# avikde/robobee3d

Measured on AMD Instinct MI355X. Metric: closed-loop MPC steps/sec (QP+dyn), higher is better.
Workload: dtype f32

## Files before the change

### robobee3d_amd/asmstep.py

```python
import functools
import os
import struct

from . import asmgen, asmtext, symbolic
from .asmgen import (A_D, A_L, A_LO, A_M, A_Q, NLDS, NVZ, S_ALPHA, S_CNT, S_ITERS, S_OMA, S_RHO, S_RINV, S_SIGMA,
                     V_W, V_WZ, V_X, V_Y, V_Z, Emit, f32bits, pk, _sb, _vp)

HERE = os.path.dirname(os.path.abspath(__file__))

PTRS = ["state", "ctrl", "ref", "ws", "out", "stats", "status", "info", "Ib", "gain", "aT0",
        "taskf", "weights", "wl", "wlu", "wlw",
        "done"]
NPTR_RES = 11
INTS = ["stride", "K", "maxIter", "nsub", "plant", "seq"]
TAIL_INTS = ["refstep"]
FLOATS = ["dt", "dtg", "Tmax", "wpr", "wpf", "ws_", "wvr", "wvf", "wds", "wthrust", "wmom",
          "iwpr", "iwpf", "iws", "iwvr", "iwvf", "iwds", "iwthrust", "iwmom",
          "Ib0", "Ib1", "Ib2", "Ibi0", "Ibi1", "Ibi2", "h", "hh", "h6", "taulim", "gpl", "idt", "mbg"]
WNAMES = ["wpr", "wpf", "ws_", "wvr", "wvf", "wds", "wthrust", "wmom"]
WROW = {"ws_": 0, "wds": 1, "wpr": 2, "wpf": 3, "wvr": 4, "wvf": 5, "wthrust": 6, "wmom": 7}
A_W, A_IW = 230, 238
S_PARAM = 4
S_PBLK = 2
S_PTR = {n: 40 + 2 * k for k, n in enumerate(PTRS[:NPTR_RES])}
S_PTR["taskf"], S_PTR["weights"] = 0, 96
S_PTR["wl"], S_PTR["wlu"], S_PTR["wlw"] = 30, 32, 34
S_INT = {"stride": 10, "K": 13, "maxIter": S_ITERS, "nsub": 5, "plant": 39}
S_F = {n: 64 + k for k, n in enumerate(FLOATS)}
assert max(S_F.values()) <= 95
S_STEP, S_SUB, S_RUIZ = 12, 15, 15
S_EXACT = 14
S_MBAD, S_MP0 = 62, 14
S_M0, S_M1, S_M2, S_M3 = 30, 32, 34, 36
S_C = {"minscal": 16, "maxscal": 17, "c45": 18, "eps10": 19, "eps": 38, "rho": 6, "rinv": 7, "rmin": 8,
       "rmininv": 9, "infty_ms": 100, "rhotol": 101}
S_TMP = 4
OFF = {}
_o = 0
for _n in PTRS:
    OFF[_n] = _o
    _o += 8
for _n in INTS + FLOATS + TAIL_INTS:
    OFF[_n] = _o
    _o += 4
PARAM_BYTES = _o
HIST_INTS = ["statestep", "outstep", "statusstep", "infostep"]
HIST_OFF = (PARAM_BYTES + 7) // 8 * 8
for _k, _n in enumerate(HIST_INTS):
    OFF[_n] = HIST_OFF + 4 * _k
HIST_BYTES = 4 * len(HIST_INTS)
S_HIST = 32
IMP_OFF = HIST_OFF + HIST_BYTES
assert IMP_OFF % 8 == 0
OFF["imp"], OFF["impstep"] = IMP_OFF, IMP_OFF + 8
IMP_BYTES = 16
S_IMP = 32

VFIRST, VEND = 2, 256
NRING = 6
XV_N, XV_B = 2, 254
NT_PTRS = ("state", "ctrl", "ref", "out", "stats")
A_SPARE, N_SPARE_D = 246, 9


class Pool:

    def __init__(self, e):
        self.e = e
        self.free_ = set(range(VFIRST, VEND))
        self.peak = 0
        self.fixed = set()

    def _take(self, regs):
        for r in regs:
            assert r in self.free_, "v%d is not free" % r
            self.free_.discard(r)
        self.peak = max(self.peak, VEND - VFIRST - len(self.free_))

    def reserve(self, lo, n):
        self._take(range(lo, lo + n))
        return lo

    def get(self):
        cand = sorted(self.free_)
        assert cand, "out of VGPRs"
        for r in cand:
            if (r ^ 1) not in self.free_:
                self._take([r])
                return r
        self._take([cand[0]])
        return cand[0]

    def get2(self):
        for r in sorted(self.free_):
            if r % 2 == 0 and r + 1 in self.free_:
                self._take([r, r + 1])
                return r
        raise AssertionError("out of aligned VGPR pairs")

    def get4(self):
        for r in sorted(self.free_):
            if r % 4 == 0 and all(r + k in self.free_ for k in range(4)):
                self._take([r, r + 1, r + 2, r + 3])
                return r
        raise AssertionError("out of aligned VGPR quads")

    def getn(self, n):
        for r in sorted(self.free_):
            if r % 2 == 0 and all(r + k in self.free_ for k in range(n)):
                self._take(range(r, r + n))
                return r
        raise AssertionError("out of consecutive VGPRs")

    def getn_high(self, n):
        r = VEND - n - (VEND - n) % 2
# ... 77 lines not shown
        for p in range(len(s.A_i)):
            if p in used:
                continue
            i0, j0 = s.A_i[p], self.col_of[p]
            for q_ in range(p + 1, len(s.A_i)):
                if q_ in used:
                    continue
                i1, j1 = s.A_i[q_], self.col_of[q_]
                if (self.zs[i0] ^ 1) == self.zs[i1] and (j0 == j1 or (self.xs[j0] ^ 1) == self.xs[j1]):
                    lo, hi = (p, q_) if self.zs[i0] % 2 == 0 else (q_, p)
                    pairs.append((lo, hi))
                    used.update((p, q_))
                    break
        self.apairs = pairs
        self.asingles = [p for p in range(len(s.A_i)) if p not in used]
        self.apos = [0] * len(s.A_i)
        k = 0
        for (lo, hi) in pairs:
            self.apos[lo], self.apos[hi] = k, k + 1
            k += 2
        for p in self.asingles:
            self.apos[p] = k
            k += 1
        self.na = k
        self.pair_of = {}
        for (lo, hi) in pairs:
            self.pair_of[lo] = self.pair_of[hi] = (lo, hi)
        NYv = symbolic.NY
        self.qnz = list(range(s.N * NYv)) + [s.N * NYv + k_ * NYv + i for k_ in range(s.N) for i in range(3)]
        self.qslot = {}
        for j in range(s.N * NYv):
            self.qslot[j] = self.xs[j]
        base = s.N * NYv
        for k_ in range(s.N):
            for i in range(3):
                self.qslot[s.N * NYv + k_ * NYv + i] = base + 3 * k_ + i
        self.nq = base + 3 * s.N
        self.qzero = frozenset(j for j in range(nx) if j not in self.qslot)
        lnz = set(range(6)) | set(range(3 * 6, 3 * 6 + 6)) | set(range(4 * 6, 4 * 6 + 3)) | {5 * 6 + 2}
        self.lzero = frozenset(i for i in range(self.neq) if i not in lnz) if s.N == 3 else frozenset()

    def weight_of(self, j):
        N, NYv = self.s.N, symbolic.NY
        if j < N * NYv:
            k, i = divmod(j, NYv)
            return ("wpf" if k == N - 1 else "wpr") if i < 3 else "ws_"
        if j < 2 * N * NYv:
            k, i = divmod(j - N * NYv, NYv)
            return ("wvf" if k == N - 1 else "wvr") if i < 3 else "wds"
        return "wthrust" if (j - 2 * N * NYv) % 3 == 0 else "wmom"


class StepGen:
    def __init__(self, N=3, perm=None, quad=False, exact_ruiz=False):
        self.st = Struct(N, perm)
        self.s = self.st.s
        self.e = Emit()
        self.pool = Pool(self.e)
        self.lab = 20
        self.lab_spec = 500
        self.quad = quad
        self.speculate = not quad and not exact_ruiz
        self.ruiz_span = self.restart_at = None
        self.nt = () if quad else ("nt",)
        self.homes = asmgen.Homes(NRING, 0 if quad else XV_N, XV_B)

    def label(self):
        self.lab += 1
        return str(self.lab)

    def label_spec(self):
        self.lab_spec += 1
        return str(self.lab_spec)

    def rcp_nr(self, dst, src, t):
        e = self.e
        e("v_rcp_f32", v(dst), v(src))
        e("s_nop", 0)
        e("v_fma_f32", v(t), "-" + v(src), v(dst), 1.0)
        e("v_fma_f32", v(dst), v(t), v(dst), v(dst))

    def rows_ptr(self, voff, first_row):
        e = self.e
        if first_row == 0:
            e("v_mov_b32", v(voff), "v0")
        else:
            e("s_mul_i32", sg(S_TMP), sg(S_INT["stride"]), first_row)
            e("v_add_u32", v(voff), sg(S_TMP), "v0")

    def load_taskf(self):
        e = self.e
        e("s_lshl_b32", sg(S_TMP), sg(S_STEP), 5)
        e("s_load_dwordx2", sp(S_M0), sp(S_PTR["taskf"]), sg(S_TMP), "offset:0")
        e("s_load_dwordx4", "s[%d:%d]" % (S_M0 + 2, S_M0 + 5), sp(S_PTR["taskf"]), sg(S_TMP), "offset:8")
        e("s_load_dwordx2", sp(S_M0 + 6), sp(S_PTR["taskf"]), sg(S_TMP), "offset:24")
        e("s_waitcnt", "vmcnt(0) lgkmcnt(0)")

    def adv(self, voff):
        self.e("v_add_u32", v(voff), sg(S_INT["stride"]), v(voff))

    def advance_ptr(self, ptr, sstep):
        e, lo = self.e, S_PTR[ptr]
        e("s_add_i32", sg(lo), sg(lo), sg(sstep))
        e("s_cmp_lt_u32", sg(lo), sg(sstep))
        e("s_cselect_b32", sg(sstep), 1, 0)
        e("s_add_i32", sg(lo + 1), sg(lo + 1), sg(sstep))

    def impulse(self, Y0, YS):
        e = self.e
        lab_off = self.label()
        lo, hi, st, oh = S_IMP, S_IMP + 1, S_IMP + 2, S_IMP + 3
        e("s_mov_b32", sg(S_TMP), IMP_OFF)
        e("s_load_dwordx4", "s[%d:%d]" % (S_IMP, S_IMP + 3), sp(S_PBLK), sg(S_TMP))
        e("s_waitcnt", "lgkmcnt(0)")
        e("s_cmp_eq_u64", sp(lo), 0)
        e("s_cbranch_scc1", lab_off + "f")
        e("s_mul_hi_u32", sg(oh), sg(S_STEP), sg(st))
        e("s_mul_i32", sg(st), sg(S_STEP), sg(st))
        e("s_add_i32", sg(hi), sg(hi), sg(oh))
        for i in range(6):
            addend = st if i == 0 else S_INT["stride"]
            lab_nc = self.label()
            e("s_add_i32", sg(lo), sg(lo), sg(addend))
            e("s_cmp_gt_u32", sg(addend), sg(lo))
            e("s_cbranch_scc0", lab_nc + "f")
            e("s_add_i32", sg(hi), sg(hi), 1)
            e("label", lab_nc)
            e("global_load_dword", v(YS + i), "v0", sp(lo))
        e("s_waitcnt", "vmcnt(0)")
        for i in range(6):
            e("v_add_f32", v(Y0 + 12 + i), v(Y0 + 12 + i), v(YS + i))
        e("label", lab_off)

    def load_rows(self, ptr, first_row, regs, voff=None):
        own = voff is None
        if own:
            voff = self.pool.get()
        self.rows_ptr(voff, first_row)
        for k, r in enumerate(regs):
            self.e("global_load_dword", r if isinstance(r, str) else v(r), v(voff), sp(S_PTR[ptr]),
                   *(self.nt if ptr in NT_PTRS or ptr == "ws" else ()))
            if k + 1 < len(regs):
                self.adv(voff)
        if own:
            self.pool.free(voff, kill=False)

    def store_rows(self, ptr, first_row, regs, voff=None):
        own = voff is None
        if own:
            voff = self.pool.get()
        self.rows_ptr(voff, first_row)
        for k, r in enumerate(regs):
# ... 186 lines not shown
        dtT0 = g_()
        e("v_mul_f32", v(dtT0), SF("dt"), v(T0))
        s0dt = [g_() for _ in range(3)]
        Bdt = [g_() for _ in range(6)]
        for i in range(3):
            e("v_mul_f32", v(s0dt[i]), SF("dt"), v(s0[i]))
        for i in range(6):
            e("v_mul_f32", v(Bdt[i]), SF("dt"), v(Btau[i]))
        pool.free(*Btau, *ds0, T0)
        VP = pool.getn(nx + 1)
        VQ = pool.getn_high(st.nq + st.nq % 2)
        VA = pool.getn(st.na + st.na % 2)
        self.VP, self.VQ, self.VA = VP, VQ, VA
        RP = lambda j: VP + st.xs[j]
        RA = lambda p: VA + st.apos[p]
        RQ = lambda j: VQ + st.qslot[j]
        self.RP, self.RA, self.RQ = RP, RA, RQ
        for j in range(nx):
            e("v_accvgpr_read_b32", v(RP(j)), "a%d" % (A_W + WNAMES.index(st.weight_of(j))))
        e("v_mov_b32", v(VP + nx), 0)
        ydes = RF[0:3] + RF[6:9]
        dpdes = RF[3:6]
        WV = {n: pool.get() for n in ("wpr", "wpf", "ws_", "wvr", "wvf")}
        for n, r in WV.items():
            e("v_accvgpr_read_b32", v(r), "a%d" % (A_W + WNAMES.index(n)))
        for j in st.qnz:
            if j < N * NYv:
                k, i = divmod(j, NYv)
                wname = ("wpf" if k == N - 1 else "wpr") if i < 3 else "ws_"
                e("v_mul_f32", v(RQ(j)), "-" + v(WV[wname]), v(ydes[i]))
            else:
                k, i = divmod(j - N * NYv, NYv)
                e("v_mul_f32", v(RQ(j)), "-" + v(WV["wvf" if k == N - 1 else "wvr"]), v(dpdes[i]))
        if st.nq % 2:
            e("v_mov_b32", v(VQ + st.nq), 0)
        for p, tag in enumerate(s.A_tag):
            if tag[0] == 'c':
                e("v_mov_b32", v(RA(p)), float(tag[1]))
            elif tag[0] == 'dt':
                e("v_mov_b32", v(RA(p)), SF("dt"))
            elif tag[0] == 'T0dt':
                e("v_mov_b32", v(RA(p)), v(dtT0))
            elif tag[0] == 's0':
                e("v_mov_b32", v(RA(p)), v(s0dt[tag[1]]))
            else:
                e("v_mov_b32", v(RA(p)), v(Bdt[tag[1]]))
        if st.na % 2:
            e("v_mov_b32", v(VA + st.na), 0)
        pool.free(dtT0, *s0dt, *Bdt, t)
        pool.free(*ST)
        pool.free(*RF)
        pool.free(*WV.values())
        pool.free_range(LS, 20)
        self.ruiz_quad() if self.quad else self.ruiz()
        self.recover_and_bounds()
        self.factor()

    def maxabs(self, dst, regs, acc_in=False):
        e = self.e
        regs = list(regs)
        if not acc_in:
            if len(regs) == 1:
                e("v_and_b32", v(dst), 0x7fffffff, v(regs[0]))
                return
            if len(regs) == 2:
                e("v_max_f32", v(dst), "|%s|" % v(regs[0]), "|%s|" % v(regs[1]))
                return
            e("v_max3_f32", v(dst), "|%s|" % v(regs[0]), "|%s|" % v(regs[1]), "|%s|" % v(regs[2]))
            regs = regs[3:]
        while len(regs) >= 2:
            e("v_max3_f32", v(dst), v(dst), "|%s|" % v(regs[0]), "|%s|" % v(regs[1]))
            regs = regs[2:]
        if regs:
            e("v_max_f32", v(dst), v(dst), "|%s|" % v(regs[0]))

    def limit(self, regs, rsq):
        e = self.e
        regs = list(regs)
        prev = None
        for r in regs + [None]:
            if r is not None:
                e("v_cmp_lt_f32", "vcc", sg(S_C["minscal"]), v(r))
            if prev is not None:
                e("v_min_f32", v(prev), sg(S_C["maxscal"]), v(prev))
            if r is not None:
                e("v_cndmask_b32", v(r), 1.0, v(r), "vcc")
            prev = r
        if rsq:
            for r in regs:
                e("v_rsq_f32", v(r), v(r))
            e("s_nop", 0)

    def scalings(self, regs, track):
        if track is None:
            return self.limit(regs, rsq=True)
        e = self.e
        regs = list(regs)
        lo, hi = track
        for k in range(0, len(regs) - 1, 2):
            e("v_min3_f32", v(lo), v(lo), v(regs[k]), v(regs[k + 1]))
            e("v_max3_f32", v(hi), v(hi), v(regs[k]), v(regs[k + 1]))
        if len(regs) % 2:
            e("v_min_f32", v(lo), v(lo), v(regs[-1]))
            e("v_max_f32", v(hi), v(hi), v(regs[-1]))
        for r in regs:
            e("v_rsq_f32", v(r), v(r))
        e("s_nop", 0)

# ... 252 lines not shown
        self.maxabs(qn, [hostQ[C] for C in sorted(hostQ)])
        e("s_mov_b64", "exec", sp(S_L3))
        e("v_mov_b32", v(acc), 0)
        e("v_mov_b32", v(qn), 0)
        e("s_mov_b64", "exec", sp(asmquad.S_EXEC))
        e("s_nop", 4)
        for perm_ in ([1, 0, 3, 2], [2, 3, 0, 1]):
            e("v_add_f32_dpp", v(acc), v(acc), v(acc), asmquad.qperm(perm_))
            e("v_max_f32_dpp", v(qn), v(qn), v(qn), asmquad.qperm(perm_))
            e("s_nop", 1)
        e("v_mul_f32", v(acc), sg(S_C["c45"]), v(acc))
        self.limit([qn], rsq=False)
        e("v_max_f32", v(acc), v(acc), v(qn))
        self.limit([acc], rsq=False)
        self.rcp_nr(ct, acc, tt)
        for C in range(15):
            e("v_mul_f32", v(hostP[C]), v(hostP[C]), v(ct))
            if C in hostQ:
                e("v_mul_f32", v(hostQ[C]), v(hostQ[C]), v(ct))
        e("v_mul_f32", v(cs), v(cs), v(ct))
        e("s_sub_i32", sg(S_RUIZ), sg(S_RUIZ), 1)
        e("s_cmp_gt_i32", sg(S_RUIZ), 0)
        e("s_cbranch_scc1", top + "b")
        e("s_nop", 1)

        def bcast(dst, src, ln):
            e("v_mov_b32_dpp", v(dst), v(src), asmquad.qperm([ln] * 4))
        for key, d in rp.slots.items():
            for ln in sorted(d, reverse=True):
                bcast(RA(d[ln]), hostA[key], ln)
        for C, m in colmem.items():
            for ln in sorted(m, reverse=True):
                bcast(RP(m[ln]), hostP[C], ln)
            if C in hostQ:
                for ln in sorted(m, reverse=True):
                    bcast(RQ(m[ln]), hostQ[C], ln)
        e("v_mov_b32", v(self.VP + nx), 0)
        if st.nq % 2:
            e("v_mov_b32", v(self.VQ + st.nq), 0)
        if st.na % 2:
            e("v_mov_b32", v(self.VA + st.na), 0)
        e("s_nop", 1)
        e("quad_end", tuple(keep))

    def recover_and_bounds(self):
        e, pool, st, s = self.e, self.pool, self.st, self.s
        N, nx, nc, neq = s.N, s.nx, s.nc, st.neq
        RP, RA, RQ, RE, cs = self.RP, self.RA, self.RQ, self.RE, self.cs
        SF = lambda n: sg(S_F[n])
        cinv, t, d, r = pool.get(), pool.get(), pool.get(), pool.get()
        self.rcp_nr(cinv, cs, t)
        voff = pool.get()
        npark = 0 if self.quad else N_SPARE_D
        self.rows_ptr(voff, npark)
        rows_of_col = {}
        for i in range(nc):
            rows_of_col.setdefault(st.unit[i][1], []).append(i)
        IWV = {n: pool.get() for n in WNAMES}
        for k, n in enumerate(WNAMES):
            e("v_accvgpr_read_b32", v(IWV[n]), "a%d" % (A_IW + k))
        for j in range(nx):
            e("v_mul_f32", v(d), v(RP(j)), v(cinv))
            e("v_mul_f32", v(d), v(IWV[st.weight_of(j)]), v(d))
            e("v_sqrt_f32", v(d), v(d))
            e("s_nop", 0)
            if j < npark:
                e("v_accvgpr_write_b32", "a%d" % (A_SPARE + j), v(d))
            else:
                e("global_store_dword", v(voff), v(d), sp(S_PTR["ws"]), *self.nt)
                self.adv(voff)
            if j in rows_of_col:
                e("v_rcp_f32", v(r), v(d))
                e("s_nop", 0)
                for i in rows_of_col[j]:
                    e("v_mul_f32", v(RE(i)), "|%s|" % v(RA(st.unit[i][0])), v(r))
        assert asmgen.WS_ES == asmgen.WS_DS + nx and asmgen.WS_C == asmgen.WS_ES + nc
        for i in range(nc):
            e("global_store_dword", v(voff), v(RE(i)), sp(S_PTR["ws"]), *self.nt)
            self.adv(voff)
        if npark:
            e("v_accvgpr_write_b32", "a%d" % (A_SPARE + N_SPARE_D), v(cs))
        else:
            e("global_store_dword", v(voff), v(cs), sp(S_PTR["ws"]))
        self.store_rows("ctrl", nx + 2 * nc + 1, [RE(neq + k) for k in range(N)], voff)
        pool.free(cinv, d, r, voff, cs, *IWV.values())
        LS = pool.getn(20)
        for qd in range(5):
            e("ds_read_b128", "v[%d:%d]" % (LS + 4 * qd, LS + 4 * qd + 3), "v1", qd * 1024)
        zero = pool.get()
        e("v_mov_b32", v(zero), 0)
        for j in range(nx):
            e("v_accvgpr_write_b32", "a%d" % (A_Q + j), v(RQ(j)) if j in st.qslot else v(zero))
        e("s_waitcnt", "lgkmcnt(0)")
        src = {}
        for i in range(6):
            src[i] = LS + i
            src[3 * 6 + i] = LS + 6 + i
        for i in range(3):
            src[4 * 6 + i] = LS + 12 + i
        for i in range(neq):
            if i in src:
                e("v_mul_f32", v(t), v(src[i]), v(RE(i)))
                e("v_accvgpr_write_b32", "a%d" % (A_LO + i), v(t))
            elif i == 5 * 6 + 2:
                e("v_mul_f32", v(t), SF("dtg"), v(RE(i)))
                e("v_accvgpr_write_b32", "a%d" % (A_LO + i), v(t))
            else:
                e("v_accvgpr_write_b32", "a%d" % (A_LO + i), v(zero))
        for k in range(N):
            e("v_mul_f32", v(t), v(LS + 15), v(RE(neq + k)))
            e("v_accvgpr_write_b32", "a%d" % (A_M + k), v(t))
            e("v_mul_f32", v(t), v(LS + 16), v(RE(neq + k)))
            e("v_accvgpr_write_b32", "a%d" % (A_M + N + k), v(t))
        pool.free(zero, t)
        pool.free_range(LS, 20)
        pool.free_range(self.VE, nc + 1)
        pool.free_range(self.VQ, st.nq + st.nq % 2)

    def factor(self):
        e, pool, st, s = self.e, self.pool, self.st, self.s
        nx, nc, nk, neq = s.nx, s.nc, s.nk, st.neq
        RP, RA = self.RP, self.RA
        lpos = st.lpos
        last_row = {}
        for c in range(nk):
            if s.L_p[c + 1] > s.L_p[c]:
                last_row[c] = s.L_i[s.L_p[c + 1] - 1]
        done_at = {}
        for c, r in last_row.items():
            done_at.setdefault(r, []).append(c)
# ... 60 lines not shown
                pool.free(yc)
            assert not y
            di = pool.get()
            self.rcp_nr(di, dk, t)
            pool.free(dk)
            Dinv[k] = di
            for c in done_at.get(k, []):
                retire_col(c)
            if k not in last_row:
                retire_dinv(k)
        assert not nL and not Dinv
        pool.free(t)
        if self._rinv_reg is not None:
            pool.free(self._rinv_reg)
            self._rinv_reg = None
        if st.na % 2:
            pool.free(self.VA + st.na)
        pool.free(self.VP + nx)

    _rinv_reg = None

    def _vconst_rinv(self):
        if self._rinv_reg is None:
            self._rinv_reg = self.pool.get()
            self.e("v_mov_b32", v(self._rinv_reg), sg(S_RINV))
        return v(self._rinv_reg)

    def admm(self):
        e, pool, st, s = self.e, self.pool, self.st, self.s
        nx, nc = s.nx, s.nc
        left = set(range(VFIRST, VEND)) - pool.free_ - set(range(246, 256))
        assert not left, "phase A leaked registers: %s" % sorted(left)
        pool.reserve(V_W, V_X - V_W)
        pool.reserve(V_X, V_Y - V_X)
        pool.reserve(V_Y, V_Z - V_Y)
        pool.reserve(V_Z, 40)
        voff = 245
        self.load_rows("ctrl", 0, [V_X + st.xs[r] for r in range(nx)] + [V_Y + st.zs[r] for r in range(nc)] +
                       [V_Z + st.zs[r] for r in range(nc)], voff)
        for pad in (V_X + nx, V_Y + nc, V_Z + nc, V_W + nx, V_WZ + nc):
            e("v_mov_b32", v(pad), 0)
        e("s_waitcnt", "vmcnt(0) lgkmcnt(0)")
        plan = st.plan
        zk = dict(qzero=st.qzero, lzero=st.lzero, homes=self.homes)
        asmgen.body(e, s, first=True, capture=True, plan=plan, delta_in_w=True, **zk)
        if self.quad:
            from . import asmquad
            lab6 = self.label()
            e("s_cmp_lt_i32", sg(S_ITERS), 2)
            e("s_cbranch_scc1", lab6 + "f")
            asmquad.section(e, asmquad.QuadPlan(st), self.label)
            e("label", lab6)
        else:
            self._admm_rest(plan, zk)
        for i in range(st.neq):
            pool.free(V_Z + st.zs[i], kill=True)
        pool.free_range(246, 10)


    def _admm_rest(self, plan, zk):
        e, s, st = self.e, self.s, self.st
        import numpy as np
        for p_ in range(NVZ):
            e("v_accvgpr_read_b32", v(V_Z + p_), "a%d" % (A_L + p_))
        lab7, lab6 = self.label(), self.label()
        e("s_sub_i32", sg(S_CNT), sg(S_ITERS), 1)
        e("s_cmp_lt_i32", sg(S_CNT), 1)
        e("s_cbranch_scc1", lab6 + "f")
        e("label", lab7)
        asmgen.body(e, s, first=False, capture=False, plan=plan, lv=True, dy3_in_w=True, **zk)
        e("s_sub_i32", sg(S_CNT), sg(S_CNT), 1)
        e("s_cmp_gt_i32", sg(S_CNT), 0)
        e("s_cbranch_scc1", lab7 + "b")
        k = float(np.float32(1.6) / (np.float32(1.6) - np.float32(1.0)))
        e("s_mov_b32", sg(S_TMP), f32bits(k))
        nx, neq = s.nx, st.neq
        for p_ in range(0, nx - 1, 2):
            pk(e, "v_pk_add_f32", V_W + p_, [P2(V_X + p_), P2(V_W + p_)], [0, 1])
        for p_ in range(0, nx - 1, 2):
            pk(e, "v_pk_mul_f32", V_W + p_, [PS(S_TMP), P2(V_W + p_)])
        if nx % 2:
            jl = st.xinv[nx - 1]
            e("v_sub_f32", v(V_W + st.xs[jl]), v(V_X + st.xs[jl]), v(V_W + st.xs[jl]))
            e("v_mul_f32", v(V_W + st.xs[jl]), sg(S_TMP), v(V_W + st.xs[jl]))
        for p_ in range(0, neq, 2):
            pk(e, "v_pk_add_f32", V_WZ + p_, [P2(V_Y + p_), P2(V_WZ + p_)], [0, 1])
        for p_ in range(0, neq, 2):
            pk(e, "v_pk_mul_f32", V_WZ + p_, [PS(S_TMP), P2(V_WZ + p_)])
        e("label", lab6)

    def phase_c(self):
        e, pool, st, s = self.e, self.pool, self.st, self.s
        N, NYv = s.N, symbolic.NY
        nx, nc, neq = s.nx, s.nc, st.neq
        SF = lambda n: sg(S_F[n])
        g_ = pool.get
        XR = lambda j: V_X + st.xs[j]
        YR = lambda i: V_Y + st.zs[i]
        ZR = lambda i: V_Z + st.zs[i]
        DXR = lambda j: V_W + st.xs[j]
        DYR = lambda i: V_WZ + st.zs[i]
        voff = g_()
        def slot_blocks(n, chunk=16):
            n2 = n + n % 2
            blocks = [(lo, pool.getn(min(chunk, n2 - lo))) for lo in range(0, n2, chunk)]
            def reg(slot):
                for lo, base in reversed(blocks):
                    if slot >= lo:
                        return base + slot - lo
            return reg, [(base, min(chunk, n2 - lo)) for lo, base in blocks]
        DS, dblocks = slot_blocks(nx)
        DR = lambda j: DS(st.xs[j])
        cr, T0 = g_(), g_()
        npark = 0 if self.quad else N_SPARE_D
        self.load_rows("ws", npark, [DR(j) for j in range(npark, nx)], voff)
        if npark:
            for j in range(npark):
                e("v_accvgpr_read_b32", v(DR(j)), "a%d" % (A_SPARE + j))
            e("v_accvgpr_read_b32", v(cr), "a%d" % (A_SPARE + N_SPARE_D))
        else:
            self.load_rows("ws", asmgen.WS_C - asmgen.WS_DS, [cr], voff)
        self.load_rows("ctrl", nx + 2 * nc, [T0], voff)
        e("v_mov_b32", v(DS(nx)), 0)
        zt = [g_() for _ in range(4)]
        self.rows_ptr(voff, 0)
        for r in range(nx):
            e("global_store_dword", v(voff), v(XR(r)), sp(S_PTR["ctrl"]), *self.nt)
            self.adv(voff)
        for r in range(nc):
            e("global_store_dword", v(voff), v(YR(r)), sp(S_PTR["ctrl"]), *self.nt)
            self.adv(voff)
        for r in range(nc):
            if r < neq:
                t_ = zt[r % 4]
                e("v_accvgpr_read_b32", v(t_), "a%d" % (A_LO + r))
                e("global_store_dword", v(voff), v(t_), sp(S_PTR["ctrl"]), *self.nt)
            else:
                e("global_store_dword", v(voff), v(ZR(r)), sp(S_PTR["ctrl"]), *self.nt)
            self.adv(voff)
        pool.free(*zt)
        e("s_waitcnt", "vmcnt(0)")
        for k in range(0, nx + 1, 2):
            pk(e, "v_pk_mul_f32", V_W + k, [P2(DS(k)), P2(V_W + k)])
            pk(e, "v_pk_mul_f32", V_X + k, [P2(DS(k)), P2(V_X + k)])
        for base, n_ in dblocks:
            pool.free_range(base, n_)
        ES, eblocks = slot_blocks(nc)
        ER = lambda i: ES(st.zs[i])
        ST = [g_() for _ in range(18)]
        RF = [g_() for _ in range(9)]
        self.load_rows("ws", asmgen.WS_ES - asmgen.WS_DS, [ER(i) for i in range(nc)], voff)
        self.load_rows("state", 0, ST, voff)
        self.load_rows("ref", 0, RF, voff)
        e("v_mov_b32", v(ES(nc)), 1.0)
        lab_tk = self.label()
        e("s_cmp_eq_u64", sp(S_PTR["taskf"]), 0)
        e("s_cbranch_scc1", lab_tk + "f")
        self.load_taskf()
        for i in range(3):
            e("v_add_f32", v(RF[i]), sg(S_M0 + i), v(RF[i]))
            e("v_mov_b32", v(RF[3 + i]), sg(S_M0 + 3 + i))
        e("v_mov_b32", v(RF[6]), sg(S_M0 + 6))
        e("v_mov_b32", v(RF[7]), 0)
        e("v_mov_b32", v(RF[8]), sg(S_M0 + 7))
        e("label", lab_tk)
        cinv, t = g_(), g_()
        self.rcp_nr(cinv, cr, t)
        pool.free(cr)
        ibi0, ibi1 = g_(), g_()
        lab_ib, lab_ib2 = self.label(), self.label()
        e("s_cmp_eq_u64", sp(S_PTR["Ib"]), 0)
        e("s_cbranch_scc1", lab_ib + "f")
        self.load_rows("Ib", 0, [ibi0, ibi1], voff)
        e("s_waitcnt", "vmcnt(0)")
        tt = g_()
        for r in (ibi0, ibi1):
            e("v_mov_b32", v(tt), v(r))
            self.rcp_nr(r, tt, t)
        pool.free(tt)
        e("s_branch", lab_ib2 + "f")
        e("label", lab_ib)
        e("v_mov_b32", v(ibi0), SF("Ibi0"))
        e("v_mov_b32", v(ibi1), SF("Ibi1"))
        e("label", lab_ib2)
        e("s_waitcnt", "vmcnt(0)")
        for k in range(0, nc + 1, 2):
            pk(e, "v_pk_mul_f32", V_WZ + k, [P2(ES(k)), P2(V_WZ + k)])
            pk(e, "v_pk_mul_f32", V_Y + k, [P2(ES(k)), P2(V_Y + k)])
        for k in range(0, nc + 1, 2):
            pk(e, "v_pk_mul_f32", V_Y + k, [P2(V_Y + k), PB(cinv)])
        pool.free(cinv)
        zu3 = [g_() for _ in range(N)]
        for k in range(N):
            e("v_rcp_f32", v(zu3[k]), v(ER(neq + k)))
        e("s_nop", 0)
        for k in range(N):
            e("v_mul_f32", v(zu3[k]), v(ZR(neq + k)), v(zu3[k]))
        for base, n_ in eblocks:
            pool.free_range(base, n_)
        for k in range(N):
            pool.free(ZR(neq + k))
        pool.free(V_Z + nc)
        p0, R0, dq0 = ST[0:3], ST[3:12], ST[12:18]
        dtT0 = g_()
        e("v_mul_f32", v(dtT0), SF("dt"), v(T0))
        s0dt = [g_() for _ in range(3)]
        Bdt = [g_() for _ in range(6)]
        for i in range(3):
            e("v_mul_f32", v(s0dt[i]), SF("dt"), v(R0[6 + i]))
            e("v_mul_f32", v(Bdt[i]), "-" + v(R0[i + 3]), v(ibi0))
            e("v_mul_f32", v(Bdt[3 + i]), v(R0[i]), v(ibi1))
        for i in range(6):
            e("v_mul_f32", v(Bdt[i]), SF("dt"), v(Bdt[i]))
        pool.free(ibi0, ibi1)
        ds0 = [g_() for _ in range(3)]
        for r in range(3):
            e("v_mul_f32", v(t), "-" + v(R0[r]), v(dq0[4]))
            e("v_mul_f32", v(ds0[r]), v(R0[r + 3]), v(dq0[3]))
            e("v_add_f32", v(ds0[r]), v(t), v(ds0[r]))
            e("v_mul_f32", v(ds0[r]), -1.0, v(ds0[r]))
        y0 = p0 + R0[6:9]
        dy0 = dq0[0:3] + ds0
        LR = {}
        y1 = [g_() for _ in range(6)]
        for i in range(6):
            LR[i] = g_()
            e("v_mul_f32", v(t), SF("dt"), v(dy0[i]))
            e("v_add_f32", v(y1[i]), v(y0[i]), v(t))
            e("v_mul_f32", v(LR[i]), -1.0, v(y1[i]))
        for i in range(6):
            LR[18 + i] = g_()
            if i < 3:
                e("v_mul_f32", v(t), v(T0), v(y0[i + 3]))
                e("v_mul_f32", v(t), SF("dt"), v(t))
                e("v_sub_f32", v(LR[18 + i]), "-" + v(dy0[i]), v(t))
                if i == 2:
                    e("v_add_f32", v(LR[18 + i]), SF("dtg"), v(LR[18 + i]))
            else:
# ... 205 lines not shown
            e("v_cndmask_b32", v(r), v(r), v(nanv), "vcc")
        pool.free(nanv)
        u0, u1, u2 = sol[0:3]
        dy1 = sol[3:9]
        OUT = [g_() for _ in range(9)]
        e("v_add_f32", v(OUT[0]), v(T0), v(u0))
        e("v_mov_b32", v(OUT[1]), v(u1))
        e("v_mov_b32", v(OUT[2]), v(u2))
        e("v_mul_f32", v(a1), v(R0[0]), v(dy1[3]))
        e("v_mul_f32", v(t), v(R0[1]), v(dy1[4]))
        e("v_add_f32", v(a1), v(a1), v(t))
        e("v_mul_f32", v(t), v(R0[2]), v(dy1[5]))
        e("v_add_f32", v(a1), v(a1), v(t))
        e("v_mul_f32", v(a2), v(R0[3]), v(dy1[3]))
        e("v_mul_f32", v(t), v(R0[4]), v(dy1[4]))
        e("v_add_f32", v(a2), v(a2), v(t))
        e("v_mul_f32", v(t), v(R0[5]), v(dy1[5]))
        e("v_add_f32", v(a2), v(a2), v(t))
        for i in range(3):
            e("v_sub_f32", v(OUT[3 + i]), v(dy1[i]), v(dq0[i]))
        e("v_sub_f32", v(OUT[6]), "-" + v(a2), v(dq0[3]))
        e("v_sub_f32", v(OUT[7]), v(a1), v(dq0[4]))
        e("v_sub_f32", v(OUT[8]), 0, v(dq0[5]))
        for i in range(6):
            e("v_mul_f32", v(OUT[3 + i]), SF("idt"), v(OUT[3 + i]))
        self.store_rows("out", 0, OUT, voff)
        lab_s, lab_i, lab_c = self.label(), self.label(), self.label()
        e("s_cmp_eq_u64", sp(S_PTR["status"]), 0)
        e("s_cbranch_scc1", lab_s + "f")
        e("global_store_dword", "v0", v(stv), sp(S_PTR["status"]))
        e("label", lab_s)
        e("s_cmp_eq_u64", sp(S_PTR["info"]), 0)
        e("s_cbranch_scc1", lab_i + "f")
        self.store_rows("info", 0, [pri, dua], voff)
        e("label", lab_i)
        e("s_and_saveexec_b64", sp(S_M1), MBAD)
        e("s_cbranch_execz", lab_c + "f")
        e("v_mov_b32", v(a1), 0)
        self.rows_ptr(voff, 0)
        for r in range(nx + 2 * nc):
            e("global_store_dword", v(voff), v(a1), sp(S_PTR["ctrl"]))
            self.adv(voff)
        e("label", lab_c)
        e("s_mov_b64", "exec", sp(S_M1))
        pool.free(pri, dua, stv, a1, a2, t, T0, *RF)
        pool.free_range(V_W, V_X - V_W, kill=False)
        pool.free_range(V_X, V_Y - V_X, kill=False)
        pool.free_range(V_Y, V_Z - V_Y, kill=False)
        T0n = g_()
        e("v_mov_b32", v(T0n), v(OUT[0]))
        self.wl_step(OUT, R0, T0n, voff)
        self.store_rows("ctrl", nx + 2 * nc, [T0n], voff)
        pool.free(T0n)
        self.plant(ST, OUT, voff)
        pool.free(*OUT, *ST, voff)
        assert len(pool.free_) == VEND - VFIRST, "phase C leaked registers: %s" % sorted(set(range(VFIRST, VEND)) - pool.free_)

    def wl_step(self, OUT, R0, T0n, voff):
        e, pool = self.e, self.pool
        g_ = pool.get
        lab_end = self.label()
        P = sp(S_PBLK)
        e("s_load_dwordx2", sp(S_PTR["wl"]), P, OFF["wl"])
        e("s_load_dwordx2", sp(S_PTR["wlu"]), P, OFF["wlu"])
        e("s_load_dwordx2", sp(S_PTR["wlw"]), P, OFF["wlw"])
        e("s_waitcnt", "lgkmcnt(0)")
        e("s_cmp_eq_u64", sp(S_PTR["wl"]), 0)
        e("s_cbranch_scc1", lab_end + "f")
        O_UMIN, O_UMAX, O_DUMAX, O_QW, O_A0, O_A1, O_A2, O_MD = 0, 4, 8, 12, 18, 24, 48, 144
        a1, a2, t = g_(), g_(), g_()
        zero = g_()
        e("v_mov_b32", v(zero), 0)

        def prm(dst, word):
            e("global_load_dword", v(dst), v(zero), sp(S_PTR["wl"]), "offset:%d" % (4 * word))
        u0 = [g_() for _ in range(4)]
        self.load_rows("wlu", 0, u0, voff)
        Md = [g_() for _ in range(6)]
        for i in range(6):
            prm(Md[i], O_MD + i)
        e("s_waitcnt", "vmcnt(0)")
        h0 = [g_() for _ in range(3)]
        pd = [g_() for _ in range(6)]
        for c in range(3):
            e("v_mul_f32", v(h0[c]), SF_("mbg"), v(R0[2 + 3 * c]))
        for i in range(6):
            e("v_mul_f32", v(pd[i]), v(Md[i]), v(OUT[3 + i]))
        w0 = [g_() for _ in range(6)]
        a0v = [g_() for _ in range(6)]
        A1 = [[g_() for _ in range(4)] for _ in range(6)]
        PA = [g_() for _ in range(21)]
        vout = [g_() for _ in range(4)]
        dot, quad = g_(), g_()
        for i in range(6):
            prm(PA[0], O_A0 + i)
            for l in range(4):
                prm(PA[1 + l], O_A1 + 4 * i + l)
            for k in range(16):
                prm(PA[5 + k], O_A2 + 16 * i + k)
            e("s_waitcnt", "vmcnt(0)")
            e("v_mul_f32", v(dot), v(u0[0]), v(PA[1]))
            for l in range(1, 4):
                e("v_mul_f32", v(t), v(u0[l]), v(PA[1 + l]))
                e("v_add_f32", v(dot), v(dot), v(t))
            for r in range(4):
                e("v_mul_f32", v(vout[r]), v(PA[5 + r]), v(u0[0]))
# ... 329 lines not shown
            e("v_mul_f32", v(dst + 5), v(a), v(Ibi[0]))
            e("v_sub_f32", v(b), v(u2), v(b))
            e("v_mul_f32", v(dst + 6), v(b), v(Ibi[1]))
            e("v_mul_f32", v(dst + 7), "-" + v(hz), v(Ibi[2]))
        e("s_mov_b32", sg(S_SUB), sg(S_INT["nsub"]))
        top = self.label()
        e("label", top)
        vf(Q0, QA)
        for k in range(0, 8, 2):
            pk(e, "v_pk_fma_f32", QS + k, [PS(S_F["hh"]), P2(QA + k), P2(Q0 + k)])
        vf(QS, QK)
        for k in range(0, 8, 2):
            pk(e, "v_pk_fma_f32", QA + k, [PB(two), P2(QK + k), P2(QA + k)])
            pk(e, "v_pk_fma_f32", QS + k, [PS(S_F["hh"]), P2(QK + k), P2(Q0 + k)])
        vf(QS, QK)
        for k in range(0, 8, 2):
            pk(e, "v_pk_fma_f32", QA + k, [PB(two), P2(QK + k), P2(QA + k)])
            pk(e, "v_pk_fma_f32", QS + k, [PS(S_F["h"]), P2(QK + k), P2(Q0 + k)])
        vf(QS, QK)
        for k in range(0, 8, 2):
            pk(e, "v_pk_add_f32", QA + k, [P2(QA + k), P2(QK + k)])
        for k in range(0, 8, 2):
            pk(e, "v_pk_fma_f32", Q0 + k, [PS(S_F["h6"]), P2(QA + k), P2(Q0 + k)])
        e("s_nop", 1)
        for r in range(3):
            e("v_mov_b32_dpp", v(PA + r), v(Q0), asmquad.qperm([r] * 4))
        e("s_nop", 1)
        for r in range(3):
            e("v_fmac_f32", v(serr), v(PA + r), v(PA + r))
        e("v_add_f32", v(seff), v(seff), v(einc))
        e("s_sub_i32", sg(S_SUB), sg(S_SUB), 1)
        e("s_cmp_gt_i32", sg(S_SUB), 0)
        e("s_cbranch_scc1", top + "b")
        e("s_nop", 1)
        for r in range(3):
            e("v_mov_b32_dpp", v(Y0 + r), v(Q0), asmquad.qperm([r] * 4))
            e("v_mov_b32_dpp", v(Y0 + 12 + r), v(Q0 + 1), asmquad.qperm([r] * 4))
            for c in range(3):
                e("v_mov_b32_dpp", v(Y0 + 3 + r + 3 * c), v(Q0 + 2 + c), asmquad.qperm([r] * 4))
        for i in range(3):
            e("v_mov_b32", v(Y0 + 15 + i), v(Q0 + 5 + i))
        e("s_nop", 1)
        e("quad_end", tuple(keep))

    def program(self):
        e = self.e
        self.prologue()
        top = self.label()
        e("label", top)
        if self.speculate:
            e("s_mov_b32", sg(S_EXACT), 0)
            self.lab_restart = self.label_spec()
            e("label", self.lab_restart)
        self.phase_a()
        self.admm()
        self.phase_c()
        e("s_load_dword", sg(S_TMP), sp(S_PBLK), OFF["refstep"])
        e("s_load_dwordx4", "s[%d:%d]" % (S_HIST, S_HIST + 3), sp(S_PBLK), HIST_OFF)
        e("s_waitcnt", "lgkmcnt(0)")
        e("s_add_u32", sg(S_PTR["ref"]), sg(S_PTR["ref"]), sg(S_TMP))
        e("s_addc_u32", sg(S_PTR["ref"] + 1), sg(S_PTR["ref"] + 1), 0)
        for n in ("out", "status", "info"):
            self.advance_ptr(n, S_HIST + HIST_INTS.index(n + "step"))
        e("s_add_i32", sg(S_STEP), sg(S_STEP), 1)
        e("s_cmp_lt_i32", sg(S_STEP), sg(S_INT["K"]))
        e("s_cbranch_scc1", top + "b")
        e("s_waitcnt", "vmcnt(0) lgkmcnt(0)")
        lab = self.label()
        e("s_load_dwordx2", sp(S_M0), sp(S_PBLK), OFF["done"])
        e("s_load_dword", sg(S_M1), sp(S_PBLK), OFF["seq"])
        e("s_waitcnt", "lgkmcnt(0)")
        e("s_cmp_eq_u64", sp(S_M0), 0)
        e("s_cbranch_scc1", lab + "f")
        e("buffer_wbl2", "sc0 sc1")
        e("s_waitcnt", "vmcnt(0)")
        a, b = self.pool.get(), self.pool.get()
        e("v_mov_b32", v(a), 0)
        e("v_mov_b32", v(b), sg(S_M1))
        e("global_store_dword", v(a), v(b), sp(S_M0), "sc0 sc1")
        e("s_waitcnt", "vmcnt(0)")
        self.pool.free(a, b)
        e("label", lab)
        return e.ins


fmt = functools.partial(asmtext.fmt, hex_ints=asmtext.HEX_ABOVE_64)


PSEUDO = ("kill", "quad_begin", "quad_end")


def write(path=None, N=3, perm=None, quad=False):
    path = path or os.path.join(HERE, "csrc", "umpc_step_asm_quad.h" if quad else "umpc_step_asm.h")
    g = StepGen(N, perm, quad=quad)
    ins = [t for t in g.program() if t[0] not in PSEUDO]
    if quad:
        head = ["// GENERATED by robobee3d_amd/asmstep.py (quad=True) + asmquad.py -- do not edit.", asmgen.switch_banner(),
               "// The all-assembly fp32 step kernel body, ONE ROBOT PER LANE QUAD (16 robots per wavefront): %d instructions."
               % len(ins),
               "// Every lane of a quad gets the same v0 (= 4 * robot) and its own LDS slice; include umpc_step_asm.h first (StepParams).",
               "#pragma once"]
    else:
        head = ["// GENERATED by robobee3d_amd/asmstep.py -- do not edit.", asmgen.switch_banner(),
               "// The all-assembly fp32 step kernel body: %d instructions (K closed-loop steps of one wavefront)." % len(ins),
               "#pragma once", "#include <stddef.h>", "#include <stdint.h>", "namespace umpcasm {",
               "// parameter block read by the kernel with s_load (byte offsets are part of the generated code)",
               "struct StepParams {"]
        for n in PTRS:
            head.append("  const void *%s;" % n)
        for n in INTS:
            head.append("  int32_t %s;" % n)
        for n in FLOATS:
            head.append("  float %s;" % n)
        for n in TAIL_INTS:
            head.append("  int32_t %s;" % n)
        head += ["};", "static_assert(sizeof(StepParams) == %d, \"StepParams layout\");" % ((PARAM_BYTES + 7) // 8 * 8),
                "// step history (umpcBatchSetHistory): bytes the state / out / status / info pointers advance per closed-loop step,",
                "// read by the stream at byte %d of the kernarg segment: the kernels take ONE StepArgs as their first argument" % HIST_OFF,
                "struct StepHist {"] + ["  int32_t %s;" % n for n in HIST_INTS] + ["};",
                "// velocity impulses (umpcBatchSetImpulses): slice `cursor` of the table [steps][6][B] (null: none) and the bytes per slice,",
                "// read by the stream at byte %d of the kernarg segment" % IMP_OFF,
                "struct StepImp {", "  const void *imp;", "  int32_t impstep;", "  int32_t pad_;", "};",
                "struct StepArgs {", "  StepParams p;", "  StepHist h;", "  StepImp i;", "};",
                "static_assert(offsetof(StepArgs, h) == %d && sizeof(StepHist) == %d, \"StepHist layout\");" % (HIST_OFF, HIST_BYTES),
                "static_assert(offsetof(StepArgs, i) == %d && sizeof(StepImp) == %d && offsetof(StepImp, impstep) == 8, \"StepImp layout\");" % (IMP_OFF, IMP_BYTES),
                "constexpr int STEP_LDS_BYTES_PER_LANE = %d;" % (NLDS * 4), "}  // namespace umpcasm",
                "// inputs: v0 = 4 * robot, v1 = lane LDS address, s[4:5] = &StepParams (kernarg)"]
    asmtext.write_if_changed(path, asmtext.asm_block(
        head, "UMPC_STEP_ASM%s(voff, ldsaddr, params)" % ("_QUAD" if quad else ""), ins,
        '"{v0}"(voff), "{v1}"(ldsaddr), "{s[4:5]}"(params)',
        asmtext.clobbers(range(2, 256), range(256), range(4, 102)), fmt))
    return path, len(ins)


_KEEP_V = {0, 1} | set(range(V_W, V_Z)) | set(range(V_Z + 2 * 3 * symbolic.NY, V_Z + 40))
QUAD = {None: None}


def _quad():
    from . import isasim
    if QUAD[None] is None:
        QUAD.update({None: isasim.Quad(v=_KEEP_V, dead_v=set(range(256)) - _KEEP_V, a=range(A_LO, 256), dead_a=range(A_LO)),
                     "ruiz": isasim.Quad(a=range(256)), "plant": isasim.Quad(a=range(256))})
    return QUAD


FLAT = ("taskf", "wl")
STRIDE = 4096
PBASE = 0x00007E0080000000


def simulate(ins, arrays, ints, floats, max_exec=3000000, ptr_xform=None, lanes=1, hits=False):
    import numpy as np
    from . import isasim
    base_of = {n: 0x00007F0080000000 + (k << 36) for k, n in enumerate(PTRS + ["impulse"])}
    ptr_xform = ptr_xform or (lambda a: a)
    blob = bytearray(IMP_OFF + IMP_BYTES)
    for n in PTRS:
        struct.pack_into("<Q", blob, OFF[n], ptr_xform(base_of[n]) if arrays.get(n) is not None else 0)
    stride = STRIDE if lanes == 1 else 4 * lanes
    allints = dict(ints, stride=stride)
    allints.setdefault("seq", 0)
    allints.setdefault("refstep", 0)
    for n in HIST_INTS:
        allints.setdefault(n, 0)
    for n in INTS + TAIL_INTS + HIST_INTS:
        struct.pack_into("<i", blob, OFF[n], int(allints[n]))
    for n in FLOATS:
        struct.pack_into("<f", blob, OFF[n], float(floats[n]))
    allints.setdefault("impstep", 6 * stride if arrays.get("impulse") is not None else 0)
    struct.pack_into("<Q", blob, OFF["imp"], ptr_xform(base_of["impulse"]) if arrays.get("impulse") is not None else 0)
    struct.pack_into("<i", blob, OFF["impstep"], int(allints["impstep"]))
    regions = [(PBASE, 4, np.frombuffer(bytes(blob), np.uint32))] + \
        [(base_of[n], 4 if n in FLAT or lanes > 1 else STRIDE, arrays[n].reshape(-1))
         for n in PTRS + ["impulse"] if arrays.get(n) is not None]
    assert all(arrays[n].flags.c_contiguous for n in PTRS + ["impulse"] if arrays.get(n) is not None)
    m = isasim.Machine(ins, lanes, regions=regions, sgpr={S_PARAM: PBASE & 0xFFFFFFFF, S_PARAM + 1: PBASE >> 32},
                       vgpr={0: 4 * np.arange(lanes)}, lds=np.zeros((lanes, NLDS), np.uint32), max_exec=max_exec,
                       quad=_quad() if lanes == 1 else None)
    if hits:
        m.hits = np.zeros(len(ins), np.int64)
    isasim.run(m)
    simulate.last_hits = m.hits
    simulate.last_quad_sections = {("admm" if k is None else k): n for k, n in m.sections.items()}
    simulate.last_quad_instructions = sum(m.sections.values())
    return m.nexec


if __name__ == "__main__":
    p, n = write()
    print("wrote", p, n, "instructions")


def host_floats(dt=5.0, g=9.81e-3, TtoWmax=2.0, ws=1e1, wds=1e3, wpr=1.0, wpf=5.0, wvr=1e3, wvf=2e3, wthrust=1e-1, wmom=1e-2,
                Ib=(3333.0, 3333.0, 1000.0), dtsim=0.2, taulim=100.0, mb=100.0):
    import numpy as np
    f = np.float32
    one = f(1.0)
    w = dict(wpr=f(wpr), wpf=f(wpf), ws_=f(ws), wvr=f(wvr), wvf=f(wvf), wds=f(wds), wthrust=f(wthrust), wmom=f(wmom))
    d = dict(dt=f(dt), dtg=f(f(dt) * f(g)), Tmax=f(f(TtoWmax) * f(g)), **w)
    for k, val in w.items():
        d["i" + k.rstrip("_")] = f(one / val)
    for i in range(3):
        d["Ib%d" % i] = f(Ib[i])
        d["Ibi%d" % i] = f(one / f(Ib[i]))
    d.update(h=f(dtsim), hh=f(f(0.5) * f(dtsim)), h6=f(f(dtsim) / f(6.0)), taulim=f(taulim), gpl=f(9.81e-3), idt=f(one / f(dt)),
             mbg=f(f(mb) * f(g)))
    assert set(d) == set(FLOATS), set(FLOATS) ^ set(d)
    return {k: float(val) for k, val in d.items()}
```

### robobee3d_amd/csrc/umpc_step_asm.h

```cpp
#pragma once
#include <stddef.h>
#include <stdint.h>
namespace umpcasm {
struct StepParams {
  const void *state;
  const void *ctrl;
  const void *ref;
  const void *ws;
  const void *out;
  const void *stats;
  const void *status;
  const void *info;
  const void *Ib;
  const void *gain;
  const void *aT0;
  const void *taskf;
  const void *weights;
  const void *wl;
  const void *wlu;
  const void *wlw;
  const void *done;
  int32_t stride;
  int32_t K;
  int32_t maxIter;
// ... 1929 lines not shown
  "v_pk_mul_f32 v[82:83], v[82:83], v[48:49] op_sel:[0,0] op_sel_hi:[1,0] neg_lo:[0,0] neg_hi:[0,0]\n" \
  "v_pk_mul_f32 v[84:85], v[84:85], v[48:49] op_sel:[0,0] op_sel_hi:[1,0] neg_lo:[0,0] neg_hi:[0,0]\n" \
  "v_pk_mul_f32 v[86:87], v[86:87], v[48:49] op_sel:[0,0] op_sel_hi:[1,0] neg_lo:[0,0] neg_hi:[0,0]\n" \
  "v_pk_mul_f32 v[88:89], v[88:89], v[48:49] op_sel:[0,0] op_sel_hi:[1,0] neg_lo:[0,0] neg_hi:[0,0]\n" \
  "v_pk_mul_f32 v[90:91], v[90:91], v[48:49] op_sel:[0,0] op_sel_hi:[1,0] neg_lo:[0,0] neg_hi:[0,0]\n" \
  "v_pk_mul_f32 v[92:93], v[92:93], v[48:49] op_sel:[0,0] op_sel_hi:[1,0] neg_lo:[0,0] neg_hi:[0,0]\n" \
  "v_pk_mul_f32 v[94:95], v[94:95], v[48:49] op_sel:[0,0] op_sel_hi:[1,0] neg_lo:[0,0] neg_hi:[0,0]\n" \
  "v_pk_mul_f32 v[96:97], v[96:97], v[48:49] op_sel:[0,0] op_sel_hi:[1,0] neg_lo:[0,0] neg_hi:[0,0]\n" \
  "v_pk_mul_f32 v[98:99], v[98:99], v[48:49] op_sel:[0,0] op_sel_hi:[1,0] neg_lo:[0,0] neg_hi:[0,0]\n" \
  "v_pk_mul_f32 v[100:101], v[100:101], v[48:49] op_sel:[0,0] op_sel_hi:[1,0] neg_lo:[0,0] neg_hi:[0,0]\n" \
  "v_pk_mul_f32 v[102:103], v[102:103], v[48:49] op_sel:[0,0] op_sel_hi:[1,0] neg_lo:[0,0] neg_hi:[0,0]\n" \
  "v_pk_mul_f32 v[104:105], v[104:105], v[48:49] op_sel:[0,0] op_sel_hi:[1,0] neg_lo:[0,0] neg_hi:[0,0]\n" \
  "v_pk_mul_f32 v[106:107], v[106:107], v[48:49] op_sel:[0,0] op_sel_hi:[1,0] neg_lo:[0,0] neg_hi:[0,0]\n" \
  "v_pk_mul_f32 v[108:109], v[108:109], v[48:49] op_sel:[0,0] op_sel_hi:[1,0] neg_lo:[0,0] neg_hi:[0,0]\n" \
  "v_pk_mul_f32 v[110:111], v[110:111], v[48:49] op_sel:[0,0] op_sel_hi:[1,0] neg_lo:[0,0] neg_hi:[0,0]\n" \
  "v_pk_mul_f32 v[112:113], v[112:113], v[48:49] op_sel:[0,0] op_sel_hi:[1,0] neg_lo:[0,0] neg_hi:[0,0]\n" \
  "v_pk_mul_f32 v[114:115], v[114:115], v[48:49] op_sel:[0,0] op_sel_hi:[1,0] neg_lo:[0,0] neg_hi:[0,0]\n" \
  "v_pk_mul_f32 v[228:229], v[228:229], v[48:49] op_sel:[0,0] op_sel_hi:[1,0] neg_lo:[0,0] neg_hi:[0,0]\n" \
  "v_pk_mul_f32 v[230:231], v[230:231], v[48:49] op_sel:[0,0] op_sel_hi:[1,0] neg_lo:[0,0] neg_hi:[0,0]\n" \
  "v_pk_mul_f32 v[232:233], v[232:233], v[48:49] op_sel:[0,0] op_sel_hi:[1,0] neg_lo:[0,0] neg_hi:[0,0]\n" \
  "v_pk_mul_f32 v[234:235], v[234:235], v[48:49] op_sel:[0,0] op_sel_hi:[1,0] neg_lo:[0,0] neg_hi:[0,0]\n" \
  "v_pk_mul_f32 v[236:237], v[236:237], v[48:49] op_sel:[0,0] op_sel_hi:[1,0] neg_lo:[0,0] neg_hi:[0,0]\n" \
  "v_pk_mul_f32 v[238:239], v[238:239], v[48:49] op_sel:[0,0] op_sel_hi:[1,0] neg_lo:[0,0] neg_hi:[0,0]\n" \
  "v_pk_mul_f32 v[240:241], v[240:241], v[48:49] op_sel:[0,0] op_sel_hi:[1,0] neg_lo:[0,0] neg_hi:[0,0]\n" \
  "v_pk_mul_f32 v[242:243], v[242:243], v[48:49] op_sel:[0,0] op_sel_hi:[1,0] neg_lo:[0,0] neg_hi:[0,0]\n" \
  "v_pk_mul_f32 v[244:245], v[244:245], v[48:49] op_sel:[0,0] op_sel_hi:[1,0] neg_lo:[0,0] neg_hi:[0,0]\n" \
  "v_pk_mul_f32 v[246:247], v[246:247], v[48:49] op_sel:[0,0] op_sel_hi:[1,0] neg_lo:[0,0] neg_hi:[0,0]\n" \
  "v_pk_mul_f32 v[248:249], v[248:249], v[48:49] op_sel:[0,0] op_sel_hi:[1,0] neg_lo:[0,0] neg_hi:[0,0]\n" \
  "v_pk_mul_f32 v[250:251], v[250:251], v[48:49] op_sel:[0,0] op_sel_hi:[1,0] neg_lo:[0,0] neg_hi:[0,0]\n" \
  "v_pk_mul_f32 v[252:253], v[252:253], v[48:49] op_sel:[0,0] op_sel_hi:[1,0] neg_lo:[0,0] neg_hi:[0,0]\n" \
  "v_pk_mul_f32 v[254:255], v[254:255], v[48:49] op_sel:[0,0] op_sel_hi:[1,0] neg_lo:[0,0] neg_hi:[0,0]\n" \
  "v_mul_f32 v42, v42, v48\n" \
  "s_sub_i32 s15, s15, 1\n" \
  "s_cmp_gt_i32 s15, 0\n" \
  "s_cbranch_scc1 503b\n" \
  "v_cmp_lt_f32_e64 s[30:31], s16, v43\n" \
  "v_cmp_ge_f32_e64 s[32:33], s17, v44\n" \
  "s_and_b64 s[30:31], s[30:31], s[32:33]\n" \
  "s_andn2_b64 s[30:31], exec, s[30:31]\n" \
  "s_cbranch_scc0 505f\n" \
  "s_mov_b32 s14, 1\n" \
  "s_waitcnt vmcnt(0) lgkmcnt(0)\n" \
  "s_branch 501b\n" \
  "504:\n" \
  "s_cmp_gt_i32 s15, 0\n" \
  "s_cbranch_scc1 28b\n" \
  "505:\n" \
  "v_rcp_f32 v43, v42\n" \
  "s_nop 0\n" \
  "v_fma_f32 v44, -v42, v43, 1.0\n" \
  "v_fma_f32 v43, v44, v43, v43\n" \
  "s_mul_i32 s4, s10, 9\n" \
  "v_add_u32 v47, s4, v0\n" \
  "v_accvgpr_read_b32 v48, a238\n" \
  "v_accvgpr_read_b32 v49, a239\n" \
  "v_accvgpr_read_b32 v50, a240\n" \
  "v_accvgpr_read_b32 v51, a241\n" \
  "v_accvgpr_read_b32 v52, a242\n" \
  "v_accvgpr_read_b32 v53, a243\n" \
  "v_accvgpr_read_b32 v54, a244\n" \
  "v_accvgpr_read_b32 v55, a245\n" \
  "v_mul_f32 v45, v70, v43\n" \
  "v_mul_f32 v45, v48, v45\n" \
  "v_sqrt_f32 v45, v45\n" \
  "s_nop 0\n" \
  "v_accvgpr_write_b32 a246, v45\n" \
  "v_rcp_f32 v46, v45\n" \
  "s_nop 0\n" \
  "v_mul_f32 v2, |v116|, v46\n" \
  "v_mul_f32 v8, |v118|, v46\n" \
  "v_mul_f32 v45, v71, v43\n" \
  "v_mul_f32 v45, v48, v45\n" \
  "v_sqrt_f32 v45, v45\n" \
  "s_nop 0\n" \
  "v_accvgpr_write_b32 a247, v45\n" \
  "v_rcp_f32 v46, v45\n" \
  "s_nop 0\n" \
  "v_mul_f32 v3, |v117|, v46\n" \
  "v_mul_f32 v9, |v119|, v46\n" \
  "v_mul_f32 v45, v72, v43\n" \
  "v_mul_f32 v45, v48, v45\n" \
  "v_sqrt_f32 v45, v45\n" \
  "s_nop 0\n" \
  "v_accvgpr_write_b32 a248, v45\n" \
  "v_rcp_f32 v46, v45\n" \
  "s_nop 0\n" \
  "v_mul_f32 v4, |v120|, v46\n" \
  "v_mul_f32 v10, |v122|, v46\n" \
  "v_mul_f32 v45, v74, v43\n" \
  "v_mul_f32 v45, v50, v45\n" \
  "v_sqrt_f32 v45, v45\n" \
  "s_nop 0\n" \
  "v_accvgpr_write_b32 a249, v45\n" \
  "v_rcp_f32 v46, v45\n" \
  "s_nop 0\n" \
  "v_mul_f32 v6, |v124|, v46\n" \
  "v_mul_f32 v12, |v126|, v46\n" \
  "v_mul_f32 v45, v75, v43\n" \
  "v_mul_f32 v45, v50, v45\n" \
  "v_sqrt_f32 v45, v45\n" \
  "s_nop 0\n" \
  "v_accvgpr_write_b32 a250, v45\n" \
  "v_rcp_f32 v46, v45\n" \
  "s_nop 0\n" \
  "v_mul_f32 v7, |v125|, v46\n" \
  "v_mul_f32 v13, |v127|, v46\n" \
  "v_mul_f32 v45, v73, v43\n" \
  "v_mul_f32 v45, v50, v45\n" \
  "v_sqrt_f32 v45, v45\n" \
  "s_nop 0\n" \
  "v_accvgpr_write_b32 a251, v45\n" \
  "v_rcp_f32 v46, v45\n" \
  "s_nop 0\n" \
  "v_mul_f32 v5, |v121|, v46\n" \
  "v_mul_f32 v11, |v123|, v46\n" \
  "v_mul_f32 v45, v76, v43\n" \
  "v_mul_f32 v45, v48, v45\n" \
  "v_sqrt_f32 v45, v45\n" \
  "s_nop 0\n" \
  "v_accvgpr_write_b32 a252, v45\n" \
  "v_rcp_f32 v46, v45\n" \
  "s_nop 0\n" \
  "v_mul_f32 v14, |v132|, v46\n" \
  "v_mul_f32 v45, v77, v43\n" \
  "v_mul_f32 v45, v48, v45\n" \
  "v_sqrt_f32 v45, v45\n" \
  "s_nop 0\n" \
  "v_accvgpr_write_b32 a253, v45\n" \
  "v_rcp_f32 v46, v45\n" \
  "s_nop 0\n" \
  "v_mul_f32 v15, |v133|, v46\n" \
  "v_mul_f32 v45, v78, v43\n" \
  "v_mul_f32 v45, v48, v45\n" \
  "v_sqrt_f32 v45, v45\n" \
  "s_nop 0\n" \
  "v_accvgpr_write_b32 a254, v45\n" \
  "v_rcp_f32 v46, v45\n" \
  "s_nop 0\n" \
  "v_mul_f32 v16, |v136|, v46\n" \
  "v_mul_f32 v45, v80, v43\n" \
  "v_mul_f32 v45, v50, v45\n" \
  "v_sqrt_f32 v45, v45\n" \
  "s_nop 0\n" \
  "global_store_dword v47, v45, s[46:47] nt\n" \
  "v_add_u32 v47, s10, v47\n" \
  "v_rcp_f32 v46, v45\n" \
  "s_nop 0\n" \
  "v_mul_f32 v18, |v140|, v46\n" \
  "v_mul_f32 v45, v81, v43\n" \
  "v_mul_f32 v45, v50, v45\n" \
  "v_sqrt_f32 v45, v45\n" \
  "s_nop 0\n" \
  "global_store_dword v47, v45, s[46:47] nt\n" \
  "v_add_u32 v47, s10, v47\n" \
  "v_rcp_f32 v46, v45\n" \
  "s_nop 0\n" \
  "v_mul_f32 v19, |v141|, v46\n" \
  "v_mul_f32 v45, v79, v43\n" \
  "v_mul_f32 v45, v50, v45\n" \
  "v_sqrt_f32 v45, v45\n" \
  "s_nop 0\n" \
  "global_store_dword v47, v45, s[46:47] nt\n" \
  "v_add_u32 v47, s10, v47\n" \
  "v_rcp_f32 v46, v45\n" \
  "s_nop 0\n" \
  "v_mul_f32 v17, |v137|, v46\n" \
  "v_mul_f32 v45, v82, v43\n" \
  "v_mul_f32 v45, v49, v45\n" \
  "v_sqrt_f32 v45, v45\n" \
  "s_nop 0\n" \
  "global_store_dword v47, v45, s[46:47] nt\n" \
  "v_add_u32 v47, s10, v47\n" \
  "v_mul_f32 v45, v83, v43\n" \
  "v_mul_f32 v45, v49, v45\n" \
  "v_sqrt_f32 v45, v45\n" \
  "s_nop 0\n" \
  "global_store_dword v47, v45, s[46:47] nt\n" \
  "v_add_u32 v47, s10, v47\n" \
  "v_mul_f32 v45, v84, v43\n" \
  "v_mul_f32 v45, v49, v45\n" \
  "v_sqrt_f32 v45, v45\n" \
  "s_nop 0\n" \
  "global_store_dword v47, v45, s[46:47] nt\n" \
  "v_add_u32 v47, s10, v47\n" \
  "v_mul_f32 v45, v86, v43\n" \
  "v_mul_f32 v45, v50, v45\n" \
  "v_sqrt_f32 v45, v45\n" \
  "s_nop 0\n" \
  "global_store_dword v47, v45, s[46:47] nt\n" \
  "v_add_u32 v47, s10, v47\n" \
  "v_mul_f32 v45, v87, v43\n" \
  "v_mul_f32 v45, v50, v45\n" \
  "v_sqrt_f32 v45, v45\n" \
  "s_nop 0\n" \
  "global_store_dword v47, v45, s[46:47] nt\n" \
  "v_add_u32 v47, s10, v47\n" \
  "v_mul_f32 v45, v85, v43\n" \
  "v_mul_f32 v45, v50, v45\n" \
  "v_sqrt_f32 v45, v45\n" \
  "s_nop 0\n" \
  "global_store_dword v47, v45, s[46:47] nt\n" \
  "v_add_u32 v47, s10, v47\n" \
  "v_mul_f32 v45, v88, v43\n" \
  "v_mul_f32 v45, v51, v45\n" \
  "v_sqrt_f32 v45, v45\n" \
  "s_nop 0\n" \
  "global_store_dword v47, v45, s[46:47] nt\n" \
  "v_add_u32 v47, s10, v47\n" \
  "v_rcp_f32 v46, v45\n" \
  "s_nop 0\n" \
  "v_mul_f32 v20, |v150|, v46\n" \
  "v_mul_f32 v26, |v152|, v46\n" \
  "v_mul_f32 v45, v89, v43\n" \
  "v_mul_f32 v45, v51, v45\n" \
  "v_sqrt_f32 v45, v45\n" \
  "s_nop 0\n" \
  "global_store_dword v47, v45, s[46:47] nt\n" \
  "v_add_u32 v47, s10, v47\n" \
  "v_rcp_f32 v46, v45\n" \
  "s_nop 0\n" \
  "v_mul_f32 v21, |v151|, v46\n" \
  "v_mul_f32 v27, |v153|, v46\n" \
  "v_mul_f32 v45, v90, v43\n" \
  "v_mul_f32 v45, v51, v45\n" \
  "v_sqrt_f32 v45, v45\n" \
  "s_nop 0\n" \
  "global_store_dword v47, v45, s[46:47] nt\n" \
  "v_add_u32 v47, s10, v47\n" \
  "v_rcp_f32 v46, v45\n" \
  "s_nop 0\n" \
  "v_mul_f32 v22, |v156|, v46\n" \
  "v_mul_f32 v28, |v158|, v46\n" \
  "v_mul_f32 v45, v92, v43\n" \
  "v_mul_f32 v45, v53, v45\n" \
  "v_sqrt_f32 v45, v45\n" \
  "s_nop 0\n" \
  "global_store_dword v47, v45, s[46:47] nt\n" \
  "v_add_u32 v47, s10, v47\n" \
  "v_rcp_f32 v46, v45\n" \
  "s_nop 0\n" \
  "v_mul_f32 v24, |v162|, v46\n" \
  "v_mul_f32 v30, |v164|, v46\n" \
  "v_mul_f32 v45, v93, v43\n" \
  "v_mul_f32 v45, v53, v45\n" \
  "v_sqrt_f32 v45, v45\n" \
  "s_nop 0\n" \
  "global_store_dword v47, v45, s[46:47] nt\n" \
  "v_add_u32 v47, s10, v47\n" \
  "v_rcp_f32 v46, v45\n" \
  "s_nop 0\n" \
  "v_mul_f32 v25, |v163|, v46\n" \
  "v_mul_f32 v31, |v165|, v46\n" \
  "v_mul_f32 v45, v91, v43\n" \
  "v_mul_f32 v45, v53, v45\n" \
  "v_sqrt_f32 v45, v45\n" \
  "s_nop 0\n" \
  "global_store_dword v47, v45, s[46:47] nt\n" \
  "v_add_u32 v47, s10, v47\n" \
  "v_rcp_f32 v46, v45\n" \
  "s_nop 0\n" \
  "v_mul_f32 v23, |v157|, v46\n" \
  "v_mul_f32 v29, |v159|, v46\n" \
  "v_mul_f32 v45, v94, v43\n" \
  "v_mul_f32 v45, v51, v45\n" \
  "v_sqrt_f32 v45, v45\n" \
  "s_nop 0\n" \
  "global_store_dword v47, v45, s[46:47] nt\n" \
  "v_add_u32 v47, s10, v47\n" \
  "v_rcp_f32 v46, v45\n" \
  "s_nop 0\n" \
  "v_mul_f32 v32, |v170|, v46\n" \
  "v_mul_f32 v45, v95, v43\n" \
  "v_mul_f32 v45, v51, v45\n" \
  "v_sqrt_f32 v45, v45\n" \
  "s_nop 0\n" \
  "global_store_dword v47, v45, s[46:47] nt\n" \
  "v_add_u32 v47, s10, v47\n" \
  "v_rcp_f32 v46, v45\n" \
  "s_nop 0\n" \
  "v_mul_f32 v33, |v171|, v46\n" \
  "v_mul_f32 v45, v96, v43\n" \
  "v_mul_f32 v45, v51, v45\n" \
  "v_sqrt_f32 v45, v45\n" \
  "s_nop 0\n" \
  "global_store_dword v47, v45, s[46:47] nt\n" \
  "v_add_u32 v47, s10, v47\n" \
  "v_rcp_f32 v46, v45\n" \
  "s_nop 0\n" \
  "v_mul_f32 v34, |v176|, v46\n" \
  "v_mul_f32 v45, v98, v43\n" \
  "v_mul_f32 v45, v53, v45\n" \
  "v_sqrt_f32 v45, v45\n" \
  "s_nop 0\n" \
  "global_store_dword v47, v45, s[46:47] nt\n" \
  "v_add_u32 v47, s10, v47\n" \
  "v_rcp_f32 v46, v45\n" \
  "s_nop 0\n" \
  "v_mul_f32 v36, |v182|, v46\n" \
  "v_mul_f32 v45, v99, v43\n" \
  "v_mul_f32 v45, v53, v45\n" \
  "v_sqrt_f32 v45, v45\n" \
  "s_nop 0\n" \
  "global_store_dword v47, v45, s[46:47] nt\n" \
  "v_add_u32 v47, s10, v47\n" \
  "v_rcp_f32 v46, v45\n" \
  "s_nop 0\n" \
  "v_mul_f32 v37, |v183|, v46\n" \
  "v_mul_f32 v45, v97, v43\n" \
  "v_mul_f32 v45, v53, v45\n" \
  "v_sqrt_f32 v45, v45\n" \
  "s_nop 0\n" \
  "global_store_dword v47, v45, s[46:47] nt\n" \
  "v_add_u32 v47, s10, v47\n" \
  "v_rcp_f32 v46, v45\n" \
  "s_nop 0\n" \
  "v_mul_f32 v35, |v177|, v46\n" \
  "v_mul_f32 v45, v100, v43\n" \
  "v_mul_f32 v45, v52, v45\n" \
  "v_sqrt_f32 v45, v45\n" \
  "s_nop 0\n" \
  "global_store_dword v47, v45, s[46:47] nt\n" \
  "v_add_u32 v47, s10, v47\n" \
  "v_mul_f32 v45, v101, v43\n" \
  "v_mul_f32 v45, v52, v45\n" \
  "v_sqrt_f32 v45, v45\n" \
  "s_nop 0\n" \
  "global_store_dword v47, v45, s[46:47] nt\n" \
  "v_add_u32 v47, s10, v47\n" \
  "v_mul_f32 v45, v102, v43\n" \
  "v_mul_f32 v45, v52, v45\n" \
  "v_sqrt_f32 v45, v45\n" \
  "s_nop 0\n" \
  "global_store_dword v47, v45, s[46:47] nt\n" \
  "v_add_u32 v47, s10, v47\n" \
  "v_mul_f32 v45, v104, v43\n" \
  "v_mul_f32 v45, v53, v45\n" \
  "v_sqrt_f32 v45, v45\n" \
  "s_nop 0\n" \
  "global_store_dword v47, v45, s[46:47] nt\n" \
  "v_add_u32 v47, s10, v47\n" \
  "v_mul_f32 v45, v105, v43\n" \
  "v_mul_f32 v45, v53, v45\n" \
  "v_sqrt_f32 v45, v45\n" \
  "s_nop 0\n" \
  "global_store_dword v47, v45, s[46:47] nt\n" \
  "v_add_u32 v47, s10, v47\n" \
  "v_mul_f32 v45, v103, v43\n" \
  "v_mul_f32 v45, v53, v45\n" \
  "v_sqrt_f32 v45, v45\n" \
  "s_nop 0\n" \
  "global_store_dword v47, v45, s[46:47] nt\n" \
  "v_add_u32 v47, s10, v47\n" \
  "v_mul_f32 v45, v106, v43\n" \
  "v_mul_f32 v45, v54, v45\n" \
  "v_sqrt_f32 v45, v45\n" \
  "s_nop 0\n" \
  "global_store_dword v47, v45, s[46:47] nt\n" \
  "v_add_u32 v47, s10, v47\n" \
  "v_rcp_f32 v46, v45\n" \
  "s_nop 0\n" \
  "v_mul_f32 v38, |v219|, v46\n" \
  "v_mul_f32 v45, v107, v43\n" \
  "v_mul_f32 v45, v55, v45\n" \
  "v_sqrt_f32 v45, v45\n" \
  "s_nop 0\n" \
  "global_store_dword v47, v45, s[46:47] nt\n" \
  "v_add_u32 v47, s10, v47\n" \
  "v_mul_f32 v45, v108, v43\n" \
  "v_mul_f32 v45, v55, v45\n" \
  "v_sqrt_f32 v45, v45\n" \
  "s_nop 0\n" \
  "global_store_dword v47, v45, s[46:47] nt\n" \
  "v_add_u32 v47, s10, v47\n" \
  "v_mul_f32 v45, v109, v43\n" \
  "v_mul_f32 v45, v54, v45\n" \
  "v_sqrt_f32 v45, v45\n" \
  "s_nop 0\n" \
  "global_store_dword v47, v45, s[46:47] nt\n" \
  "v_add_u32 v47, s10, v47\n" \
  "v_rcp_f32 v46, v45\n" \
  "s_nop 0\n" \
  "v_mul_f32 v39, |v222|, v46\n" \
  "v_mul_f32 v45, v110, v43\n" \
  "v_mul_f32 v45, v55, v45\n" \
  "v_sqrt_f32 v45, v45\n" \
  "s_nop 0\n" \
  "global_store_dword v47, v45, s[46:47] nt\n" \
  "v_add_u32 v47, s10, v47\n" \
  "v_mul_f32 v45, v111, v43\n" \
  "v_mul_f32 v45, v55, v45\n" \
  "v_sqrt_f32 v45, v45\n" \
  "s_nop 0\n" \
  "global_store_dword v47, v45, s[46:47] nt\n" \
  "v_add_u32 v47, s10, v47\n" \
  "v_mul_f32 v45, v112, v43\n" \
  "v_mul_f32 v45, v54, v45\n" \
  "v_sqrt_f32 v45, v45\n" \
  "s_nop 0\n" \
  "global_store_dword v47, v45, s[46:47] nt\n" \
  "v_add_u32 v47, s10, v47\n" \
  "v_rcp_f32 v46, v45\n" \
  "s_nop 0\n" \
  "v_mul_f32 v40, |v225|, v46\n" \
  "v_mul_f32 v45, v113, v43\n" \
  "v_mul_f32 v45, v55, v45\n" \
  "v_sqrt_f32 v45, v45\n" \
  "s_nop 0\n" \
  "global_store_dword v47, v45, s[46:47] nt\n" \
  "v_add_u32 v47, s10, v47\n" \
  "v_mul_f32 v45, v114, v43\n" \
  "v_mul_f32 v45, v55, v45\n" \
  "v_sqrt_f32 v45, v45\n" \
  "s_nop 0\n" \
  "global_store_dword v47, v45, s[46:47] nt\n" \
  "v_add_u32 v47, s10, v47\n" \
  "global_store_dword v47, v2, s[46:47] nt\n" \
  "v_add_u32 v47, s10, v47\n" \
  "global_store_dword v47, v3, s[46:47] nt\n" \
  "v_add_u32 v47, s10, v47\n" \
  "global_store_dword v47, v4, s[46:47] nt\n" \
  "v_add_u32 v47, s10, v47\n" \
  "global_store_dword v47, v6, s[46:47] nt\n" \
  "v_add_u32 v47, s10, v47\n" \
  "global_store_dword v47, v7, s[46:47] nt\n" \
  "v_add_u32 v47, s10, v47\n" \
  "global_store_dword v47, v5, s[46:47] nt\n" \
  "v_add_u32 v47, s10, v47\n" \
  "global_store_dword v47, v8, s[46:47] nt\n" \
  "v_add_u32 v47, s10, v47\n" \
  "global_store_dword v47, v9, s[46:47] nt\n" \
  "v_add_u32 v47, s10, v47\n" \
  "global_store_dword v47, v10, s[46:47] nt\n" \
  "v_add_u32 v47, s10, v47\n" \
  "global_store_dword v47, v12, s[46:47] nt\n" \
  "v_add_u32 v47, s10, v47\n" \
  "global_store_dword v47, v13, s[46:47] nt\n" \
  "v_add_u32 v47, s10, v47\n" \
  "global_store_dword v47, v11, s[46:47] nt\n" \
  "v_add_u32 v47, s10, v47\n" \
  "global_store_dword v47, v14, s[46:47] nt\n" \
  "v_add_u32 v47, s10, v47\n" \
  "global_store_dword v47, v15, s[46:47] nt\n" \
  "v_add_u32 v47, s10, v47\n" \
  "global_store_dword v47, v16, s[46:47] nt\n" \
  "v_add_u32 v47, s10, v47\n" \
  "global_store_dword v47, v18, s[46:47] nt\n" \
  "v_add_u32 v47, s10, v47\n" \
  "global_store_dword v47, v19, s[46:47] nt\n" \
  "v_add_u32 v47, s10, v47\n" \
  "global_store_dword v47, v17, s[46:47] nt\n" \
  "v_add_u32 v47, s10, v47\n" \
  "global_store_dword v47, v20, s[46:47] nt\n" \
  "v_add_u32 v47, s10, v47\n" \
  "global_store_dword v47, v21, s[46:47] nt\n" \
  "v_add_u32 v47, s10, v47\n" \
  "global_store_dword v47, v22, s[46:47] nt\n" \
  "v_add_u32 v47, s10, v47\n" \
  "global_store_dword v47, v24, s[46:47] nt\n" \
  "v_add_u32 v47, s10, v47\n" \
  "global_store_dword v47, v25, s[46:47] nt\n" \
  "v_add_u32 v47, s10, v47\n" \
  "global_store_dword v47, v23, s[46:47] nt\n" \
  "v_add_u32 v47, s10, v47\n" \
  "global_store_dword v47, v26, s[46:47] nt\n" \
  "v_add_u32 v47, s10, v47\n" \
  "global_store_dword v47, v27, s[46:47] nt\n" \
  "v_add_u32 v47, s10, v47\n" \
  "global_store_dword v47, v28, s[46:47] nt\n" \
  "v_add_u32 v47, s10, v47\n" \
  "global_store_dword v47, v30, s[46:47] nt\n" \
  "v_add_u32 v47, s10, v47\n" \
  "global_store_dword v47, v31, s[46:47] nt\n" \
  "v_add_u32 v47, s10, v47\n" \
  "global_store_dword v47, v29, s[46:47] nt\n" \
  "v_add_u32 v47, s10, v47\n" \
  "global_store_dword v47, v32, s[46:47] nt\n" \
  "v_add_u32 v47, s10, v47\n" \
  "global_store_dword v47, v33, s[46:47] nt\n" \
  "v_add_u32 v47, s10, v47\n" \
  "global_store_dword v47, v34, s[46:47] nt\n" \
  "v_add_u32 v47, s10, v47\n" \
  "global_store_dword v47, v36, s[46:47] nt\n" \
  "v_add_u32 v47, s10, v47\n" \
  "global_store_dword v47, v37, s[46:47] nt\n" \
  "v_add_u32 v47, s10, v47\n" \
  "global_store_dword v47, v35, s[46:47] nt\n" \
  "v_add_u32 v47, s10, v47\n" \
  "global_store_dword v47, v38, s[46:47] nt\n" \
  "v_add_u32 v47, s10, v47\n" \
  "global_store_dword v47, v39, s[46:47] nt\n" \
  "v_add_u32 v47, s10, v47\n" \
  "global_store_dword v47, v40, s[46:47] nt\n" \
  "v_add_u32 v47, s10, v47\n" \
  "v_accvgpr_write_b32 a255, v42\n" \
  "s_mul_i32 s4, s10, 0x7c\n" \
  "v_add_u32 v47, s4, v0\n" \
  "global_store_dword v47, v38, s[42:43] nt\n" \
  "v_add_u32 v47, s10, v47\n" \
  "global_store_dword v47, v39, s[42:43] nt\n" \
  "v_add_u32 v47, s10, v47\n" \
  "global_store_dword v47, v40, s[42:43] nt\n" \
  "ds_read_b128 v[46:49], v1 offset:0\n" \
  "ds_read_b128 v[50:53], v1 offset:1024\n" \
  "ds_read_b128 v[54:57], v1 offset:2048\n" \
  "ds_read_b128 v[58:61], v1 offset:3072\n" \
  "ds_read_b128 v[62:65], v1 offset:4096\n" \
  "v_mov_b32 v45, 0\n" \
  "v_accvgpr_write_b32 a137, v228\n" \
  "v_accvgpr_write_b32 a138, v229\n" \
  "v_accvgpr_write_b32 a139, v230\n" \
  "v_accvgpr_write_b32 a140, v232\n" \
  "v_accvgpr_write_b32 a141, v233\n" \
  "v_accvgpr_write_b32 a142, v231\n" \
  "v_accvgpr_write_b32 a143, v234\n" \
  "v_accvgpr_write_b32 a144, v235\n" \
  "v_accvgpr_write_b32 a145, v236\n" \
  "v_accvgpr_write_b32 a146, v238\n" \
  "v_accvgpr_write_b32 a147, v239\n" \
  "v_accvgpr_write_b32 a148, v237\n" \
  "v_accvgpr_write_b32 a149, v240\n" \
  "v_accvgpr_write_b32 a150, v241\n" \
  "v_accvgpr_write_b32 a151, v242\n" \
  "v_accvgpr_write_b32 a152, v244\n" \
  "v_accvgpr_write_b32 a153, v245\n" \
  "v_accvgpr_write_b32 a154, v243\n" \
  "v_accvgpr_write_b32 a155, v246\n" \
  "v_accvgpr_write_b32 a156, v247\n" \
  "v_accvgpr_write_b32 a157, v248\n" \
  "v_accvgpr_write_b32 a158, v45\n" \
  "v_accvgpr_write_b32 a159, v45\n" \
  "v_accvgpr_write_b32 a160, v45\n" \
  "v_accvgpr_write_b32 a161, v249\n" \
  "v_accvgpr_write_b32 a162, v250\n" \
  "v_accvgpr_write_b32 a163, v251\n" \
  "v_accvgpr_write_b32 a164, v45\n" \
  "v_accvgpr_write_b32 a165, v45\n" \
  "v_accvgpr_write_b32 a166, v45\n" \
  "v_accvgpr_write_b32 a167, v252\n" \
  "v_accvgpr_write_b32 a168, v253\n" \
  "v_accvgpr_write_b32 a169, v254\n" \
  "v_accvgpr_write_b32 a170, v45\n" \
  "v_accvgpr_write_b32 a171, v45\n" \
  "v_accvgpr_write_b32 a172, v45\n" \
  "v_accvgpr_write_b32 a173, v45\n" \
  "v_accvgpr_write_b32 a174, v45\n" \
  "v_accvgpr_write_b32 a175, v45\n" \
  "v_accvgpr_write_b32 a176, v45\n" \
  "v_accvgpr_write_b32 a177, v45\n" \
  "v_accvgpr_write_b32 a178, v45\n" \
  "v_accvgpr_write_b32 a179, v45\n" \
  "v_accvgpr_write_b32 a180, v45\n" \
  "v_accvgpr_write_b32 a181, v45\n" \
  "s_waitcnt lgkmcnt(0)\n" \
  "v_mul_f32 v44, v46, v2\n" \
  "v_accvgpr_write_b32 a182, v44\n" \
  "v_mul_f32 v44, v47, v3\n" \
  "v_accvgpr_write_b32 a183, v44\n" \
  "v_mul_f32 v44, v48, v4\n" \
  "v_accvgpr_write_b32 a184, v44\n" \
  "v_mul_f32 v44, v49, v6\n" \
  "v_accvgpr_write_b32 a185, v44\n" \
  "v_mul_f32 v44, v50, v7\n" \
  "v_accvgpr_write_b32 a186, v44\n" \
  "v_mul_f32 v44, v51, v5\n" \
  "v_accvgpr_write_b32 a187, v44\n" \
  "v_accvgpr_write_b32 a188, v45\n" \
  "v_accvgpr_write_b32 a189, v45\n" \
  "v_accvgpr_write_b32 a190, v45\n" \
  "v_accvgpr_write_b32 a191, v45\n" \
  "v_accvgpr_write_b32 a192, v45\n" \
  "v_accvgpr_write_b32 a193, v45\n" \
  "v_accvgpr_write_b32 a194, v45\n" \
  "v_accvgpr_write_b32 a195, v45\n" \
  "v_accvgpr_write_b32 a196, v45\n" \
  "v_accvgpr_write_b32 a197, v45\n" \
  "v_accvgpr_write_b32 a198, v45\n" \
  "v_accvgpr_write_b32 a199, v45\n" \
  "v_mul_f32 v44, v52, v20\n" \
  "v_accvgpr_write_b32 a200, v44\n" \
  "v_mul_f32 v44, v53, v21\n" \
  "v_accvgpr_write_b32 a201, v44\n" \
  "v_mul_f32 v44, v54, v22\n" \
  "v_accvgpr_write_b32 a202, v44\n" \
  "v_mul_f32 v44, v55, v24\n" \
  "v_accvgpr_write_b32 a203, v44\n" \
  "v_mul_f32 v44, v56, v25\n" \
  "v_accvgpr_write_b32 a204, v44\n" \
  "v_mul_f32 v44, v57, v23\n" \
  "v_accvgpr_write_b32 a205, v44\n" \
  "v_mul_f32 v44, v58, v26\n" \
  "v_accvgpr_write_b32 a206, v44\n" \
  "v_mul_f32 v44, v59, v27\n" \
  "v_accvgpr_write_b32 a207, v44\n" \
  "v_mul_f32 v44, v60, v28\n" \
  "v_accvgpr_write_b32 a208, v44\n" \
  "v_accvgpr_write_b32 a209, v45\n" \
  "v_accvgpr_write_b32 a210, v45\n" \
  "v_accvgpr_write_b32 a211, v45\n" \
  "v_accvgpr_write_b32 a212, v45\n" \
  "v_accvgpr_write_b32 a213, v45\n" \
  "v_mul_f32 v44, s65, v34\n" \
  "v_accvgpr_write_b32 a214, v44\n" \
  "v_accvgpr_write_b32 a215, v45\n" \
  "v_accvgpr_write_b32 a216, v45\n" \
  "v_accvgpr_write_b32 a217, v45\n" \
  "v_mul_f32 v44, v61, v38\n" \
  "v_accvgpr_write_b32 a218, v44\n" \
  "v_mul_f32 v44, v62, v38\n" \
  "v_accvgpr_write_b32 a221, v44\n" \
  "v_mul_f32 v44, v61, v39\n" \
  "v_accvgpr_write_b32 a219, v44\n" \
  "v_mul_f32 v44, v62, v39\n" \
  "v_accvgpr_write_b32 a222, v44\n" \
  "v_mul_f32 v44, v61, v40\n" \
  "v_accvgpr_write_b32 a220, v44\n" \
  "v_mul_f32 v44, v62, v40\n" \
  "v_accvgpr_write_b32 a223, v44\n" \
  "v_add_f32 v3, s24, v82\n" \
  "v_rcp_f32 v82, v3\n" \
  "s_nop 0\n" \
  "v_fma_f32 v2, -v3, v82, 1.0\n" \
  "v_fma_f32 v82, v2, v82, v82\n" \
  "v_add_f32 v3, s24, v83\n" \
  "v_rcp_f32 v83, v3\n" \
  "s_nop 0\n" \
  "v_fma_f32 v2, -v3, v83, 1.0\n" \
  "v_fma_f32 v83, v2, v83, v83\n" \
  "v_add_f32 v3, s24, v84\n" \
  "v_rcp_f32 v84, v3\n" \
  "s_nop 0\n" \
  "v_fma_f32 v2, -v3, v84, 1.0\n" \
  "v_fma_f32 v84, v2, v84, v84\n" \
  "v_add_f32 v3, s24, v86\n" \
  "v_rcp_f32 v86, v3\n" \
  "s_nop 0\n" \
  "v_fma_f32 v2, -v3, v86, 1.0\n" \
  "v_fma_f32 v86, v2, v86, v86\n" \
  "v_add_f32 v3, s24, v87\n" \
  "v_rcp_f32 v87, v3\n" \
  "s_nop 0\n" \
  "v_fma_f32 v2, -v3, v87, 1.0\n" \
// ... 3615 lines not shown
  "v_pk_mul_f32 v[32:33], s[4:5], v[32:33] op_sel:[0,0] op_sel_hi:[0,1] neg_lo:[0,0] neg_hi:[0,0]\n" \
  "v_pk_mul_f32 v[34:35], s[4:5], v[34:35] op_sel:[0,0] op_sel_hi:[0,1] neg_lo:[0,0] neg_hi:[0,0]\n" \
  "v_pk_mul_f32 v[36:37], s[4:5], v[36:37] op_sel:[0,0] op_sel_hi:[0,1] neg_lo:[0,0] neg_hi:[0,0]\n" \
  "v_pk_mul_f32 v[38:39], s[4:5], v[38:39] op_sel:[0,0] op_sel_hi:[0,1] neg_lo:[0,0] neg_hi:[0,0]\n" \
  "v_pk_mul_f32 v[40:41], s[4:5], v[40:41] op_sel:[0,0] op_sel_hi:[0,1] neg_lo:[0,0] neg_hi:[0,0]\n" \
  "v_pk_mul_f32 v[42:43], s[4:5], v[42:43] op_sel:[0,0] op_sel_hi:[0,1] neg_lo:[0,0] neg_hi:[0,0]\n" \
  "v_pk_mul_f32 v[44:45], s[4:5], v[44:45] op_sel:[0,0] op_sel_hi:[0,1] neg_lo:[0,0] neg_hi:[0,0]\n" \
  "v_sub_f32 v46, v132, v46\n" \
  "v_mul_f32 v46, s4, v46\n" \
  "v_pk_add_f32 v[48:49], v[134:135], v[48:49] op_sel:[0,0] op_sel_hi:[1,1] neg_lo:[0,1] neg_hi:[0,1]\n" \
  "v_pk_add_f32 v[50:51], v[136:137], v[50:51] op_sel:[0,0] op_sel_hi:[1,1] neg_lo:[0,1] neg_hi:[0,1]\n" \
  "v_pk_add_f32 v[52:53], v[138:139], v[52:53] op_sel:[0,0] op_sel_hi:[1,1] neg_lo:[0,1] neg_hi:[0,1]\n" \
  "v_pk_add_f32 v[54:55], v[140:141], v[54:55] op_sel:[0,0] op_sel_hi:[1,1] neg_lo:[0,1] neg_hi:[0,1]\n" \
  "v_pk_add_f32 v[56:57], v[142:143], v[56:57] op_sel:[0,0] op_sel_hi:[1,1] neg_lo:[0,1] neg_hi:[0,1]\n" \
  "v_pk_add_f32 v[58:59], v[144:145], v[58:59] op_sel:[0,0] op_sel_hi:[1,1] neg_lo:[0,1] neg_hi:[0,1]\n" \
  "v_pk_add_f32 v[60:61], v[146:147], v[60:61] op_sel:[0,0] op_sel_hi:[1,1] neg_lo:[0,1] neg_hi:[0,1]\n" \
  "v_pk_add_f32 v[62:63], v[148:149], v[62:63] op_sel:[0,0] op_sel_hi:[1,1] neg_lo:[0,1] neg_hi:[0,1]\n" \
  "v_pk_add_f32 v[64:65], v[150:151], v[64:65] op_sel:[0,0] op_sel_hi:[1,1] neg_lo:[0,1] neg_hi:[0,1]\n" \
  "v_pk_add_f32 v[66:67], v[152:153], v[66:67] op_sel:[0,0] op_sel_hi:[1,1] neg_lo:[0,1] neg_hi:[0,1]\n" \
  "v_pk_add_f32 v[68:69], v[154:155], v[68:69] op_sel:[0,0] op_sel_hi:[1,1] neg_lo:[0,1] neg_hi:[0,1]\n" \
  "v_pk_add_f32 v[70:71], v[156:157], v[70:71] op_sel:[0,0] op_sel_hi:[1,1] neg_lo:[0,1] neg_hi:[0,1]\n" \
  "v_pk_add_f32 v[72:73], v[158:159], v[72:73] op_sel:[0,0] op_sel_hi:[1,1] neg_lo:[0,1] neg_hi:[0,1]\n" \
  "v_pk_add_f32 v[74:75], v[160:161], v[74:75] op_sel:[0,0] op_sel_hi:[1,1] neg_lo:[0,1] neg_hi:[0,1]\n" \
  "v_pk_add_f32 v[76:77], v[162:163], v[76:77] op_sel:[0,0] op_sel_hi:[1,1] neg_lo:[0,1] neg_hi:[0,1]\n" \
  "v_pk_add_f32 v[78:79], v[164:165], v[78:79] op_sel:[0,0] op_sel_hi:[1,1] neg_lo:[0,1] neg_hi:[0,1]\n" \
  "v_pk_add_f32 v[80:81], v[166:167], v[80:81] op_sel:[0,0] op_sel_hi:[1,1] neg_lo:[0,1] neg_hi:[0,1]\n" \
  "v_pk_add_f32 v[82:83], v[168:169], v[82:83] op_sel:[0,0] op_sel_hi:[1,1] neg_lo:[0,1] neg_hi:[0,1]\n" \
  "v_pk_mul_f32 v[48:49], s[4:5], v[48:49] op_sel:[0,0] op_sel_hi:[0,1] neg_lo:[0,0] neg_hi:[0,0]\n" \
  "v_pk_mul_f32 v[50:51], s[4:5], v[50:51] op_sel:[0,0] op_sel_hi:[0,1] neg_lo:[0,0] neg_hi:[0,0]\n" \
  "v_pk_mul_f32 v[52:53], s[4:5], v[52:53] op_sel:[0,0] op_sel_hi:[0,1] neg_lo:[0,0] neg_hi:[0,0]\n" \
  "v_pk_mul_f32 v[54:55], s[4:5], v[54:55] op_sel:[0,0] op_sel_hi:[0,1] neg_lo:[0,0] neg_hi:[0,0]\n" \
  "v_pk_mul_f32 v[56:57], s[4:5], v[56:57] op_sel:[0,0] op_sel_hi:[0,1] neg_lo:[0,0] neg_hi:[0,0]\n" \
  "v_pk_mul_f32 v[58:59], s[4:5], v[58:59] op_sel:[0,0] op_sel_hi:[0,1] neg_lo:[0,0] neg_hi:[0,0]\n" \
  "v_pk_mul_f32 v[60:61], s[4:5], v[60:61] op_sel:[0,0] op_sel_hi:[0,1] neg_lo:[0,0] neg_hi:[0,0]\n" \
  "v_pk_mul_f32 v[62:63], s[4:5], v[62:63] op_sel:[0,0] op_sel_hi:[0,1] neg_lo:[0,0] neg_hi:[0,0]\n" \
  "v_pk_mul_f32 v[64:65], s[4:5], v[64:65] op_sel:[0,0] op_sel_hi:[0,1] neg_lo:[0,0] neg_hi:[0,0]\n" \
  "v_pk_mul_f32 v[66:67], s[4:5], v[66:67] op_sel:[0,0] op_sel_hi:[0,1] neg_lo:[0,0] neg_hi:[0,0]\n" \
  "v_pk_mul_f32 v[68:69], s[4:5], v[68:69] op_sel:[0,0] op_sel_hi:[0,1] neg_lo:[0,0] neg_hi:[0,0]\n" \
  "v_pk_mul_f32 v[70:71], s[4:5], v[70:71] op_sel:[0,0] op_sel_hi:[0,1] neg_lo:[0,0] neg_hi:[0,0]\n" \
  "v_pk_mul_f32 v[72:73], s[4:5], v[72:73] op_sel:[0,0] op_sel_hi:[0,1] neg_lo:[0,0] neg_hi:[0,0]\n" \
  "v_pk_mul_f32 v[74:75], s[4:5], v[74:75] op_sel:[0,0] op_sel_hi:[0,1] neg_lo:[0,0] neg_hi:[0,0]\n" \
  "v_pk_mul_f32 v[76:77], s[4:5], v[76:77] op_sel:[0,0] op_sel_hi:[0,1] neg_lo:[0,0] neg_hi:[0,0]\n" \
  "v_pk_mul_f32 v[78:79], s[4:5], v[78:79] op_sel:[0,0] op_sel_hi:[0,1] neg_lo:[0,0] neg_hi:[0,0]\n" \
  "v_pk_mul_f32 v[80:81], s[4:5], v[80:81] op_sel:[0,0] op_sel_hi:[0,1] neg_lo:[0,0] neg_hi:[0,0]\n" \
  "v_pk_mul_f32 v[82:83], s[4:5], v[82:83] op_sel:[0,0] op_sel_hi:[0,1] neg_lo:[0,0] neg_hi:[0,0]\n" \
  "30:\n" \
  "s_mul_i32 s4, s10, 9\n" \
  "v_add_u32 v174, s4, v0\n" \
  "global_load_dword v186, v174, s[46:47] nt\n" \
  "v_add_u32 v174, s10, v174\n" \
  "global_load_dword v187, v174, s[46:47] nt\n" \
  "v_add_u32 v174, s10, v174\n" \
  "global_load_dword v185, v174, s[46:47] nt\n" \
  "v_add_u32 v174, s10, v174\n" \
  "global_load_dword v188, v174, s[46:47] nt\n" \
  "v_add_u32 v174, s10, v174\n" \
  "global_load_dword v189, v174, s[46:47] nt\n" \
  "v_add_u32 v174, s10, v174\n" \
  "global_load_dword v190, v174, s[46:47] nt\n" \
  "v_add_u32 v174, s10, v174\n" \
  "global_load_dword v192, v174, s[46:47] nt\n" \
  "v_add_u32 v174, s10, v174\n" \
  "global_load_dword v193, v174, s[46:47] nt\n" \
  "v_add_u32 v174, s10, v174\n" \
  "global_load_dword v191, v174, s[46:47] nt\n" \
  "v_add_u32 v174, s10, v174\n" \
  "global_load_dword v194, v174, s[46:47] nt\n" \
  "v_add_u32 v174, s10, v174\n" \
  "global_load_dword v195, v174, s[46:47] nt\n" \
  "v_add_u32 v174, s10, v174\n" \
  "global_load_dword v196, v174, s[46:47] nt\n" \
  "v_add_u32 v174, s10, v174\n" \
  "global_load_dword v198, v174, s[46:47] nt\n" \
  "v_add_u32 v174, s10, v174\n" \
  "global_load_dword v199, v174, s[46:47] nt\n" \
  "v_add_u32 v174, s10, v174\n" \
  "global_load_dword v197, v174, s[46:47] nt\n" \
  "v_add_u32 v174, s10, v174\n" \
  "global_load_dword v200, v174, s[46:47] nt\n" \
  "v_add_u32 v174, s10, v174\n" \
  "global_load_dword v201, v174, s[46:47] nt\n" \
  "v_add_u32 v174, s10, v174\n" \
  "global_load_dword v202, v174, s[46:47] nt\n" \
  "v_add_u32 v174, s10, v174\n" \
  "global_load_dword v204, v174, s[46:47] nt\n" \
  "v_add_u32 v174, s10, v174\n" \
  "global_load_dword v205, v174, s[46:47] nt\n" \
  "v_add_u32 v174, s10, v174\n" \
  "global_load_dword v203, v174, s[46:47] nt\n" \
  "v_add_u32 v174, s10, v174\n" \
  "global_load_dword v206, v174, s[46:47] nt\n" \
  "v_add_u32 v174, s10, v174\n" \
  "global_load_dword v207, v174, s[46:47] nt\n" \
  "v_add_u32 v174, s10, v174\n" \
  "global_load_dword v214, v174, s[46:47] nt\n" \
  "v_add_u32 v174, s10, v174\n" \
  "global_load_dword v216, v174, s[46:47] nt\n" \
  "v_add_u32 v174, s10, v174\n" \
  "global_load_dword v217, v174, s[46:47] nt\n" \
  "v_add_u32 v174, s10, v174\n" \
  "global_load_dword v215, v174, s[46:47] nt\n" \
  "v_add_u32 v174, s10, v174\n" \
  "global_load_dword v218, v174, s[46:47] nt\n" \
  "v_add_u32 v174, s10, v174\n" \
  "global_load_dword v219, v174, s[46:47] nt\n" \
  "v_add_u32 v174, s10, v174\n" \
  "global_load_dword v220, v174, s[46:47] nt\n" \
  "v_add_u32 v174, s10, v174\n" \
  "global_load_dword v221, v174, s[46:47] nt\n" \
  "v_add_u32 v174, s10, v174\n" \
  "global_load_dword v222, v174, s[46:47] nt\n" \
  "v_add_u32 v174, s10, v174\n" \
  "global_load_dword v223, v174, s[46:47] nt\n" \
  "v_add_u32 v174, s10, v174\n" \
  "global_load_dword v224, v174, s[46:47] nt\n" \
  "v_add_u32 v174, s10, v174\n" \
  "global_load_dword v225, v174, s[46:47] nt\n" \
  "v_add_u32 v174, s10, v174\n" \
  "global_load_dword v226, v174, s[46:47] nt\n" \
  "v_accvgpr_read_b32 v176, a246\n" \
  "v_accvgpr_read_b32 v177, a247\n" \
  "v_accvgpr_read_b32 v178, a248\n" \
  "v_accvgpr_read_b32 v180, a249\n" \
  "v_accvgpr_read_b32 v181, a250\n" \
  "v_accvgpr_read_b32 v179, a251\n" \
  "v_accvgpr_read_b32 v182, a252\n" \
  "v_accvgpr_read_b32 v183, a253\n" \
  "v_accvgpr_read_b32 v184, a254\n" \
  "v_accvgpr_read_b32 v175, a255\n" \
  "s_mul_i32 s4, s10, 0x7b\n" \
  "v_add_u32 v174, s4, v0\n" \
  "global_load_dword v208, v174, s[42:43] nt\n" \
  "v_mov_b32 v227, 0\n" \
  "v_mov_b32 v174, v0\n" \
  "global_store_dword v174, v88, s[42:43] nt\n" \
  "v_add_u32 v174, s10, v174\n" \
  "global_store_dword v174, v89, s[42:43] nt\n" \
  "v_add_u32 v174, s10, v174\n" \
  "global_store_dword v174, v90, s[42:43] nt\n" \
  "v_add_u32 v174, s10, v174\n" \
  "global_store_dword v174, v92, s[42:43] nt\n" \
  "v_add_u32 v174, s10, v174\n" \
  "global_store_dword v174, v93, s[42:43] nt\n" \
  "v_add_u32 v174, s10, v174\n" \
  "global_store_dword v174, v91, s[42:43] nt\n" \
  "v_add_u32 v174, s10, v174\n" \
  "global_store_dword v174, v94, s[42:43] nt\n" \
  "v_add_u32 v174, s10, v174\n" \
  "global_store_dword v174, v95, s[42:43] nt\n" \
  "v_add_u32 v174, s10, v174\n" \
  "global_store_dword v174, v96, s[42:43] nt\n" \
  "v_add_u32 v174, s10, v174\n" \
  "global_store_dword v174, v98, s[42:43] nt\n" \
  "v_add_u32 v174, s10, v174\n" \
  "global_store_dword v174, v99, s[42:43] nt\n" \
  "v_add_u32 v174, s10, v174\n" \
  "global_store_dword v174, v97, s[42:43] nt\n" \
  "v_add_u32 v174, s10, v174\n" \
  "global_store_dword v174, v100, s[42:43] nt\n" \
  "v_add_u32 v174, s10, v174\n" \
  "global_store_dword v174, v101, s[42:43] nt\n" \
  "v_add_u32 v174, s10, v174\n" \
  "global_store_dword v174, v102, s[42:43] nt\n" \
  "v_add_u32 v174, s10, v174\n" \
  "global_store_dword v174, v104, s[42:43] nt\n" \
  "v_add_u32 v174, s10, v174\n" \
  "global_store_dword v174, v105, s[42:43] nt\n" \
  "v_add_u32 v174, s10, v174\n" \
  "global_store_dword v174, v103, s[42:43] nt\n" \
  "v_add_u32 v174, s10, v174\n" \
  "global_store_dword v174, v106, s[42:43] nt\n" \
// ... 193 lines not shown
  "v_add_u32 v174, s10, v174\n" \
  "v_accvgpr_read_b32 v228, a203\n" \
  "global_store_dword v174, v228, s[42:43] nt\n" \
  "v_add_u32 v174, s10, v174\n" \
  "v_accvgpr_read_b32 v229, a204\n" \
  "global_store_dword v174, v229, s[42:43] nt\n" \
  "v_add_u32 v174, s10, v174\n" \
  "v_accvgpr_read_b32 v230, a205\n" \
  "global_store_dword v174, v230, s[42:43] nt\n" \
  "v_add_u32 v174, s10, v174\n" \
  "v_accvgpr_read_b32 v209, a206\n" \
  "global_store_dword v174, v209, s[42:43] nt\n" \
  "v_add_u32 v174, s10, v174\n" \
  "v_accvgpr_read_b32 v228, a207\n" \
  "global_store_dword v174, v228, s[42:43] nt\n" \
  "v_add_u32 v174, s10, v174\n" \
  "v_accvgpr_read_b32 v229, a208\n" \
  "global_store_dword v174, v229, s[42:43] nt\n" \
  "v_add_u32 v174, s10, v174\n" \
  "v_accvgpr_read_b32 v230, a209\n" \
  "global_store_dword v174, v230, s[42:43] nt\n" \
  "v_add_u32 v174, s10, v174\n" \
  "v_accvgpr_read_b32 v209, a210\n" \
  "global_store_dword v174, v209, s[42:43] nt\n" \
  "v_add_u32 v174, s10, v174\n" \
  "v_accvgpr_read_b32 v228, a211\n" \
  "global_store_dword v174, v228, s[42:43] nt\n" \
  "v_add_u32 v174, s10, v174\n" \
  "v_accvgpr_read_b32 v229, a212\n" \
  "global_store_dword v174, v229, s[42:43] nt\n" \
  "v_add_u32 v174, s10, v174\n" \
  "v_accvgpr_read_b32 v230, a213\n" \
  "global_store_dword v174, v230, s[42:43] nt\n" \
  "v_add_u32 v174, s10, v174\n" \
  "v_accvgpr_read_b32 v209, a214\n" \
  "global_store_dword v174, v209, s[42:43] nt\n" \
  "v_add_u32 v174, s10, v174\n" \
  "v_accvgpr_read_b32 v228, a215\n" \
  "global_store_dword v174, v228, s[42:43] nt\n" \
  "v_add_u32 v174, s10, v174\n" \
  "v_accvgpr_read_b32 v229, a216\n" \
  "global_store_dword v174, v229, s[42:43] nt\n" \
  "v_add_u32 v174, s10, v174\n" \
  "v_accvgpr_read_b32 v230, a217\n" \
  "global_store_dword v174, v230, s[42:43] nt\n" \
  "v_add_u32 v174, s10, v174\n" \
  "global_store_dword v174, v210, s[42:43] nt\n" \
  "v_add_u32 v174, s10, v174\n" \
  "global_store_dword v174, v211, s[42:43] nt\n" \
  "v_add_u32 v174, s10, v174\n" \
  "global_store_dword v174, v212, s[42:43] nt\n" \
  "v_add_u32 v174, s10, v174\n" \
  "s_waitcnt vmcnt(0)\n" \
  "v_pk_mul_f32 v[2:3], v[176:177], v[2:3] op_sel:[0,0] op_sel_hi:[1,1] neg_lo:[0,0] neg_hi:[0,0]\n" \
  "v_pk_mul_f32 v[88:89], v[176:177], v[88:89] op_sel:[0,0] op_sel_hi:[1,1] neg_lo:[0,0] neg_hi:[0,0]\n" \
  "v_pk_mul_f32 v[4:5], v[178:179], v[4:5] op_sel:[0,0] op_sel_hi:[1,1] neg_lo:[0,0] neg_hi:[0,0]\n" \
  "v_pk_mul_f32 v[90:91], v[178:179], v[90:91] op_sel:[0,0] op_sel_hi:[1,1] neg_lo:[0,0] neg_hi:[0,0]\n" \
  "v_pk_mul_f32 v[6:7], v[180:181], v[6:7] op_sel:[0,0] op_sel_hi:[1,1] neg_lo:[0,0] neg_hi:[0,0]\n" \
  "v_pk_mul_f32 v[92:93], v[180:181], v[92:93] op_sel:[0,0] op_sel_hi:[1,1] neg_lo:[0,0] neg_hi:[0,0]\n" \
  "v_pk_mul_f32 v[8:9], v[182:183], v[8:9] op_sel:[0,0] op_sel_hi:[1,1] neg_lo:[0,0] neg_hi:[0,0]\n" \
  "v_pk_mul_f32 v[94:95], v[182:183], v[94:95] op_sel:[0,0] op_sel_hi:[1,1] neg_lo:[0,0] neg_hi:[0,0]\n" \
  "v_pk_mul_f32 v[10:11], v[184:185], v[10:11] op_sel:[0,0] op_sel_hi:[1,1] neg_lo:[0,0] neg_hi:[0,0]\n" \
  "v_pk_mul_f32 v[96:97], v[184:185], v[96:97] op_sel:[0,0] op_sel_hi:[1,1] neg_lo:[0,0] neg_hi:[0,0]\n" \
  "v_pk_mul_f32 v[12:13], v[186:187], v[12:13] op_sel:[0,0] op_sel_hi:[1,1] neg_lo:[0,0] neg_hi:[0,0]\n" \
  "v_pk_mul_f32 v[98:99], v[186:187], v[98:99] op_sel:[0,0] op_sel_hi:[1,1] neg_lo:[0,0] neg_hi:[0,0]\n" \
  "v_pk_mul_f32 v[14:15], v[188:189], v[14:15] op_sel:[0,0] op_sel_hi:[1,1] neg_lo:[0,0] neg_hi:[0,0]\n" \
  "v_pk_mul_f32 v[100:101], v[188:189], v[100:101] op_sel:[0,0] op_sel_hi:[1,1] neg_lo:[0,0] neg_hi:[0,0]\n" \
  "v_pk_mul_f32 v[16:17], v[190:191], v[16:17] op_sel:[0,0] op_sel_hi:[1,1] neg_lo:[0,0] neg_hi:[0,0]\n" \
  "v_pk_mul_f32 v[102:103], v[190:191], v[102:103] op_sel:[0,0] op_sel_hi:[1,1] neg_lo:[0,0] neg_hi:[0,0]\n" \
  "v_pk_mul_f32 v[18:19], v[192:193], v[18:19] op_sel:[0,0] op_sel_hi:[1,1] neg_lo:[0,0] neg_hi:[0,0]\n" \
  "v_pk_mul_f32 v[104:105], v[192:193], v[104:105] op_sel:[0,0] op_sel_hi:[1,1] neg_lo:[0,0] neg_hi:[0,0]\n" \
  "v_pk_mul_f32 v[20:21], v[194:195], v[20:21] op_sel:[0,0] op_sel_hi:[1,1] neg_lo:[0,0] neg_hi:[0,0]\n" \
  "v_pk_mul_f32 v[106:107], v[194:195], v[106:107] op_sel:[0,0] op_sel_hi:[1,1] neg_lo:[0,0] neg_hi:[0,0]\n" \
  "v_pk_mul_f32 v[22:23], v[196:197], v[22:23] op_sel:[0,0] op_sel_hi:[1,1] neg_lo:[0,0] neg_hi:[0,0]\n" \
  "v_pk_mul_f32 v[108:109], v[196:197], v[108:109] op_sel:[0,0] op_sel_hi:[1,1] neg_lo:[0,0] neg_hi:[0,0]\n" \
  "v_pk_mul_f32 v[24:25], v[198:199], v[24:25] op_sel:[0,0] op_sel_hi:[1,1] neg_lo:[0,0] neg_hi:[0,0]\n" \
  "v_pk_mul_f32 v[110:111], v[198:199], v[110:111] op_sel:[0,0] op_sel_hi:[1,1] neg_lo:[0,0] neg_hi:[0,0]\n" \
  "v_pk_mul_f32 v[26:27], v[200:201], v[26:27] op_sel:[0,0] op_sel_hi:[1,1] neg_lo:[0,0] neg_hi:[0,0]\n" \
  "v_pk_mul_f32 v[112:113], v[200:201], v[112:113] op_sel:[0,0] op_sel_hi:[1,1] neg_lo:[0,0] neg_hi:[0,0]\n" \
  "v_pk_mul_f32 v[28:29], v[202:203], v[28:29] op_sel:[0,0] op_sel_hi:[1,1] neg_lo:[0,0] neg_hi:[0,0]\n" \
  "v_pk_mul_f32 v[114:115], v[202:203], v[114:115] op_sel:[0,0] op_sel_hi:[1,1] neg_lo:[0,0] neg_hi:[0,0]\n" \
  "v_pk_mul_f32 v[30:31], v[204:205], v[30:31] op_sel:[0,0] op_sel_hi:[1,1] neg_lo:[0,0] neg_hi:[0,0]\n" \
  "v_pk_mul_f32 v[116:117], v[204:205], v[116:117] op_sel:[0,0] op_sel_hi:[1,1] neg_lo:[0,0] neg_hi:[0,0]\n" \
  "v_pk_mul_f32 v[32:33], v[206:207], v[32:33] op_sel:[0,0] op_sel_hi:[1,1] neg_lo:[0,0] neg_hi:[0,0]\n" \
  "v_pk_mul_f32 v[118:119], v[206:207], v[118:119] op_sel:[0,0] op_sel_hi:[1,1] neg_lo:[0,0] neg_hi:[0,0]\n" \
  "v_pk_mul_f32 v[34:35], v[214:215], v[34:35] op_sel:[0,0] op_sel_hi:[1,1] neg_lo:[0,0] neg_hi:[0,0]\n" \
  "v_pk_mul_f32 v[120:121], v[214:215], v[120:121] op_sel:[0,0] op_sel_hi:[1,1] neg_lo:[0,0] neg_hi:[0,0]\n" \
  "v_pk_mul_f32 v[36:37], v[216:217], v[36:37] op_sel:[0,0] op_sel_hi:[1,1] neg_lo:[0,0] neg_hi:[0,0]\n" \
  "v_pk_mul_f32 v[122:123], v[216:217], v[122:123] op_sel:[0,0] op_sel_hi:[1,1] neg_lo:[0,0] neg_hi:[0,0]\n" \
  "v_pk_mul_f32 v[38:39], v[218:219], v[38:39] op_sel:[0,0] op_sel_hi:[1,1] neg_lo:[0,0] neg_hi:[0,0]\n" \
  "v_pk_mul_f32 v[124:125], v[218:219], v[124:125] op_sel:[0,0] op_sel_hi:[1,1] neg_lo:[0,0] neg_hi:[0,0]\n" \
  "v_pk_mul_f32 v[40:41], v[220:221], v[40:41] op_sel:[0,0] op_sel_hi:[1,1] neg_lo:[0,0] neg_hi:[0,0]\n" \
  "v_pk_mul_f32 v[126:127], v[220:221], v[126:127] op_sel:[0,0] op_sel_hi:[1,1] neg_lo:[0,0] neg_hi:[0,0]\n" \
  "v_pk_mul_f32 v[42:43], v[222:223], v[42:43] op_sel:[0,0] op_sel_hi:[1,1] neg_lo:[0,0] neg_hi:[0,0]\n" \
  "v_pk_mul_f32 v[128:129], v[222:223], v[128:129] op_sel:[0,0] op_sel_hi:[1,1] neg_lo:[0,0] neg_hi:[0,0]\n" \
  "v_pk_mul_f32 v[44:45], v[224:225], v[44:45] op_sel:[0,0] op_sel_hi:[1,1] neg_lo:[0,0] neg_hi:[0,0]\n" \
  "v_pk_mul_f32 v[130:131], v[224:225], v[130:131] op_sel:[0,0] op_sel_hi:[1,1] neg_lo:[0,0] neg_hi:[0,0]\n" \
  "v_pk_mul_f32 v[46:47], v[226:227], v[46:47] op_sel:[0,0] op_sel_hi:[1,1] neg_lo:[0,0] neg_hi:[0,0]\n" \
  "v_pk_mul_f32 v[132:133], v[226:227], v[132:133] op_sel:[0,0] op_sel_hi:[1,1] neg_lo:[0,0] neg_hi:[0,0]\n" \
  "s_mul_i32 s4, s10, 45\n" \
  "v_add_u32 v174, s4, v0\n" \
  "global_load_dword v176, v174, s[46:47] nt\n" \
  "v_add_u32 v174, s10, v174\n" \
  "global_load_dword v177, v174, s[46:47] nt\n" \
  "v_add_u32 v174, s10, v174\n" \
  "global_load_dword v178, v174, s[46:47] nt\n" \
  "v_add_u32 v174, s10, v174\n" \
  "global_load_dword v180, v174, s[46:47] nt\n" \
  "v_add_u32 v174, s10, v174\n" \
  "global_load_dword v181, v174, s[46:47] nt\n" \
  "v_add_u32 v174, s10, v174\n" \
  "global_load_dword v179, v174, s[46:47] nt\n" \
  "v_add_u32 v174, s10, v174\n" \
  "global_load_dword v182, v174, s[46:47] nt\n" \
  "v_add_u32 v174, s10, v174\n" \
  "global_load_dword v183, v174, s[46:47] nt\n" \
  "v_add_u32 v174, s10, v174\n" \
  "global_load_dword v184, v174, s[46:47] nt\n" \
  "v_add_u32 v174, s10, v174\n" \
  "global_load_dword v186, v174, s[46:47] nt\n" \
  "v_add_u32 v174, s10, v174\n" \
  "global_load_dword v187, v174, s[46:47] nt\n" \
  "v_add_u32 v174, s10, v174\n" \
  "global_load_dword v185, v174, s[46:47] nt\n" \
  "v_add_u32 v174, s10, v174\n" \
  "global_load_dword v188, v174, s[46:47] nt\n" \
  "v_add_u32 v174, s10, v174\n" \
  "global_load_dword v189, v174, s[46:47] nt\n" \
  "v_add_u32 v174, s10, v174\n" \
  "global_load_dword v190, v174, s[46:47] nt\n" \
  "v_add_u32 v174, s10, v174\n" \
  "global_load_dword v192, v174, s[46:47] nt\n" \
  "v_add_u32 v174, s10, v174\n" \
  "global_load_dword v193, v174, s[46:47] nt\n" \
  "v_add_u32 v174, s10, v174\n" \
  "global_load_dword v191, v174, s[46:47] nt\n" \
  "v_add_u32 v174, s10, v174\n" \
  "global_load_dword v194, v174, s[46:47] nt\n" \
  "v_add_u32 v174, s10, v174\n" \
  "global_load_dword v195, v174, s[46:47] nt\n" \
  "v_add_u32 v174, s10, v174\n" \
  "global_load_dword v196, v174, s[46:47] nt\n" \
  "v_add_u32 v174, s10, v174\n" \
  "global_load_dword v198, v174, s[46:47] nt\n" \
  "v_add_u32 v174, s10, v174\n" \
  "global_load_dword v199, v174, s[46:47] nt\n" \
  "v_add_u32 v174, s10, v174\n" \
  "global_load_dword v197, v174, s[46:47] nt\n" \
  "v_add_u32 v174, s10, v174\n" \
  "global_load_dword v200, v174, s[46:47] nt\n" \
  "v_add_u32 v174, s10, v174\n" \
  "global_load_dword v201, v174, s[46:47] nt\n" \
  "v_add_u32 v174, s10, v174\n" \
  "global_load_dword v202, v174, s[46:47] nt\n" \
  "v_add_u32 v174, s10, v174\n" \
  "global_load_dword v204, v174, s[46:47] nt\n" \
  "v_add_u32 v174, s10, v174\n" \
  "global_load_dword v205, v174, s[46:47] nt\n" \
  "v_add_u32 v174, s10, v174\n" \
  "global_load_dword v203, v174, s[46:47] nt\n" \
  "v_add_u32 v174, s10, v174\n" \
  "global_load_dword v206, v174, s[46:47] nt\n" \
  "v_add_u32 v174, s10, v174\n" \
  "global_load_dword v207, v174, s[46:47] nt\n" \
  "v_add_u32 v174, s10, v174\n" \
  "global_load_dword v214, v174, s[46:47] nt\n" \
  "v_add_u32 v174, s10, v174\n" \
  "global_load_dword v216, v174, s[46:47] nt\n" \
  "v_add_u32 v174, s10, v174\n" \
  "global_load_dword v217, v174, s[46:47] nt\n" \
  "v_add_u32 v174, s10, v174\n" \
  "global_load_dword v215, v174, s[46:47] nt\n" \
  "v_add_u32 v174, s10, v174\n" \
  "global_load_dword v218, v174, s[46:47] nt\n" \
  "v_add_u32 v174, s10, v174\n" \
  "global_load_dword v219, v174, s[46:47] nt\n" \
  "v_add_u32 v174, s10, v174\n" \
  "global_load_dword v220, v174, s[46:47] nt\n" \
  "v_mov_b32 v174, v0\n" \
  "global_load_dword v209, v174, s[40:41] nt\n" \
  "v_add_u32 v174, s10, v174\n" \
  "global_load_dword v222, v174, s[40:41] nt\n" \
  "v_add_u32 v174, s10, v174\n" \
  "global_load_dword v223, v174, s[40:41] nt\n" \
  "v_add_u32 v174, s10, v174\n" \
  "global_load_dword v224, v174, s[40:41] nt\n" \
  "v_add_u32 v174, s10, v174\n" \
  "global_load_dword v225, v174, s[40:41] nt\n" \
  "v_add_u32 v174, s10, v174\n" \
  "global_load_dword v226, v174, s[40:41] nt\n" \
  "v_add_u32 v174, s10, v174\n" \
  "global_load_dword v227, v174, s[40:41] nt\n" \
  "v_add_u32 v174, s10, v174\n" \
  "global_load_dword v228, v174, s[40:41] nt\n" \
  "v_add_u32 v174, s10, v174\n" \
  "global_load_dword v229, v174, s[40:41] nt\n" \
  "v_add_u32 v174, s10, v174\n" \
  "global_load_dword v230, v174, s[40:41] nt\n" \
  "v_add_u32 v174, s10, v174\n" \
  "global_load_dword v231, v174, s[40:41] nt\n" \
  "v_add_u32 v174, s10, v174\n" \
  "global_load_dword v232, v174, s[40:41] nt\n" \
  "v_add_u32 v174, s10, v174\n" \
  "global_load_dword v233, v174, s[40:41] nt\n" \
  "v_add_u32 v174, s10, v174\n" \
  "global_load_dword v234, v174, s[40:41] nt\n" \
  "v_add_u32 v174, s10, v174\n" \
  "global_load_dword v235, v174, s[40:41] nt\n" \
  "v_add_u32 v174, s10, v174\n" \
  "global_load_dword v236, v174, s[40:41] nt\n" \
  "v_add_u32 v174, s10, v174\n" \
  "global_load_dword v237, v174, s[40:41] nt\n" \
  "v_add_u32 v174, s10, v174\n" \
  "global_load_dword v238, v174, s[40:41] nt\n" \
  "v_mov_b32 v174, v0\n" \
  "global_load_dword v239, v174, s[44:45] nt\n" \
  "v_add_u32 v174, s10, v174\n" \
  "global_load_dword v240, v174, s[44:45] nt\n" \
  "v_add_u32 v174, s10, v174\n" \
  "global_load_dword v241, v174, s[44:45] nt\n" \
  "v_add_u32 v174, s10, v174\n" \
  "global_load_dword v242, v174, s[44:45] nt\n" \
  "v_add_u32 v174, s10, v174\n" \
  "global_load_dword v243, v174, s[44:45] nt\n" \
  "v_add_u32 v174, s10, v174\n" \
  "global_load_dword v244, v174, s[44:45] nt\n" \
  "v_add_u32 v174, s10, v174\n" \
  "global_load_dword v245, v174, s[44:45] nt\n" \
  "v_add_u32 v174, s10, v174\n" \
  "global_load_dword v246, v174, s[44:45] nt\n" \
  "v_add_u32 v174, s10, v174\n" \
  "global_load_dword v247, v174, s[44:45] nt\n" \
  "v_mov_b32 v221, 1.0\n" \
  "s_cmp_eq_u64 s[0:1], 0\n" \
  "s_cbranch_scc1 31f\n" \
  "s_lshl_b32 s4, s12, 5\n" \
  "s_load_dwordx2 s[30:31], s[0:1], s4 offset:0\n" \
  "s_load_dwordx4 s[32:35], s[0:1], s4 offset:8\n" \
  "s_load_dwordx2 s[36:37], s[0:1], s4 offset:24\n" \
  "s_waitcnt vmcnt(0) lgkmcnt(0)\n" \
  "v_add_f32 v239, s30, v239\n" \
  "v_mov_b32 v242, s33\n" \
  "v_add_f32 v240, s31, v240\n" \
  "v_mov_b32 v243, s34\n" \
  "v_add_f32 v241, s32, v241\n" \
  "v_mov_b32 v244, s35\n" \
  "v_mov_b32 v245, s36\n" \
  "v_mov_b32 v246, 0\n" \
  "v_mov_b32 v247, s37\n" \
  "31:\n" \
  "v_rcp_f32 v248, v175\n" \
  "s_nop 0\n" \
  "v_fma_f32 v249, -v175, v248, 1.0\n" \
  "v_fma_f32 v248, v249, v248, v248\n" \
  "s_cmp_eq_u64 s[56:57], 0\n" \
  "s_cbranch_scc1 32f\n" \
  "v_mov_b32 v174, v0\n" \
  "global_load_dword v175, v174, s[56:57]\n" \
  "v_add_u32 v174, s10, v174\n" \
  "global_load_dword v250, v174, s[56:57]\n" \
  "s_waitcnt vmcnt(0)\n" \
  "v_mov_b32 v251, v175\n" \
  "v_rcp_f32 v175, v251\n" \
  "s_nop 0\n" \
  "v_fma_f32 v249, -v251, v175, 1.0\n" \
  "v_fma_f32 v175, v249, v175, v175\n" \
  "v_mov_b32 v251, v250\n" \
  "v_rcp_f32 v250, v251\n" \
  "s_nop 0\n" \
  "v_fma_f32 v249, -v251, v250, 1.0\n" \
  "v_fma_f32 v250, v249, v250, v250\n" \
  "s_branch 33f\n" \
  "32:\n" \
  "v_mov_b32 v175, s86\n" \
  "v_mov_b32 v250, s87\n" \
  "33:\n" \
  "s_waitcnt vmcnt(0)\n" \
  "v_pk_mul_f32 v[48:49], v[176:177], v[48:49] op_sel:[0,0] op_sel_hi:[1,1] neg_lo:[0,0] neg_hi:[0,0]\n" \
  "v_pk_mul_f32 v[134:135], v[176:177], v[134:135] op_sel:[0,0] op_sel_hi:[1,1] neg_lo:[0,0] neg_hi:[0,0]\n" \
  "v_pk_mul_f32 v[50:51], v[178:179], v[50:51] op_sel:[0,0] op_sel_hi:[1,1] neg_lo:[0,0] neg_hi:[0,0]\n" \
  "v_pk_mul_f32 v[136:137], v[178:179], v[136:137] op_sel:[0,0] op_sel_hi:[1,1] neg_lo:[0,0] neg_hi:[0,0]\n" \
  "v_pk_mul_f32 v[52:53], v[180:181], v[52:53] op_sel:[0,0] op_sel_hi:[1,1] neg_lo:[0,0] neg_hi:[0,0]\n" \
  "v_pk_mul_f32 v[138:139], v[180:181], v[138:139] op_sel:[0,0] op_sel_hi:[1,1] neg_lo:[0,0] neg_hi:[0,0]\n" \
  "v_pk_mul_f32 v[54:55], v[182:183], v[54:55] op_sel:[0,0] op_sel_hi:[1,1] neg_lo:[0,0] neg_hi:[0,0]\n" \
  "v_pk_mul_f32 v[140:141], v[182:183], v[140:141] op_sel:[0,0] op_sel_hi:[1,1] neg_lo:[0,0] neg_hi:[0,0]\n" \
  "v_pk_mul_f32 v[56:57], v[184:185], v[56:57] op_sel:[0,0] op_sel_hi:[1,1] neg_lo:[0,0] neg_hi:[0,0]\n" \
  "v_pk_mul_f32 v[142:143], v[184:185], v[142:143] op_sel:[0,0] op_sel_hi:[1,1] neg_lo:[0,0] neg_hi:[0,0]\n" \
  "v_pk_mul_f32 v[58:59], v[186:187], v[58:59] op_sel:[0,0] op_sel_hi:[1,1] neg_lo:[0,0] neg_hi:[0,0]\n" \
  "v_pk_mul_f32 v[144:145], v[186:187], v[144:145] op_sel:[0,0] op_sel_hi:[1,1] neg_lo:[0,0] neg_hi:[0,0]\n" \
  "v_pk_mul_f32 v[60:61], v[188:189], v[60:61] op_sel:[0,0] op_sel_hi:[1,1] neg_lo:[0,0] neg_hi:[0,0]\n" \
  "v_pk_mul_f32 v[146:147], v[188:189], v[146:147] op_sel:[0,0] op_sel_hi:[1,1] neg_lo:[0,0] neg_hi:[0,0]\n" \
  "v_pk_mul_f32 v[62:63], v[190:191], v[62:63] op_sel:[0,0] op_sel_hi:[1,1] neg_lo:[0,0] neg_hi:[0,0]\n" \
  "v_pk_mul_f32 v[148:149], v[190:191], v[148:149] op_sel:[0,0] op_sel_hi:[1,1] neg_lo:[0,0] neg_hi:[0,0]\n" \
  "v_pk_mul_f32 v[64:65], v[192:193], v[64:65] op_sel:[0,0] op_sel_hi:[1,1] neg_lo:[0,0] neg_hi:[0,0]\n" \
  "v_pk_mul_f32 v[150:151], v[192:193], v[150:151] op_sel:[0,0] op_sel_hi:[1,1] neg_lo:[0,0] neg_hi:[0,0]\n" \
  "v_pk_mul_f32 v[66:67], v[194:195], v[66:67] op_sel:[0,0] op_sel_hi:[1,1] neg_lo:[0,0] neg_hi:[0,0]\n" \
  "v_pk_mul_f32 v[152:153], v[194:195], v[152:153] op_sel:[0,0] op_sel_hi:[1,1] neg_lo:[0,0] neg_hi:[0,0]\n" \
  "v_pk_mul_f32 v[68:69], v[196:197], v[68:69] op_sel:[0,0] op_sel_hi:[1,1] neg_lo:[0,0] neg_hi:[0,0]\n" \
  "v_pk_mul_f32 v[154:155], v[196:197], v[154:155] op_sel:[0,0] op_sel_hi:[1,1] neg_lo:[0,0] neg_hi:[0,0]\n" \
  "v_pk_mul_f32 v[70:71], v[198:199], v[70:71] op_sel:[0,0] op_sel_hi:[1,1] neg_lo:[0,0] neg_hi:[0,0]\n" \
  "v_pk_mul_f32 v[156:157], v[198:199], v[156:157] op_sel:[0,0] op_sel_hi:[1,1] neg_lo:[0,0] neg_hi:[0,0]\n" \
  "v_pk_mul_f32 v[72:73], v[200:201], v[72:73] op_sel:[0,0] op_sel_hi:[1,1] neg_lo:[0,0] neg_hi:[0,0]\n" \
  "v_pk_mul_f32 v[158:159], v[200:201], v[158:159] op_sel:[0,0] op_sel_hi:[1,1] neg_lo:[0,0] neg_hi:[0,0]\n" \
  "v_pk_mul_f32 v[74:75], v[202:203], v[74:75] op_sel:[0,0] op_sel_hi:[1,1] neg_lo:[0,0] neg_hi:[0,0]\n" \
  "v_pk_mul_f32 v[160:161], v[202:203], v[160:161] op_sel:[0,0] op_sel_hi:[1,1] neg_lo:[0,0] neg_hi:[0,0]\n" \
  "v_pk_mul_f32 v[76:77], v[204:205], v[76:77] op_sel:[0,0] op_sel_hi:[1,1] neg_lo:[0,0] neg_hi:[0,0]\n" \
  "v_pk_mul_f32 v[162:163], v[204:205], v[162:163] op_sel:[0,0] op_sel_hi:[1,1] neg_lo:[0,0] neg_hi:[0,0]\n" \
  "v_pk_mul_f32 v[78:79], v[206:207], v[78:79] op_sel:[0,0] op_sel_hi:[1,1] neg_lo:[0,0] neg_hi:[0,0]\n" \
  "v_pk_mul_f32 v[164:165], v[206:207], v[164:165] op_sel:[0,0] op_sel_hi:[1,1] neg_lo:[0,0] neg_hi:[0,0]\n" \
  "v_pk_mul_f32 v[80:81], v[214:215], v[80:81] op_sel:[0,0] op_sel_hi:[1,1] neg_lo:[0,0] neg_hi:[0,0]\n" \
  "v_pk_mul_f32 v[166:167], v[214:215], v[166:167] op_sel:[0,0] op_sel_hi:[1,1] neg_lo:[0,0] neg_hi:[0,0]\n" \
  "v_pk_mul_f32 v[82:83], v[216:217], v[82:83] op_sel:[0,0] op_sel_hi:[1,1] neg_lo:[0,0] neg_hi:[0,0]\n" \
  "v_pk_mul_f32 v[168:169], v[216:217], v[168:169] op_sel:[0,0] op_sel_hi:[1,1] neg_lo:[0,0] neg_hi:[0,0]\n" \
  "v_pk_mul_f32 v[84:85], v[218:219], v[84:85] op_sel:[0,0] op_sel_hi:[1,1] neg_lo:[0,0] neg_hi:[0,0]\n" \
  "v_pk_mul_f32 v[170:171], v[218:219], v[170:171] op_sel:[0,0] op_sel_hi:[1,1] neg_lo:[0,0] neg_hi:[0,0]\n" \
  "v_pk_mul_f32 v[86:87], v[220:221], v[86:87] op_sel:[0,0] op_sel_hi:[1,1] neg_lo:[0,0] neg_hi:[0,0]\n" \
  "v_pk_mul_f32 v[172:173], v[220:221], v[172:173] op_sel:[0,0] op_sel_hi:[1,1] neg_lo:[0,0] neg_hi:[0,0]\n" \
  "v_pk_mul_f32 v[134:135], v[134:135], v[248:249] op_sel:[0,0] op_sel_hi:[1,0] neg_lo:[0,0] neg_hi:[0,0]\n" \
  "v_pk_mul_f32 v[136:137], v[136:137], v[248:249] op_sel:[0,0] op_sel_hi:[1,0] neg_lo:[0,0] neg_hi:[0,0]\n" \
  "v_pk_mul_f32 v[138:139], v[138:139], v[248:249] op_sel:[0,0] op_sel_hi:[1,0] neg_lo:[0,0] neg_hi:[0,0]\n" \
  "v_pk_mul_f32 v[140:141], v[140:141], v[248:249] op_sel:[0,0] op_sel_hi:[1,0] neg_lo:[0,0] neg_hi:[0,0]\n" \
  "v_pk_mul_f32 v[142:143], v[142:143], v[248:249] op_sel:[0,0] op_sel_hi:[1,0] neg_lo:[0,0] neg_hi:[0,0]\n" \
  "v_pk_mul_f32 v[144:145], v[144:145], v[248:249] op_sel:[0,0] op_sel_hi:[1,0] neg_lo:[0,0] neg_hi:[0,0]\n" \
  "v_pk_mul_f32 v[146:147], v[146:147], v[248:249] op_sel:[0,0] op_sel_hi:[1,0] neg_lo:[0,0] neg_hi:[0,0]\n" \
  "v_pk_mul_f32 v[148:149], v[148:149], v[248:249] op_sel:[0,0] op_sel_hi:[1,0] neg_lo:[0,0] neg_hi:[0,0]\n" \
  "v_pk_mul_f32 v[150:151], v[150:151], v[248:249] op_sel:[0,0] op_sel_hi:[1,0] neg_lo:[0,0] neg_hi:[0,0]\n" \
  "v_pk_mul_f32 v[152:153], v[152:153], v[248:249] op_sel:[0,0] op_sel_hi:[1,0] neg_lo:[0,0] neg_hi:[0,0]\n" \
  "v_pk_mul_f32 v[154:155], v[154:155], v[248:249] op_sel:[0,0] op_sel_hi:[1,0] neg_lo:[0,0] neg_hi:[0,0]\n" \
  "v_pk_mul_f32 v[156:157], v[156:157], v[248:249] op_sel:[0,0] op_sel_hi:[1,0] neg_lo:[0,0] neg_hi:[0,0]\n" \
  "v_pk_mul_f32 v[158:159], v[158:159], v[248:249] op_sel:[0,0] op_sel_hi:[1,0] neg_lo:[0,0] neg_hi:[0,0]\n" \
// ... 2963 lines not shown
```

### robobee3d_amd/isasim.py

```python
import functools
import re
from fractions import Fraction

import numpy as np

f32, f64, u32, u64 = np.float32, np.float64, np.uint32, np.uint64
POISON = 0x7ff8dead
VCC = 106
LANE_LDS_VGPR = 1


class AddressFault(Exception):
    """A simulated global access outside every array handed to the interpreter (on the GPU: a memory access fault)."""


class Quad:

    def __init__(self, v=(), a=(), lds=(), dead_v=(), dead_a=(), dead_lds=()):
        self.v, self.a, self.lds = list(v), list(a), list(lds)
        self.dead_v, self.dead_a, self.dead_lds = list(dead_v), list(dead_a), list(dead_lds)


_REG = re.compile(r"([vas])(\d+)$|([vas])\[(\d+):(\d+)\]$")

# ... 34 lines not shown
        return frozenset({(mm.group(1), int(mm.group(2)))})
    return frozenset((mm.group(3), r) for r in range(int(mm.group(4)), int(mm.group(5)) + 1))


def _srcs(t, k):
    x, d = t[k], t[-1]
    if isinstance(x, dict):
        return frozenset()
    if not isinstance(d, dict) or k < 2:
        return _regs(x)
    kind, lo = _decode(x)[:2]
    q = k - 2
    sels = (d["op_sel"][q],) if t[0] == "v_pk_mov_b32" else (d["op_sel"][q], d["op_sel_hi"][q])
    return frozenset((kind, lo + h) for h in sels)


def _fmax(a, b):
    return np.where(b != b, a, np.where(a != a, b, np.where(b > a, b, a)))


def _fmin(a, b):
    return np.where(b != b, a, np.where(a != a, b, np.where(b < a, b, a)))


def _imm(t, k):
    for x in t[k:]:
        if isinstance(x, int):
            return x
        if isinstance(x, str) and x.startswith("offset:"):
            return int(x[7:])
    return 0


_CMP = {"lt": np.less, "le": np.less_equal, "gt": np.greater, "ge": np.greater_equal, "eq": np.equal,
        "nlt": lambda a, b: ~(a < b), "neq": lambda a, b: ~(a == b), "ne": np.not_equal, "u": lambda a, b: (a != a) | (b != b)}
_WAITABLE = ("ds_read", "global_load", "s_load")
_T1_READ = ("ds_write", "ds_min", "global_store", "s_cmp", "s_cbranch", "s_branch", "v_fmac")


class Machine:
    def __init__(self, ins, lanes=1, regions=(), sgpr=None, vgpr=None, lds=None, max_exec=3000000, quad=None, log=None,
                 V=None, A=None):
        self.ins, self.lanes = ins, lanes
        self.V = np.full((lanes, 256), POISON, u32) if V is None else V
        self.A = np.full((lanes, 256), POISON, u32) if A is None else A
        self.S = [0] * 128
        for r, val in (sgpr or {}).items():
            self.S[r] = val & 0xFFFFFFFF
        if V is None:
            for r, val in (vgpr or {}).items():
                self.V[:, r] = val
            self.V[:, LANE_LDS_VGPR] = 16 * np.arange(lanes)
        self.lds = np.zeros((1, 0), u32) if lds is None else lds
        self.regions = [(b, st, arr, arr.view(u32).reshape(-1), arr.itemsize) for b, st, arr in regions]
        self.set_exec(np.ones(lanes, bool))
        self.scc = 0
        self.max_exec, self.quad, self.log = max_exec, quad or {}, log
        self.nexec = 0
        self.sections = {}
        self.hits = None
        self.pend = {"vmcnt": [], "lgkmcnt": []}
        self.labels = {}
        for k, t in enumerate(ins):
            if t[0] == "label":
                self.labels.setdefault(t[1], []).append(k)
        self._use, self._rw = {}, {}
        self.dead = set()
        self.src_word, self.src_phase, self.phase = {}, {}, 0

    def set_exec(self, bits):
        self.exec, self.full, self.any = bits, bool(bits.all()), bool(bits.any())

    def mask64(self, bits):
        return sum(1 << ln for ln in range(self.lanes) if bits[ln])

    def lanes_of(self, m):
        return np.array([(m >> ln) & 1 for ln in range(self.lanes)], bool)

    def s32(self, x):
        k, lo = _decode(x)[:2]
        return lo & 0xFFFFFFFF if k == "i" else self.S[lo]

    def s64(self, x):
        k, lo = _decode(x)[:2]
        if k == "i":
            return lo & 0xFFFFFFFFFFFFFFFF
        if k == "exec":
            return self.mask64(self.exec)
        return self.S[lo] | (self.S[lo + 1] << 32)

    def set64(self, x, val):
        k, lo = _decode(x)[:2]
        if k == "exec":
            self.set_exec(self.lanes_of(val))
        else:
            self.S[lo], self.S[lo + 1] = val & 0xFFFFFFFF, (val >> 32) & 0xFFFFFFFF

    def bits(self, x, dpp=None):
        k, lo, _, neg, ab = _decode(x)
        if k == "f":
            b = np.full(self.lanes, np.array(lo, f32).view(u32), u32)
        elif k == "i":
            b = np.full(self.lanes, lo & 0xFFFFFFFF, u32)
        elif k == "s":
            b = np.full(self.lanes, self.S[lo], u32)
        else:
            b = (self.V if k == "v" else self.A)[:, lo].copy()
# ... 2 lines not shown
                for ln in range(self.lanes):
                    if self.exec[ln] and not self.exec[qp[ln]]:
                        raise AssertionError("DPP read of a masked-off lane: %r" % (dpp,))
                b = b[qp]
        if ab:
            b = b & u32(0x7FFFFFFF)
        return b ^ u32(0x80000000) if neg else b

    def f(self, x, dpp=None):
        return self.bits(x, dpp).view(f32)

    def d(self, x):
        k, lo, _, neg, ab = _decode(x)
        if k == "f":
            val = np.full(self.lanes, lo, f64)
        else:
            if k == "s":
                b = np.full(self.lanes, self.S[lo] | (self.S[lo + 1] << 32), u64)
            else:
                R = self.V if k == "v" else self.A
                b = R[:, lo].astype(u64) | (R[:, lo + 1].astype(u64) << u64(32))
            val = b.view(f64)
        if ab:
            val = np.abs(val)
        return -val if neg else val

    def write(self, x, b, lo_off=0):
        k, lo = _decode(x)[:2]
        R = self.V if k == "v" else self.A
        if self.full:
            R[:, lo + lo_off] = b
        else:
            R[self.exec, lo + lo_off] = np.asarray(b, u32)[self.exec]

    def wf(self, x, val):
        self.write(x, np.asarray(val, f32).view(u32))

    def wd(self, x, val):
        b = np.asarray(val, f64).view(u64)
        self.write(x, (b & u64(0xFFFFFFFF)).astype(u32))
        self.write(x, (b >> u64(32)).astype(u32), 1)

    def wmask(self, x, cond):
        self.set64(x, self.mask64(cond & self.exec))

    def half(self, x, sel):
        k, lo = _decode(x)[:2]
        if k == "v":
            return self.V[:, lo + sel].view(f32).astype(f64)
        return np.full(self.lanes, np.array(self.S[lo + sel], u32).view(f32), f64)

    def gaddr(self, sbase, voff, imm, ln, n):
        addr = (self.s64(sbase) + (int(self.V[ln, _decode(voff)[1]]) if voff is not None else 0) + imm) & 0xFFFFFFFFFFFFFFFF
        for base, stride, arr, words, size in self.regions:
            if base <= addr < base + len(arr) * stride:
                i, b = divmod(addr - base, stride)
                if b % 4 == 0 and b + 4 * n <= size * (len(arr) - i if stride == size else 1):
                    return words, (i * size + b) // 4
        raise AddressFault("%r touches 0x%016x, outside every array of the call" % (self.ins[self.pc], addr))

    def lds_word(self, base, off, ln):
        byte = int(self.V[ln, _decode(base)[1]]) + off
        w = (byte // 1024) * 4 + (byte % 16) // 4
        if w >= self.lds.shape[1]:
            raise AddressFault("%r touches LDS byte 0x%x, outside the lane's slice" % (self.ins[self.pc], byte))
        return ln, w

    def active(self):
        return [ln for ln in range(self.lanes) if self.exec[ln]]

    def uses(self, pc):
        u = self._use.get(pc)
        if u is None:
            t = self.ins[pc]
            u = self._use[pc] = set().union(*[_regs(x) for x in t[1:] if not isinstance(x, dict)])
        return u

    def wait(self, t):
        for part in " ".join(str(x) for x in t[1:]).split():
            name, val = part[:-1].split("(")
            del self.pend[name][:max(0, len(self.pend[name]) - int(val))]

    def track(self, pc, m):
        used = self.uses(pc)
        for q in self.pend.values():
            for dst in q:
                assert not (dst & used), ("register used before its load was waited for", pc, self.ins[pc], sorted(dst & used))
        if m.startswith(_WAITABLE):
            (self.pend["vmcnt"] if m.startswith("global") else self.pend["lgkmcnt"]).append(_regs(self.ins[pc][1]))
        elif m.startswith("ds_"):
            self.pend["lgkmcnt"].append(set())
        elif m.startswith("global_"):
            self.pend["vmcnt"].append(set())
        if self.dead:
            rw = self._rw.get(pc)
            if rw is None:
                t = self.ins[pc]
                dst = frozenset() if m.startswith(_T1_READ) else _regs(t[1])
                rw = self._rw[pc] = (set().union(*[_srcs(t, k) for k in range(2 if dst else 1, len(t))]), dst)
            assert not (rw[0] & self.dead), ("register read after its kill", pc, self.ins[pc], sorted(rw[0] & self.dead))
            self.dead -= rw[1]
        if self.log is not None:
            self.log_reads(pc, m, used)

    def log_reads(self, pc, m, used):
        if m.startswith("ds_read"):
            return
        t = self.ins[pc]
        wr_only = _regs(t[1]) if m in ("global_load_dword", "v_mov_b32", "v_accvgpr_read_b32") else set()
        for r in wr_only:
            self.src_word.pop(r, None)
# ... 297 lines not shown
    for ln in mc.active():
        sl, w = mc.lds_word(base, t[3], ln)
        if read:
            mc.V[ln, lo:lo + n] = mc.lds[sl, w:w + n]
        elif m == "ds_min_f32":
            cur, val = mc.lds[sl, w:w + 1].view(f32)[0], mc.V[ln, lo:lo + 1].view(f32)[0]
            mc.lds[sl, w] = np.array(val if val < cur else cur, f32).view(u32)
        else:
            mc.lds[sl, w:w + n] = mc.V[ln, lo:lo + n]
    if mc.log is not None:
        sl, w = mc.lds_word(base, t[3], mc.active()[0])
        if read:
            for h in range(n):
                mc.src_word[("v", lo + h)], mc.src_phase[("v", lo + h)] = w + h, mc.phase
        else:
            mc.log["a" if m == "ds_min_f32" else "w"].update(range(w, w + n))


def _global(mc, t):
    m = t[0]
    n = {"dword": 1, "dwordx2": 2, "dwordx4": 4}[m.rsplit("_", 1)[1]]
    load = m.startswith("global_load")
    voff, reg = (t[2], t[1]) if load else (t[1], t[2])
    k, lo = _decode(reg)[:2]
    R = mc.V if k == "v" else mc.A
    for ln in mc.active():
        words, w0 = mc.gaddr(t[3], voff, _imm(t, 4), ln, n)
        if load:
            R[ln, lo:lo + n] = words[w0:w0 + n]
        else:
            words[w0:w0 + n] = R[ln, lo:lo + n]


def _readfirstlane(mc, t):
    act = mc.active()
    mc.S[_decode(t[1])[1]] = int(mc.bits(t[2])[act[0] if act else 0])


def _bitop(op):
    return lambda mc, t: mc.write(t[1], op(mc.bits(t[2]).astype(u64), mc.bits(t[3]).astype(u64)).astype(u32))


VECTOR = {
    "v_mov_b32": lambda mc, t: mc.write(t[1], mc.bits(t[2])),
    "v_mov_b32_dpp": lambda mc, t: mc.write(t[1], mc.bits(t[2], t[3])),
    "v_accvgpr_read_b32": lambda mc, t: mc.write(t[1], mc.bits(t[2])),
    "v_accvgpr_write_b32": lambda mc, t: mc.write(t[1], mc.bits(t[2])),
    "v_readfirstlane_b32": _readfirstlane,
    "v_pk_mov_b32": _pk_mov,
    "v_add_u32": _bitop(lambda a, b: (a + b) & u64(0xFFFFFFFF)),
    "v_and_b32": _bitop(lambda a, b: a & b),
    "v_or_b32": _bitop(lambda a, b: a | b),
    "v_lshrrev_b32": _bitop(lambda a, b: b >> (a & u64(31))),
    "v_mul_u32_u24": _bitop(lambda a, b: ((a & u64(0xFFFFFF)) * (b & u64(0xFFFFFF))) & u64(0xFFFFFFFF)),
    "v_bfe_u32": lambda mc, t: mc.write(t[1], (mc.bits(t[2]) >> u32(t[3] & 31)) & u32((1 << t[4]) - 1)),
    "v_cvt_f32_i32": lambda mc, t: mc.wf(t[1], mc.bits(t[2]).view(np.int32).astype(f32)),
    "v_fma_f32": _f32op(_fma32),
    "v_fmac_f32": _fmac(),
    "v_fmac_f32_dpp": _fmac(True),
    "v_fmaak_f32": lambda mc, t: mc.wf(t[1], _fma32(mc.f(t[2]), mc.f(t[3]), mc.f(t[4]))),
    "v_mul_f32": _f32op(lambda a, b: a * b),
    "v_mul_f32_dpp": _f32op(lambda a, b: a * b, True),
    "v_add_f32": _f32op(lambda a, b: a + b),
    "v_add_f32_dpp": _f32op(lambda a, b: a + b, True),
    "v_sub_f32": _f32op(lambda a, b: a - b),
    "v_subrev_f32": _f32op(lambda a, b: b - a),
    "v_max_f32": _f32op(_fmax),
    "v_max_f32_dpp": _f32op(_fmax, True),
    "v_min_f32": _f32op(_fmin),
    "v_max3_f32": _f32op(_nanless(np.fmax)),
    "v_min3_f32": _f32op(_nanless(np.fmin)),
    "v_med3_f32": _f32op(lambda a, b, c: np.sort(np.stack([a, b, c]), 0)[1]),
    "v_rcp_f32": _f32op(lambda a: f32(1.0) / a),
    "v_rsq_f32": _f32op(lambda a: (1.0 / np.sqrt(a.astype(f64))).astype(f32)),
    "v_sqrt_f32": _f32op(lambda a: np.sqrt(a.astype(f64)).astype(f32)),
    "v_pk_fma_f32": _pk("fma"),
    "v_pk_mul_f32": _pk("mul"),
    "v_pk_add_f32": _pk("add"),
    "v_cndmask_b32": _cndmask,
    "v_cndmask_b32_e64": _cndmask,
    "v_fma_f64": _f64op(_fma64),
    "v_mul_f64": _f64op(lambda a, b: a * b),
    "v_add_f64": _f64op(lambda a, b: a + b),
    "v_max_f64": _f64op(_fmax),
    "v_min_f64": _f64op(_fmin),
    "v_rcp_f64": _f64op(lambda a: 1.0 / a),
    "v_rsq_f64": _f64op(lambda a: 1.0 / np.sqrt(a)),
    "v_cmp_nlt_f64": _cmp("f64"),
    "v_cmp_eq_i32_e64": _cmp("int"),
    "v_cmp_ne_u32": _cmp("int"),
}
for _op in ("lt", "le", "gt", "ge", "eq", "nlt", "neq", "u"):
    VECTOR["v_cmp_%s_f32" % _op] = VECTOR["v_cmp_%s_f32_e64" % _op] = _cmp("f32")
OPS = dict(SALU, **VECTOR)
for _m in ("ds_read_b32", "ds_read_b64", "ds_read_b128", "ds_write_b32", "ds_write_b64", "ds_write_b128", "ds_min_f32",
           "global_load_dword", "global_load_dwordx2", "global_load_dwordx4", "global_store_dword", "global_store_dwordx2"):
    OPS[_m] = _ds if _m.startswith("ds_") else _global
```

Before: 545.8 million.

## Use dwordx4 stores and loads for parked Ruiz scaling vectors in workspace

Instead of storing and reloading each Ruiz scaling entry (D and E) as a separate strided dword in the workspace, a contiguous block of entries is written and read per lane as 16-byte dwordx4 cells. This cuts the number of global memory instructions and address increments in the factor and reload phases. Because the original slot order is permuted, extra v_mov sequences un-rotate the loaded values. The workspace layout changes for those entries, and the simulator gains cell-addressing support to model it.

```diff
diff --git a/robobee3d_amd/asmstep.py b/robobee3d_amd/asmstep.py
--- a/robobee3d_amd/asmstep.py
+++ b/robobee3d_amd/asmstep.py
@@ -61,6 +61,8 @@
 XV_N, XV_B = 2, 254
 NT_PTRS = ("state", "ctrl", "ref", "out", "stats")
 A_SPARE, N_SPARE_D = 246, 9
+PARK_D0, PARK_D1 = 12, 44
+PARK_E1 = 36
 
 
 class Pool:
@@ -244,7 +246,7 @@
 
 
 class StepGen:
-    def __init__(self, N=3, perm=None, quad=False, exact_ruiz=False):
+    def __init__(self, N=3, perm=None, quad=False, exact_ruiz=False, narrow_roundtrip=False):
         self.st = Struct(N, perm)
         self.s = self.st.s
         self.e = Emit()
@@ -255,7 +257,13 @@
         self.speculate = not quad and not exact_ruiz
         self.ruiz_span = self.restart_at = None
         self.nt = () if quad else ("nt",)
+        self.wide = not quad and not narrow_roundtrip
+        self.park_at = None
+        self.marks = []
         self.homes = asmgen.Homes(NRING, 0 if quad else XV_N, XV_B)
+
+    def mark(self, name):
+        self.marks.append((name, len(self.e.ins)))
 
     def label(self):
         self.lab += 1
@@ -290,6 +298,16 @@
 
     def adv(self, voff):
         self.e("v_add_u32", v(voff), sg(S_INT["stride"]), v(voff))
+
+    def cells_ptr(self, voff, first_row):
+        e = self.e
+        e("s_mul_i32", sg(S_TMP), sg(S_INT["stride"]), first_row)
+        e("v_lshlrev_b32", v(voff), 2, "v0")
+        e("v_add_u32", v(voff), sg(S_TMP), v(voff))
+        e("s_lshl_b32", sg(S_TMP), sg(S_INT["stride"]), 2)
+
+    def cells_adv(self, voff):
+        self.e("v_add_u32", v(voff), sg(S_TMP), v(voff))
 
     def advance_ptr(self, ptr, sstep):
         e, lo = self.e, S_PTR[ptr]
@@ -582,8 +600,11 @@
         pool.free(*RF)
         pool.free(*WV.values())
         pool.free_range(LS, 20)
+        self.mark("ruiz")
         self.ruiz_quad() if self.quad else self.ruiz()
+        self.mark("recover")
         self.recover_and_bounds()
+        self.mark("factor")
         self.factor()
 
     def maxabs(self, dst, regs, acc_in=False):
@@ -942,20 +963,39 @@
         self.rcp_nr(cinv, cs, t)
         voff = pool.get()
         npark = 0 if self.quad else N_SPARE_D
+        wide = self.wide
+        self.park_at = len(e.ins)
         self.rows_ptr(voff, npark)
+        if wide:
+            assert npark <= PARK_D0 <= PARK_D1 <= nx and PARK_D0 % 4 == 0 and (PARK_D1 - PARK_D0) % 4 == 0 and PARK_E1 % 4 == 0
+            DB = pool.getn(8)
+            assert self.VE % 2 == 0
+            RE = lambda i: self.VE + i
         rows_of_col = {}
         for i in range(nc):
             rows_of_col.setdefault(st.unit[i][1], []).append(i)
         IWV = {n: pool.get() for n in WNAMES}
         for k, n in enumerate(WNAMES):
             e("v_accvgpr_read_b32", v(IWV[n]), "a%d" % (A_IW + k))
+        dsingle = d
         for j in range(nx):
+            grouped = wide and PARK_D0 <= j < PARK_D1
+            d = DB + (j - PARK_D0) % 8 if grouped else dsingle
             e("v_mul_f32", v(d), v(RP(j)), v(cinv))
             e("v_mul_f32", v(d), v(IWV[st.weight_of(j)]), v(d))
             e("v_sqrt_f32", v(d), v(d))
             e("s_nop", 0)
             if j < npark:
                 e("v_accvgpr_write_b32", "a%d" % (A_SPARE + j), v(d))
+            elif grouped:
+                if j == PARK_D0:
+                    self.cells_ptr(voff, PARK_D0)
+                if (j - PARK_D0) % 4 == 3:
+                    e("global_store_dwordx4", v(voff), "v[%d:%d]" % (d - 3, d), sp(S_PTR["ws"]), *self.nt)
+                    if j + 1 < PARK_D1:
+                        self.cells_adv(voff)
+                    else:
+                        self.rows_ptr(voff, PARK_D1)
             else:
                 e("global_store_dword", v(voff), v(d), sp(S_PTR["ws"]), *self.nt)
                 self.adv(voff)
@@ -965,7 +1005,16 @@
                 for i in rows_of_col[j]:
                     e("v_mul_f32", v(RE(i)), "|%s|" % v(RA(st.unit[i][0])), v(r))
         assert asmgen.WS_ES == asmgen.WS_DS + nx and asmgen.WS_C == asmgen.WS_ES + nc
-        for i in range(nc):
+        d = dsingle
+        if wide:
+            pool.free_range(DB, 8)
+            self.cells_ptr(voff, nx)
+            for i in range(0, PARK_E1, 4):
+                e("global_store_dwordx4", v(voff), "v[%d:%d]" % (RE(i), RE(i) + 3), sp(S_PTR["ws"]), *self.nt)
+                if i + 4 < PARK_E1:
+                    self.cells_adv(voff)
+            self.rows_ptr(voff, nx + PARK_E1)
+        for i in range(PARK_E1 if wide else 0, nc):
             e("global_store_dword", v(voff), v(RE(i)), sp(S_PTR["ws"]), *self.nt)
             self.adv(voff)
         if npark:
@@ -1132,6 +1181,7 @@
             asmquad.section(e, asmquad.QuadPlan(st), self.label)
             e("label", lab6)
         else:
+            self.mark("loop")
             self._admm_rest(plan, zk)
         for i in range(st.neq):
             pool.free(V_Z + st.zs[i], kill=True)
@@ -1193,7 +1243,28 @@
         DR = lambda j: DS(st.xs[j])
         cr, T0 = g_(), g_()
         npark = 0 if self.quad else N_SPARE_D
-        self.load_rows("ws", npark, [DR(j) for j in range(npark, nx)], voff)
+        def unrotate(reg, slots, lo, hi):
+            ks = [k for k in range(0, hi - 2, 3) if [slots[k], slots[k + 1], slots[k + 2]] != [k, k + 1, k + 2] and k + 2 >= lo]
+            assert all(lo <= k and [slots[k], slots[k + 1], slots[k + 2]] == [k + 1, k + 2, k] for k in ks)
+            ts = [g_() for _ in range(min(len(ks), len(pool.free_), 3))]
+            for lo_ in range(0, len(ks), len(ts)):
+                for step in range(4):
+                    for k, t in zip(ks[lo_:lo_ + len(ts)], ts):
+                        dst, src = [(t, reg(k + 2)), (reg(k + 2), reg(k + 1)), (reg(k + 1), reg(k)), (reg(k), t)][step]
+                        e("v_mov_b32", v(dst), v(src))
+            pool.free(*ts)
+        if self.wide:
+            assert [st.xs[j] for j in range(PARK_D0 - 3, PARK_D0)] == [PARK_D0 - 2, PARK_D0 - 1, PARK_D0 - 3] and st.xs[44] == 44
+            self.load_rows("ws", npark, [DR(j) for j in range(npark, PARK_D0)], voff)
+            self.cells_ptr(voff, PARK_D0)
+            for j in range(PARK_D0, PARK_D1, 4):
+                assert DS(j) % 2 == 0 and DS(j + 3) == DS(j) + 3
+                e("global_load_dwordx4", "v[%d:%d]" % (DS(j), DS(j) + 3), v(voff), sp(S_PTR["ws"]), *self.nt)
+                if j + 4 < PARK_D1:
+                    self.cells_adv(voff)
+            self.load_rows("ws", PARK_D1, [DR(j) for j in range(PARK_D1, nx)], voff)
+        else:
+            self.load_rows("ws", npark, [DR(j) for j in range(npark, nx)], voff)
         if npark:
             for j in range(npark):
                 e("v_accvgpr_read_b32", v(DR(j)), "a%d" % (A_SPARE + j))
@@ -1220,6 +1291,8 @@
             self.adv(voff)
         pool.free(*zt)
         e("s_waitcnt", "vmcnt(0)")
+        if self.wide:
+            unrotate(DS, st.xs, PARK_D0, PARK_D1)
         for k in range(0, nx + 1, 2):
             pk(e, "v_pk_mul_f32", V_W + k, [P2(DS(k)), P2(V_W + k)])
             pk(e, "v_pk_mul_f32", V_X + k, [P2(DS(k)), P2(V_X + k)])
@@ -1229,7 +1302,16 @@
         ER = lambda i: ES(st.zs[i])
         ST = [g_() for _ in range(18)]
         RF = [g_() for _ in range(9)]
-        self.load_rows("ws", asmgen.WS_ES - asmgen.WS_DS, [ER(i) for i in range(nc)], voff)
+        if self.wide:
+            self.cells_ptr(voff, nx)
+            for i in range(0, PARK_E1, 4):
+                assert ES(i) % 2 == 0 and ES(i + 3) == ES(i) + 3
+                e("global_load_dwordx4", "v[%d:%d]" % (ES(i), ES(i) + 3), v(voff), sp(S_PTR["ws"]), *self.nt)
+                if i + 4 < PARK_E1:
+                    self.cells_adv(voff)
+            self.load_rows("ws", nx + PARK_E1, [ER(i) for i in range(PARK_E1, nc)], voff)
+        else:
+            self.load_rows("ws", asmgen.WS_ES - asmgen.WS_DS, [ER(i) for i in range(nc)], voff)
         self.load_rows("state", 0, ST, voff)
         self.load_rows("ref", 0, RF, voff)
         e("v_mov_b32", v(ES(nc)), 1.0)
@@ -1264,6 +1346,8 @@
         e("v_mov_b32", v(ibi1), SF("Ibi1"))
         e("label", lab_ib2)
         e("s_waitcnt", "vmcnt(0)")
+        if self.wide:
+            unrotate(ES, st.zs, 0, PARK_E1)
         for k in range(0, nc + 1, 2):
             pk(e, "v_pk_mul_f32", V_WZ + k, [P2(ES(k)), P2(V_WZ + k)])
             pk(e, "v_pk_mul_f32", V_Y + k, [P2(ES(k)), P2(V_Y + k)])
@@ -1575,6 +1659,7 @@
         self.wl_step(OUT, R0, T0n, voff)
         self.store_rows("ctrl", nx + 2 * nc, [T0n], voff)
         pool.free(T0n)
+        self.mark("plant")
         self.plant(ST, OUT, voff)
         pool.free(*OUT, *ST, voff)
         assert len(pool.free_) == VEND - VFIRST, "phase C leaked registers: %s" % sorted(set(range(VFIRST, VEND)) - pool.free_)
@@ -2010,9 +2095,13 @@
             e("s_mov_b32", sg(S_EXACT), 0)
             self.lab_restart = self.label_spec()
             e("label", self.lab_restart)
+        self.mark("assemble")
         self.phase_a()
+        self.mark("first iteration")
         self.admm()
+        self.mark("phase C")
         self.phase_c()
+        self.mark("step end")
         e("s_load_dword", sg(S_TMP), sp(S_PBLK), OFF["refstep"])
         e("s_load_dwordx4", "s[%d:%d]" % (S_HIST, S_HIST + 3), sp(S_PBLK), HIST_OFF)
         e("s_waitcnt", "lgkmcnt(0)")
@@ -2039,6 +2128,10 @@
         e("s_waitcnt", "vmcnt(0)")
         self.pool.free(a, b)
         e("label", lab)
+        if self.restart_at is not None:
+            early = [t for t in e.ins[:self.restart_at] if t[0].startswith("global_store")]
+            assert len(early) == 1 and early[0][3] == sp(S_PTR["ctrl"]) and early[0][0] == "global_store_dword", early
+            assert self.park_at > self.restart_at
         return e.ins
 
 
@@ -2108,7 +2201,7 @@
 PBASE = 0x00007E0080000000
 
 
-def simulate(ins, arrays, ints, floats, max_exec=3000000, ptr_xform=None, lanes=1, hits=False):
+def simulate(ins, arrays, ints, floats, max_exec=3000000, ptr_xform=None, lanes=1, hits=False, exec_mask=None):
     import numpy as np
     from . import isasim
     base_of = {n: 0x00007F0080000000 + (k << 36) for k, n in enumerate(PTRS + ["impulse"])}
@@ -2130,7 +2223,7 @@
     struct.pack_into("<Q", blob, OFF["imp"], ptr_xform(base_of["impulse"]) if arrays.get("impulse") is not None else 0)
     struct.pack_into("<i", blob, OFF["impstep"], int(allints["impstep"]))
     regions = [(PBASE, 4, np.frombuffer(bytes(blob), np.uint32))] + \
-        [(base_of[n], 4 if n in FLAT or lanes > 1 else STRIDE, arrays[n].reshape(-1))
+        [(base_of[n], 4 if n in FLAT or lanes > 1 else STRIDE, arrays[n].reshape(-1)) + ((16,) if n == "ws" and lanes == 1 else ())
          for n in PTRS + ["impulse"] if arrays.get(n) is not None]
     assert all(arrays[n].flags.c_contiguous for n in PTRS + ["impulse"] if arrays.get(n) is not None)
     m = isasim.Machine(ins, lanes, regions=regions, sgpr={S_PARAM: PBASE & 0xFFFFFFFF, S_PARAM + 1: PBASE >> 32},
@@ -2138,6 +2231,8 @@
                        quad=_quad() if lanes == 1 else None)
     if hits:
         m.hits = np.zeros(len(ins), np.int64)
+    if exec_mask is not None:
+        m.set_exec(np.asarray(exec_mask, bool))
     isasim.run(m)
     simulate.last_hits = m.hits
     simulate.last_quad_sections = {("admm" if k is None else k): n for k, n in m.sections.items()}
diff --git a/robobee3d_amd/csrc/umpc_step_asm.h b/robobee3d_amd/csrc/umpc_step_asm.h
--- a/robobee3d_amd/csrc/umpc_step_asm.h
+++ b/robobee3d_amd/csrc/umpc_step_asm.h
@@ -2005,16 +2005,16 @@
   "v_fma_f32 v43, v44, v43, v43\n" \
   "s_mul_i32 s4, s10, 9\n" \
   "v_add_u32 v47, s4, v0\n" \
-  "v_accvgpr_read_b32 v48, a238\n" \
-  "v_accvgpr_read_b32 v49, a239\n" \
-  "v_accvgpr_read_b32 v50, a240\n" \
-  "v_accvgpr_read_b32 v51, a241\n" \
-  "v_accvgpr_read_b32 v52, a242\n" \
-  "v_accvgpr_read_b32 v53, a243\n" \
-  "v_accvgpr_read_b32 v54, a244\n" \
-  "v_accvgpr_read_b32 v55, a245\n" \
+  "v_accvgpr_read_b32 v56, a238\n" \
+  "v_accvgpr_read_b32 v57, a239\n" \
+  "v_accvgpr_read_b32 v58, a240\n" \
+  "v_accvgpr_read_b32 v59, a241\n" \
+  "v_accvgpr_read_b32 v60, a242\n" \
+  "v_accvgpr_read_b32 v61, a243\n" \
+  "v_accvgpr_read_b32 v62, a244\n" \
+  "v_accvgpr_read_b32 v63, a245\n" \
   "v_mul_f32 v45, v70, v43\n" \
-  "v_mul_f32 v45, v48, v45\n" \
+  "v_mul_f32 v45, v56, v45\n" \
   "v_sqrt_f32 v45, v45\n" \
   "s_nop 0\n" \
   "v_accvgpr_write_b32 a246, v45\n" \
@@ -2023,7 +2023,7 @@
   "v_mul_f32 v2, |v116|, v46\n" \
   "v_mul_f32 v8, |v118|, v46\n" \
   "v_mul_f32 v45, v71, v43\n" \
-  "v_mul_f32 v45, v48, v45\n" \
+  "v_mul_f32 v45, v56, v45\n" \
   "v_sqrt_f32 v45, v45\n" \
   "s_nop 0\n" \
   "v_accvgpr_write_b32 a247, v45\n" \
@@ -2032,7 +2032,7 @@
   "v_mul_f32 v3, |v117|, v46\n" \
   "v_mul_f32 v9, |v119|, v46\n" \
   "v_mul_f32 v45, v72, v43\n" \
-  "v_mul_f32 v45, v48, v45\n" \
+  "v_mul_f32 v45, v56, v45\n" \
   "v_sqrt_f32 v45, v45\n" \
   "s_nop 0\n" \
   "v_accvgpr_write_b32 a248, v45\n" \
@@ -2041,34 +2041,34 @@
   "v_mul_f32 v4, |v120|, v46\n" \
   "v_mul_f32 v10, |v122|, v46\n" \
   "v_mul_f32 v45, v74, v43\n" \
-  "v_mul_f32 v45, v50, v45\n" \
+  "v_mul_f32 v45, v58, v45\n" \
   "v_sqrt_f32 v45, v45\n" \
   "s_nop 0\n" \
   "v_accvgpr_write_b32 a249, v45\n" \
   "v_rcp_f32 v46, v45\n" \
   "s_nop 0\n" \
-  "v_mul_f32 v6, |v124|, v46\n" \
-  "v_mul_f32 v12, |v126|, v46\n" \
+  "v_mul_f32 v5, |v124|, v46\n" \
+  "v_mul_f32 v11, |v126|, v46\n" \
   "v_mul_f32 v45, v75, v43\n" \
-  "v_mul_f32 v45, v50, v45\n" \
+  "v_mul_f32 v45, v58, v45\n" \
   "v_sqrt_f32 v45, v45\n" \
   "s_nop 0\n" \
   "v_accvgpr_write_b32 a250, v45\n" \
   "v_rcp_f32 v46, v45\n" \
   "s_nop 0\n" \
-  "v_mul_f32 v7, |v125|, v46\n" \
-  "v_mul_f32 v13, |v127|, v46\n" \
+  "v_mul_f32 v6, |v125|, v46\n" \
+  "v_mul_f32 v12, |v127|, v46\n" \
   "v_mul_f32 v45, v73, v43\n" \
-  "v_mul_f32 v45, v50, v45\n" \
+  "v_mul_f32 v45, v58, v45\n" \
   "v_sqrt_f32 v45, v45\n" \
   "s_nop 0\n" \
   "v_accvgpr_write_b32 a251, v45\n" \
   "v_rcp_f32 v46, v45\n" \
   "s_nop 0\n" \
-  "v_mul_f32 v5, |v121|, v46\n" \
-  "v_mul_f32 v11, |v123|, v46\n" \
+  "v_mul_f32 v7, |v121|, v46\n" \
+  "v_mul_f32 v13, |v123|, v46\n" \
   "v_mul_f32 v45, v76, v43\n" \
-  "v_mul_f32 v45, v48, v45\n" \
+  "v_mul_f32 v45, v56, v45\n" \
   "v_sqrt_f32 v45, v45\n" \
   "s_nop 0\n" \
   "v_accvgpr_write_b32 a252, v45\n" \
@@ -2076,7 +2076,7 @@
   "s_nop 0\n" \
   "v_mul_f32 v14, |v132|, v46\n" \
   "v_mul_f32 v45, v77, v43\n" \
-  "v_mul_f32 v45, v48, v45\n" \
+  "v_mul_f32 v45, v56, v45\n" \
   "v_sqrt_f32 v45, v45\n" \
   "s_nop 0\n" \
   "v_accvgpr_write_b32 a253, v45\n" \
@@ -2084,7 +2084,7 @@
   "s_nop 0\n" \
   "v_mul_f32 v15, |v133|, v46\n" \
   "v_mul_f32 v45, v78, v43\n" \
-  "v_mul_f32 v45, v48, v45\n" \
+  "v_mul_f32 v45, v56, v45\n" \
   "v_sqrt_f32 v45, v45\n" \
   "s_nop 0\n" \
   "v_accvgpr_write_b32 a254, v45\n" \
@@ -2092,353 +2092,261 @@
   "s_nop 0\n" \
   "v_mul_f32 v16, |v136|, v46\n" \
   "v_mul_f32 v45, v80, v43\n" \
-  "v_mul_f32 v45, v50, v45\n" \
+  "v_mul_f32 v45, v58, v45\n" \
   "v_sqrt_f32 v45, v45\n" \
   "s_nop 0\n" \
   "global_store_dword v47, v45, s[46:47] nt\n" \
   "v_add_u32 v47, s10, v47\n" \
   "v_rcp_f32 v46, v45\n" \
   "s_nop 0\n" \
-  "v_mul_f32 v18, |v140|, v46\n" \
+  "v_mul_f32 v17, |v140|, v46\n" \
   "v_mul_f32 v45, v81, v43\n" \
-  "v_mul_f32 v45, v50, v45\n" \
+  "v_mul_f32 v45, v58, v45\n" \
   "v_sqrt_f32 v45, v45\n" \
   "s_nop 0\n" \
   "global_store_dword v47, v45, s[46:47] nt\n" \
   "v_add_u32 v47, s10, v47\n" \
   "v_rcp_f32 v46, v45\n" \
   "s_nop 0\n" \
-  "v_mul_f32 v19, |v141|, v46\n" \
+  "v_mul_f32 v18, |v141|, v46\n" \
   "v_mul_f32 v45, v79, v43\n" \
-  "v_mul_f32 v45, v50, v45\n" \
+  "v_mul_f32 v45, v58, v45\n" \
   "v_sqrt_f32 v45, v45\n" \
   "s_nop 0\n" \
   "global_store_dword v47, v45, s[46:47] nt\n" \
   "v_add_u32 v47, s10, v47\n" \
   "v_rcp_f32 v46, v45\n" \
   "s_nop 0\n" \
-  "v_mul_f32 v17, |v137|, v46\n" \
-  "v_mul_f32 v45, v82, v43\n" \
-  "v_mul_f32 v45, v49, v45\n" \
+  "v_mul_f32 v19, |v137|, v46\n" \
+  "v_mul_f32 v48, v82, v43\n" \
+  "v_mul_f32 v48, v57, v48\n" \
+  "v_sqrt_f32 v48, v48\n" \
+  "s_nop 0\n" \
+  "s_mul_i32 s4, s10, 12\n" \
+  "v_lshlrev_b32 v47, 2, v0\n" \
+  "v_add_u32 v47, s4, v47\n" \
+  "s_lshl_b32 s4, s10, 2\n" \
+  "v_mul_f32 v49, v83, v43\n" \
+  "v_mul_f32 v49, v57, v49\n" \
+  "v_sqrt_f32 v49, v49\n" \
+  "s_nop 0\n" \
+  "v_mul_f32 v50, v84, v43\n" \
+  "v_mul_f32 v50, v57, v50\n" \
+  "v_sqrt_f32 v50, v50\n" \
+  "s_nop 0\n" \
+  "v_mul_f32 v51, v86, v43\n" \
+  "v_mul_f32 v51, v58, v51\n" \
+  "v_sqrt_f32 v51, v51\n" \
+  "s_nop 0\n" \
+  "global_store_dwordx4 v47, v[48:51], s[46:47] nt\n" \
+  "v_add_u32 v47, s4, v47\n" \
+  "v_mul_f32 v52, v87, v43\n" \
+  "v_mul_f32 v52, v58, v52\n" \
+  "v_sqrt_f32 v52, v52\n" \
+  "s_nop 0\n" \
+  "v_mul_f32 v53, v85, v43\n" \
+  "v_mul_f32 v53, v58, v53\n" \
+  "v_sqrt_f32 v53, v53\n" \
+  "s_nop 0\n" \
+  "v_mul_f32 v54, v88, v43\n" \
+  "v_mul_f32 v54, v59, v54\n" \
+  "v_sqrt_f32 v54, v54\n" \
+  "s_nop 0\n" \
+  "v_rcp_f32 v46, v54\n" \
+  "s_nop 0\n" \
+  "v_mul_f32 v20, |v150|, v46\n" \
+  "v_mul_f32 v26, |v152|, v46\n" \
+  "v_mul_f32 v55, v89, v43\n" \
+  "v_mul_f32 v55, v59, v55\n" \
+  "v_sqrt_f32 v55, v55\n" \
+  "s_nop 0\n" \
+  "global_store_dwordx4 v47, v[52:55], s[46:47] nt\n" \
+  "v_add_u32 v47, s4, v47\n" \
+  "v_rcp_f32 v46, v55\n" \
+  "s_nop 0\n" \
+  "v_mul_f32 v21, |v151|, v46\n" \
+  "v_mul_f32 v27, |v153|, v46\n" \
+  "v_mul_f32 v48, v90, v43\n" \
+  "v_mul_f32 v48, v59, v48\n" \
+  "v_sqrt_f32 v48, v48\n" \
+  "s_nop 0\n" \
+  "v_rcp_f32 v46, v48\n" \
+  "s_nop 0\n" \
+  "v_mul_f32 v22, |v156|, v46\n" \
+  "v_mul_f32 v28, |v158|, v46\n" \
+  "v_mul_f32 v49, v92, v43\n" \
+  "v_mul_f32 v49, v61, v49\n" \
+  "v_sqrt_f32 v49, v49\n" \
+  "s_nop 0\n" \
+  "v_rcp_f32 v46, v49\n" \
+  "s_nop 0\n" \
+  "v_mul_f32 v23, |v162|, v46\n" \
+  "v_mul_f32 v29, |v164|, v46\n" \
+  "v_mul_f32 v50, v93, v43\n" \
+  "v_mul_f32 v50, v61, v50\n" \
+  "v_sqrt_f32 v50, v50\n" \
+  "s_nop 0\n" \
+  "v_rcp_f32 v46, v50\n" \
+  "s_nop 0\n" \
+  "v_mul_f32 v24, |v163|, v46\n" \
+  "v_mul_f32 v30, |v165|, v46\n" \
+  "v_mul_f32 v51, v91, v43\n" \
+  "v_mul_f32 v51, v61, v51\n" \
+  "v_sqrt_f32 v51, v51\n" \
+  "s_nop 0\n" \
+  "global_store_dwordx4 v47, v[48:51], s[46:47] nt\n" \
+  "v_add_u32 v47, s4, v47\n" \
+  "v_rcp_f32 v46, v51\n" \
+  "s_nop 0\n" \
+  "v_mul_f32 v25, |v157|, v46\n" \
+  "v_mul_f32 v31, |v159|, v46\n" \
+  "v_mul_f32 v52, v94, v43\n" \
+  "v_mul_f32 v52, v59, v52\n" \
+  "v_sqrt_f32 v52, v52\n" \
+  "s_nop 0\n" \
+  "v_rcp_f32 v46, v52\n" \
+  "s_nop 0\n" \
+  "v_mul_f32 v32, |v170|, v46\n" \
+  "v_mul_f32 v53, v95, v43\n" \
+  "v_mul_f32 v53, v59, v53\n" \
+  "v_sqrt_f32 v53, v53\n" \
+  "s_nop 0\n" \
+  "v_rcp_f32 v46, v53\n" \
+  "s_nop 0\n" \
+  "v_mul_f32 v33, |v171|, v46\n" \
+  "v_mul_f32 v54, v96, v43\n" \
+  "v_mul_f32 v54, v59, v54\n" \
+  "v_sqrt_f32 v54, v54\n" \
+  "s_nop 0\n" \
+  "v_rcp_f32 v46, v54\n" \
+  "s_nop 0\n" \
+  "v_mul_f32 v34, |v176|, v46\n" \
+  "v_mul_f32 v55, v98, v43\n" \
+  "v_mul_f32 v55, v61, v55\n" \
+  "v_sqrt_f32 v55, v55\n" \
+  "s_nop 0\n" \
+  "global_store_dwordx4 v47, v[52:55], s[46:47] nt\n" \
+  "v_add_u32 v47, s4, v47\n" \
+  "v_rcp_f32 v46, v55\n" \
+  "s_nop 0\n" \
+  "v_mul_f32 v35, |v182|, v46\n" \
+  "v_mul_f32 v48, v99, v43\n" \
+  "v_mul_f32 v48, v61, v48\n" \
+  "v_sqrt_f32 v48, v48\n" \
+  "s_nop 0\n" \
+  "v_rcp_f32 v46, v48\n" \
+  "s_nop 0\n" \
+  "v_mul_f32 v36, |v183|, v46\n" \
+  "v_mul_f32 v49, v97, v43\n" \
+  "v_mul_f32 v49, v61, v49\n" \
+  "v_sqrt_f32 v49, v49\n" \
+  "s_nop 0\n" \
+  "v_rcp_f32 v46, v49\n" \
+  "s_nop 0\n" \
+  "v_mul_f32 v37, |v177|, v46\n" \
+  "v_mul_f32 v50, v100, v43\n" \
+  "v_mul_f32 v50, v60, v50\n" \
+  "v_sqrt_f32 v50, v50\n" \
+  "s_nop 0\n" \
+  "v_mul_f32 v51, v101, v43\n" \
+  "v_mul_f32 v51, v60, v51\n" \
+  "v_sqrt_f32 v51, v51\n" \
+  "s_nop 0\n" \
+  "global_store_dwordx4 v47, v[48:51], s[46:47] nt\n" \
+  "v_add_u32 v47, s4, v47\n" \
+  "v_mul_f32 v52, v102, v43\n" \
+  "v_mul_f32 v52, v60, v52\n" \
+  "v_sqrt_f32 v52, v52\n" \
+  "s_nop 0\n" \
+  "v_mul_f32 v53, v104, v43\n" \
+  "v_mul_f32 v53, v61, v53\n" \
+  "v_sqrt_f32 v53, v53\n" \
+  "s_nop 0\n" \
+  "v_mul_f32 v54, v105, v43\n" \
+  "v_mul_f32 v54, v61, v54\n" \
+  "v_sqrt_f32 v54, v54\n" \
+  "s_nop 0\n" \
+  "v_mul_f32 v55, v103, v43\n" \
+  "v_mul_f32 v55, v61, v55\n" \
+  "v_sqrt_f32 v55, v55\n" \
+  "s_nop 0\n" \
+  "global_store_dwordx4 v47, v[52:55], s[46:47] nt\n" \
+  "v_add_u32 v47, s4, v47\n" \
+  "v_mul_f32 v48, v106, v43\n" \
+  "v_mul_f32 v48, v62, v48\n" \
+  "v_sqrt_f32 v48, v48\n" \
+  "s_nop 0\n" \
+  "v_rcp_f32 v46, v48\n" \
+  "s_nop 0\n" \
+  "v_mul_f32 v38, |v219|, v46\n" \
+  "v_mul_f32 v49, v107, v43\n" \
+  "v_mul_f32 v49, v63, v49\n" \
+  "v_sqrt_f32 v49, v49\n" \
+  "s_nop 0\n" \
+  "v_mul_f32 v50, v108, v43\n" \
+  "v_mul_f32 v50, v63, v50\n" \
+  "v_sqrt_f32 v50, v50\n" \
+  "s_nop 0\n" \
+  "v_mul_f32 v51, v109, v43\n" \
+  "v_mul_f32 v51, v62, v51\n" \
+  "v_sqrt_f32 v51, v51\n" \
+  "s_nop 0\n" \
+  "global_store_dwordx4 v47, v[48:51], s[46:47] nt\n" \
+  "v_add_u32 v47, s4, v47\n" \
+  "v_rcp_f32 v46, v51\n" \
+  "s_nop 0\n" \
+  "v_mul_f32 v39, |v222|, v46\n" \
+  "v_mul_f32 v52, v110, v43\n" \
+  "v_mul_f32 v52, v63, v52\n" \
+  "v_sqrt_f32 v52, v52\n" \
+  "s_nop 0\n" \
+  "v_mul_f32 v53, v111, v43\n" \
+  "v_mul_f32 v53, v63, v53\n" \
+  "v_sqrt_f32 v53, v53\n" \
+  "s_nop 0\n" \
+  "v_mul_f32 v54, v112, v43\n" \
+  "v_mul_f32 v54, v62, v54\n" \
+  "v_sqrt_f32 v54, v54\n" \
+  "s_nop 0\n" \
+  "v_rcp_f32 v46, v54\n" \
+  "s_nop 0\n" \
+  "v_mul_f32 v40, |v225|, v46\n" \
+  "v_mul_f32 v55, v113, v43\n" \
+  "v_mul_f32 v55, v63, v55\n" \
+  "v_sqrt_f32 v55, v55\n" \
+  "s_nop 0\n" \
+  "global_store_dwordx4 v47, v[52:55], s[46:47] nt\n" \
+  "s_mul_i32 s4, s10, 44\n" \
+  "v_add_u32 v47, s4, v0\n" \
+  "v_mul_f32 v45, v114, v43\n" \
+  "v_mul_f32 v45, v63, v45\n" \
   "v_sqrt_f32 v45, v45\n" \
   "s_nop 0\n" \
   "global_store_dword v47, v45, s[46:47] nt\n" \
   "v_add_u32 v47, s10, v47\n" \
-  "v_mul_f32 v45, v83, v43\n" \
-  "v_mul_f32 v45, v49, v45\n" \
-  "v_sqrt_f32 v45, v45\n" \
-  "s_nop 0\n" \
-  "global_store_dword v47, v45, s[46:47] nt\n" \
-  "v_add_u32 v47, s10, v47\n" \
-  "v_mul_f32 v45, v84, v43\n" \
-  "v_mul_f32 v45, v49, v45\n" \
-  "v_sqrt_f32 v45, v45\n" \
-  "s_nop 0\n" \
-  "global_store_dword v47, v45, s[46:47] nt\n" \
-  "v_add_u32 v47, s10, v47\n" \
-  "v_mul_f32 v45, v86, v43\n" \
-  "v_mul_f32 v45, v50, v45\n" \
-  "v_sqrt_f32 v45, v45\n" \
-  "s_nop 0\n" \
-  "global_store_dword v47, v45, s[46:47] nt\n" \
-  "v_add_u32 v47, s10, v47\n" \
-  "v_mul_f32 v45, v87, v43\n" \
-  "v_mul_f32 v45, v50, v45\n" \
-  "v_sqrt_f32 v45, v45\n" \
-  "s_nop 0\n" \
-  "global_store_dword v47, v45, s[46:47] nt\n" \
-  "v_add_u32 v47, s10, v47\n" \
-  "v_mul_f32 v45, v85, v43\n" \
-  "v_mul_f32 v45, v50, v45\n" \
-  "v_sqrt_f32 v45, v45\n" \
-  "s_nop 0\n" \
-  "global_store_dword v47, v45, s[46:47] nt\n" \
-  "v_add_u32 v47, s10, v47\n" \
-  "v_mul_f32 v45, v88, v43\n" \
-  "v_mul_f32 v45, v51, v45\n" \
-  "v_sqrt_f32 v45, v45\n" \
-  "s_nop 0\n" \
-  "global_store_dword v47, v45, s[46:47] nt\n" \
-  "v_add_u32 v47, s10, v47\n" \
-  "v_rcp_f32 v46, v45\n" \
-  "s_nop 0\n" \
-  "v_mul_f32 v20, |v150|, v46\n" \
-  "v_mul_f32 v26, |v152|, v46\n" \
-  "v_mul_f32 v45, v89, v43\n" \
-  "v_mul_f32 v45, v51, v45\n" \
-  "v_sqrt_f32 v45, v45\n" \
-  "s_nop 0\n" \
-  "global_store_dword v47, v45, s[46:47] nt\n" \
-  "v_add_u32 v47, s10, v47\n" \
-  "v_rcp_f32 v46, v45\n" \
-  "s_nop 0\n" \
-  "v_mul_f32 v21, |v151|, v46\n" \
-  "v_mul_f32 v27, |v153|, v46\n" \
-  "v_mul_f32 v45, v90, v43\n" \
-  "v_mul_f32 v45, v51, v45\n" \
-  "v_sqrt_f32 v45, v45\n" \
-  "s_nop 0\n" \
-  "global_store_dword v47, v45, s[46:47] nt\n" \
-  "v_add_u32 v47, s10, v47\n" \
-  "v_rcp_f32 v46, v45\n" \
-  "s_nop 0\n" \
-  "v_mul_f32 v22, |v156|, v46\n" \
-  "v_mul_f32 v28, |v158|, v46\n" \
-  "v_mul_f32 v45, v92, v43\n" \
-  "v_mul_f32 v45, v53, v45\n" \
-  "v_sqrt_f32 v45, v45\n" \
-  "s_nop 0\n" \
-  "global_store_dword v47, v45, s[46:47] nt\n" \
-  "v_add_u32 v47, s10, v47\n" \
-  "v_rcp_f32 v46, v45\n" \
-  "s_nop 0\n" \
-  "v_mul_f32 v24, |v162|, v46\n" \
-  "v_mul_f32 v30, |v164|, v46\n" \
-  "v_mul_f32 v45, v93, v43\n" \
-  "v_mul_f32 v45, v53, v45\n" \
-  "v_sqrt_f32 v45, v45\n" \
-  "s_nop 0\n" \
-  "global_store_dword v47, v45, s[46:47] nt\n" \
-  "v_add_u32 v47, s10, v47\n" \
-  "v_rcp_f32 v46, v45\n" \
-  "s_nop 0\n" \
-  "v_mul_f32 v25, |v163|, v46\n" \
-  "v_mul_f32 v31, |v165|, v46\n" \
-  "v_mul_f32 v45, v91, v43\n" \
-  "v_mul_f32 v45, v53, v45\n" \
-  "v_sqrt_f32 v45, v45\n" \
-  "s_nop 0\n" \
-  "global_store_dword v47, v45, s[46:47] nt\n" \
-  "v_add_u32 v47, s10, v47\n" \
-  "v_rcp_f32 v46, v45\n" \
-  "s_nop 0\n" \
-  "v_mul_f32 v23, |v157|, v46\n" \
-  "v_mul_f32 v29, |v159|, v46\n" \
-  "v_mul_f32 v45, v94, v43\n" \
-  "v_mul_f32 v45, v51, v45\n" \
-  "v_sqrt_f32 v45, v45\n" \
-  "s_nop 0\n" \
-  "global_store_dword v47, v45, s[46:47] nt\n" \
-  "v_add_u32 v47, s10, v47\n" \
-  "v_rcp_f32 v46, v45\n" \
-  "s_nop 0\n" \
-  "v_mul_f32 v32, |v170|, v46\n" \
-  "v_mul_f32 v45, v95, v43\n" \
-  "v_mul_f32 v45, v51, v45\n" \
-  "v_sqrt_f32 v45, v45\n" \
-  "s_nop 0\n" \
-  "global_store_dword v47, v45, s[46:47] nt\n" \
-  "v_add_u32 v47, s10, v47\n" \
-  "v_rcp_f32 v46, v45\n" \
-  "s_nop 0\n" \
-  "v_mul_f32 v33, |v171|, v46\n" \
-  "v_mul_f32 v45, v96, v43\n" \
-  "v_mul_f32 v45, v51, v45\n" \
-  "v_sqrt_f32 v45, v45\n" \
-  "s_nop 0\n" \
-  "global_store_dword v47, v45, s[46:47] nt\n" \
-  "v_add_u32 v47, s10, v47\n" \
-  "v_rcp_f32 v46, v45\n" \
-  "s_nop 0\n" \
-  "v_mul_f32 v34, |v176|, v46\n" \
-  "v_mul_f32 v45, v98, v43\n" \
-  "v_mul_f32 v45, v53, v45\n" \
-  "v_sqrt_f32 v45, v45\n" \
-  "s_nop 0\n" \
-  "global_store_dword v47, v45, s[46:47] nt\n" \
-  "v_add_u32 v47, s10, v47\n" \
-  "v_rcp_f32 v46, v45\n" \
-  "s_nop 0\n" \
-  "v_mul_f32 v36, |v182|, v46\n" \
-  "v_mul_f32 v45, v99, v43\n" \
-  "v_mul_f32 v45, v53, v45\n" \
-  "v_sqrt_f32 v45, v45\n" \
-  "s_nop 0\n" \
-  "global_store_dword v47, v45, s[46:47] nt\n" \
-  "v_add_u32 v47, s10, v47\n" \
-  "v_rcp_f32 v46, v45\n" \
-  "s_nop 0\n" \
-  "v_mul_f32 v37, |v183|, v46\n" \
-  "v_mul_f32 v45, v97, v43\n" \
-  "v_mul_f32 v45, v53, v45\n" \
-  "v_sqrt_f32 v45, v45\n" \
-  "s_nop 0\n" \
-  "global_store_dword v47, v45, s[46:47] nt\n" \
-  "v_add_u32 v47, s10, v47\n" \
-  "v_rcp_f32 v46, v45\n" \
-  "s_nop 0\n" \
-  "v_mul_f32 v35, |v177|, v46\n" \
-  "v_mul_f32 v45, v100, v43\n" \
-  "v_mul_f32 v45, v52, v45\n" \
-  "v_sqrt_f32 v45, v45\n" \
-  "s_nop 0\n" \
-  "global_store_dword v47, v45, s[46:47] nt\n" \
-  "v_add_u32 v47, s10, v47\n" \
-  "v_mul_f32 v45, v101, v43\n" \
-  "v_mul_f32 v45, v52, v45\n" \
-  "v_sqrt_f32 v45, v45\n" \
-  "s_nop 0\n" \
-  "global_store_dword v47, v45, s[46:47] nt\n" \
-  "v_add_u32 v47, s10, v47\n" \
-  "v_mul_f32 v45, v102, v43\n" \
-  "v_mul_f32 v45, v52, v45\n" \
-  "v_sqrt_f32 v45, v45\n" \
-  "s_nop 0\n" \
-  "global_store_dword v47, v45, s[46:47] nt\n" \
-  "v_add_u32 v47, s10, v47\n" \
-  "v_mul_f32 v45, v104, v43\n" \
-  "v_mul_f32 v45, v53, v45\n" \
-  "v_sqrt_f32 v45, v45\n" \
-  "s_nop 0\n" \
-  "global_store_dword v47, v45, s[46:47] nt\n" \
-  "v_add_u32 v47, s10, v47\n" \
-  "v_mul_f32 v45, v105, v43\n" \
-  "v_mul_f32 v45, v53, v45\n" \
-  "v_sqrt_f32 v45, v45\n" \
-  "s_nop 0\n" \
-  "global_store_dword v47, v45, s[46:47] nt\n" \
-  "v_add_u32 v47, s10, v47\n" \
-  "v_mul_f32 v45, v103, v43\n" \
-  "v_mul_f32 v45, v53, v45\n" \
-  "v_sqrt_f32 v45, v45\n" \
-  "s_nop 0\n" \
-  "global_store_dword v47, v45, s[46:47] nt\n" \
-  "v_add_u32 v47, s10, v47\n" \
-  "v_mul_f32 v45, v106, v43\n" \
-  "v_mul_f32 v45, v54, v45\n" \
-  "v_sqrt_f32 v45, v45\n" \
-  "s_nop 0\n" \
-  "global_store_dword v47, v45, s[46:47] nt\n" \
-  "v_add_u32 v47, s10, v47\n" \
-  "v_rcp_f32 v46, v45\n" \
-  "s_nop 0\n" \
-  "v_mul_f32 v38, |v219|, v46\n" \
-  "v_mul_f32 v45, v107, v43\n" \
-  "v_mul_f32 v45, v55, v45\n" \
-  "v_sqrt_f32 v45, v45\n" \
-  "s_nop 0\n" \
-  "global_store_dword v47, v45, s[46:47] nt\n" \
-  "v_add_u32 v47, s10, v47\n" \
-  "v_mul_f32 v45, v108, v43\n" \
-  "v_mul_f32 v45, v55, v45\n" \
-  "v_sqrt_f32 v45, v45\n" \
-  "s_nop 0\n" \
-  "global_store_dword v47, v45, s[46:47] nt\n" \
-  "v_add_u32 v47, s10, v47\n" \
-  "v_mul_f32 v45, v109, v43\n" \
-  "v_mul_f32 v45, v54, v45\n" \
-  "v_sqrt_f32 v45, v45\n" \
-  "s_nop 0\n" \
-  "global_store_dword v47, v45, s[46:47] nt\n" \
-  "v_add_u32 v47, s10, v47\n" \
-  "v_rcp_f32 v46, v45\n" \
-  "s_nop 0\n" \
-  "v_mul_f32 v39, |v222|, v46\n" \
-  "v_mul_f32 v45, v110, v43\n" \
-  "v_mul_f32 v45, v55, v45\n" \
-  "v_sqrt_f32 v45, v45\n" \
-  "s_nop 0\n" \
-  "global_store_dword v47, v45, s[46:47] nt\n" \
-  "v_add_u32 v47, s10, v47\n" \
-  "v_mul_f32 v45, v111, v43\n" \
-  "v_mul_f32 v45, v55, v45\n" \
-  "v_sqrt_f32 v45, v45\n" \
-  "s_nop 0\n" \
-  "global_store_dword v47, v45, s[46:47] nt\n" \
-  "v_add_u32 v47, s10, v47\n" \
-  "v_mul_f32 v45, v112, v43\n" \
-  "v_mul_f32 v45, v54, v45\n" \
-  "v_sqrt_f32 v45, v45\n" \
-  "s_nop 0\n" \
-  "global_store_dword v47, v45, s[46:47] nt\n" \
-  "v_add_u32 v47, s10, v47\n" \
-  "v_rcp_f32 v46, v45\n" \
-  "s_nop 0\n" \
-  "v_mul_f32 v40, |v225|, v46\n" \
-  "v_mul_f32 v45, v113, v43\n" \
-  "v_mul_f32 v45, v55, v45\n" \
-  "v_sqrt_f32 v45, v45\n" \
-  "s_nop 0\n" \
-  "global_store_dword v47, v45, s[46:47] nt\n" \
-  "v_add_u32 v47, s10, v47\n" \
-  "v_mul_f32 v45, v114, v43\n" \
-  "v_mul_f32 v45, v55, v45\n" \
-  "v_sqrt_f32 v45, v45\n" \
-  "s_nop 0\n" \
-  "global_store_dword v47, v45, s[46:47] nt\n" \
-  "v_add_u32 v47, s10, v47\n" \
-  "global_store_dword v47, v2, s[46:47] nt\n" \
-  "v_add_u32 v47, s10, v47\n" \
-  "global_store_dword v47, v3, s[46:47] nt\n" \
-  "v_add_u32 v47, s10, v47\n" \
-  "global_store_dword v47, v4, s[46:47] nt\n" \
-  "v_add_u32 v47, s10, v47\n" \
-  "global_store_dword v47, v6, s[46:47] nt\n" \
-  "v_add_u32 v47, s10, v47\n" \
-  "global_store_dword v47, v7, s[46:47] nt\n" \
-  "v_add_u32 v47, s10, v47\n" \
-  "global_store_dword v47, v5, s[46:47] nt\n" \
-  "v_add_u32 v47, s10, v47\n" \
-  "global_store_dword v47, v8, s[46:47] nt\n" \
-  "v_add_u32 v47, s10, v47\n" \
-  "global_store_dword v47, v9, s[46:47] nt\n" \
-  "v_add_u32 v47, s10, v47\n" \
-  "global_store_dword v47, v10, s[46:47] nt\n" \
-  "v_add_u32 v47, s10, v47\n" \
-  "global_store_dword v47, v12, s[46:47] nt\n" \
-  "v_add_u32 v47, s10, v47\n" \
-  "global_store_dword v47, v13, s[46:47] nt\n" \
-  "v_add_u32 v47, s10, v47\n" \
-  "global_store_dword v47, v11, s[46:47] nt\n" \
-  "v_add_u32 v47, s10, v47\n" \
-  "global_store_dword v47, v14, s[46:47] nt\n" \
-  "v_add_u32 v47, s10, v47\n" \
-  "global_store_dword v47, v15, s[46:47] nt\n" \
-  "v_add_u32 v47, s10, v47\n" \
-  "global_store_dword v47, v16, s[46:47] nt\n" \
-  "v_add_u32 v47, s10, v47\n" \
-  "global_store_dword v47, v18, s[46:47] nt\n" \
-  "v_add_u32 v47, s10, v47\n" \
-  "global_store_dword v47, v19, s[46:47] nt\n" \
-  "v_add_u32 v47, s10, v47\n" \
-  "global_store_dword v47, v17, s[46:47] nt\n" \
-  "v_add_u32 v47, s10, v47\n" \
-  "global_store_dword v47, v20, s[46:47] nt\n" \
-  "v_add_u32 v47, s10, v47\n" \
-  "global_store_dword v47, v21, s[46:47] nt\n" \
-  "v_add_u32 v47, s10, v47\n" \
-  "global_store_dword v47, v22, s[46:47] nt\n" \
-  "v_add_u32 v47, s10, v47\n" \
-  "global_store_dword v47, v24, s[46:47] nt\n" \
-  "v_add_u32 v47, s10, v47\n" \
-  "global_store_dword v47, v25, s[46:47] nt\n" \
-  "v_add_u32 v47, s10, v47\n" \
-  "global_store_dword v47, v23, s[46:47] nt\n" \
-  "v_add_u32 v47, s10, v47\n" \
-  "global_store_dword v47, v26, s[46:47] nt\n" \
-  "v_add_u32 v47, s10, v47\n" \
-  "global_store_dword v47, v27, s[46:47] nt\n" \
-  "v_add_u32 v47, s10, v47\n" \
-  "global_store_dword v47, v28, s[46:47] nt\n" \
-  "v_add_u32 v47, s10, v47\n" \
-  "global_store_dword v47, v30, s[46:47] nt\n" \
-  "v_add_u32 v47, s10, v47\n" \
-  "global_store_dword v47, v31, s[46:47] nt\n" \
-  "v_add_u32 v47, s10, v47\n" \
-  "global_store_dword v47, v29, s[46:47] nt\n" \
-  "v_add_u32 v47, s10, v47\n" \
-  "global_store_dword v47, v32, s[46:47] nt\n" \
-  "v_add_u32 v47, s10, v47\n" \
-  "global_store_dword v47, v33, s[46:47] nt\n" \
-  "v_add_u32 v47, s10, v47\n" \
-  "global_store_dword v47, v34, s[46:47] nt\n" \
-  "v_add_u32 v47, s10, v47\n" \
-  "global_store_dword v47, v36, s[46:47] nt\n" \
-  "v_add_u32 v47, s10, v47\n" \
-  "global_store_dword v47, v37, s[46:47] nt\n" \
-  "v_add_u32 v47, s10, v47\n" \
-  "global_store_dword v47, v35, s[46:47] nt\n" \
-  "v_add_u32 v47, s10, v47\n" \
+  "s_mul_i32 s4, s10, 45\n" \
+  "v_lshlrev_b32 v47, 2, v0\n" \
+  "v_add_u32 v47, s4, v47\n" \
+  "s_lshl_b32 s4, s10, 2\n" \
+  "global_store_dwordx4 v47, v[2:5], s[46:47] nt\n" \
+  "v_add_u32 v47, s4, v47\n" \
+  "global_store_dwordx4 v47, v[6:9], s[46:47] nt\n" \
+  "v_add_u32 v47, s4, v47\n" \
+  "global_store_dwordx4 v47, v[10:13], s[46:47] nt\n" \
+  "v_add_u32 v47, s4, v47\n" \
+  "global_store_dwordx4 v47, v[14:17], s[46:47] nt\n" \
+  "v_add_u32 v47, s4, v47\n" \
+  "global_store_dwordx4 v47, v[18:21], s[46:47] nt\n" \
+  "v_add_u32 v47, s4, v47\n" \
+  "global_store_dwordx4 v47, v[22:25], s[46:47] nt\n" \
+  "v_add_u32 v47, s4, v47\n" \
+  "global_store_dwordx4 v47, v[26:29], s[46:47] nt\n" \
+  "v_add_u32 v47, s4, v47\n" \
+  "global_store_dwordx4 v47, v[30:33], s[46:47] nt\n" \
+  "v_add_u32 v47, s4, v47\n" \
+  "global_store_dwordx4 v47, v[34:37], s[46:47] nt\n" \
+  "s_mul_i32 s4, s10, 0x51\n" \
+  "v_add_u32 v47, s4, v0\n" \
   "global_store_dword v47, v38, s[46:47] nt\n" \
   "v_add_u32 v47, s10, v47\n" \
   "global_store_dword v47, v39, s[46:47] nt\n" \
@@ -2511,11 +2419,11 @@
   "v_accvgpr_write_b32 a183, v44\n" \
   "v_mul_f32 v44, v48, v4\n" \
   "v_accvgpr_write_b32 a184, v44\n" \
-  "v_mul_f32 v44, v49, v6\n" \
+  "v_mul_f32 v44, v49, v5\n" \
   "v_accvgpr_write_b32 a185, v44\n" \
-  "v_mul_f32 v44, v50, v7\n" \
+  "v_mul_f32 v44, v50, v6\n" \
   "v_accvgpr_write_b32 a186, v44\n" \
-  "v_mul_f32 v44, v51, v5\n" \
+  "v_mul_f32 v44, v51, v7\n" \
   "v_accvgpr_write_b32 a187, v44\n" \
   "v_accvgpr_write_b32 a188, v45\n" \
   "v_accvgpr_write_b32 a189, v45\n" \
@@ -2535,11 +2443,11 @@
   "v_accvgpr_write_b32 a201, v44\n" \
   "v_mul_f32 v44, v54, v22\n" \
   "v_accvgpr_write_b32 a202, v44\n" \
-  "v_mul_f32 v44, v55, v24\n" \
+  "v_mul_f32 v44, v55, v23\n" \
   "v_accvgpr_write_b32 a203, v44\n" \
-  "v_mul_f32 v44, v56, v25\n" \
+  "v_mul_f32 v44, v56, v24\n" \
   "v_accvgpr_write_b32 a204, v44\n" \
-  "v_mul_f32 v44, v57, v23\n" \
+  "v_mul_f32 v44, v57, v25\n" \
   "v_accvgpr_write_b32 a205, v44\n" \
   "v_mul_f32 v44, v58, v26\n" \
   "v_accvgpr_write_b32 a206, v44\n" \
@@ -6261,71 +6169,27 @@
   "global_load_dword v187, v174, s[46:47] nt\n" \
   "v_add_u32 v174, s10, v174\n" \
   "global_load_dword v185, v174, s[46:47] nt\n" \
-  "v_add_u32 v174, s10, v174\n" \
-  "global_load_dword v188, v174, s[46:47] nt\n" \
-  "v_add_u32 v174, s10, v174\n" \
-  "global_load_dword v189, v174, s[46:47] nt\n" \
-  "v_add_u32 v174, s10, v174\n" \
-  "global_load_dword v190, v174, s[46:47] nt\n" \
-  "v_add_u32 v174, s10, v174\n" \
-  "global_load_dword v192, v174, s[46:47] nt\n" \
-  "v_add_u32 v174, s10, v174\n" \
-  "global_load_dword v193, v174, s[46:47] nt\n" \
-  "v_add_u32 v174, s10, v174\n" \
-  "global_load_dword v191, v174, s[46:47] nt\n" \
-  "v_add_u32 v174, s10, v174\n" \
-  "global_load_dword v194, v174, s[46:47] nt\n" \
-  "v_add_u32 v174, s10, v174\n" \
-  "global_load_dword v195, v174, s[46:47] nt\n" \
-  "v_add_u32 v174, s10, v174\n" \
-  "global_load_dword v196, v174, s[46:47] nt\n" \
-  "v_add_u32 v174, s10, v174\n" \
-  "global_load_dword v198, v174, s[46:47] nt\n" \
-  "v_add_u32 v174, s10, v174\n" \
-  "global_load_dword v199, v174, s[46:47] nt\n" \
-  "v_add_u32 v174, s10, v174\n" \
-  "global_load_dword v197, v174, s[46:47] nt\n" \
-  "v_add_u32 v174, s10, v174\n" \
-  "global_load_dword v200, v174, s[46:47] nt\n" \
-  "v_add_u32 v174, s10, v174\n" \
-  "global_load_dword v201, v174, s[46:47] nt\n" \
-  "v_add_u32 v174, s10, v174\n" \
-  "global_load_dword v202, v174, s[46:47] nt\n" \
-  "v_add_u32 v174, s10, v174\n" \
-  "global_load_dword v204, v174, s[46:47] nt\n" \
-  "v_add_u32 v174, s10, v174\n" \
-  "global_load_dword v205, v174, s[46:47] nt\n" \
-  "v_add_u32 v174, s10, v174\n" \
-  "global_load_dword v203, v174, s[46:47] nt\n" \
-  "v_add_u32 v174, s10, v174\n" \
-  "global_load_dword v206, v174, s[46:47] nt\n" \
-  "v_add_u32 v174, s10, v174\n" \
-  "global_load_dword v207, v174, s[46:47] nt\n" \
-  "v_add_u32 v174, s10, v174\n" \
-  "global_load_dword v214, v174, s[46:47] nt\n" \
-  "v_add_u32 v174, s10, v174\n" \
-  "global_load_dword v216, v174, s[46:47] nt\n" \
-  "v_add_u32 v174, s10, v174\n" \
-  "global_load_dword v217, v174, s[46:47] nt\n" \
-  "v_add_u32 v174, s10, v174\n" \
-  "global_load_dword v215, v174, s[46:47] nt\n" \
-  "v_add_u32 v174, s10, v174\n" \
-  "global_load_dword v218, v174, s[46:47] nt\n" \
-  "v_add_u32 v174, s10, v174\n" \
-  "global_load_dword v219, v174, s[46:47] nt\n" \
-  "v_add_u32 v174, s10, v174\n" \
-  "global_load_dword v220, v174, s[46:47] nt\n" \
-  "v_add_u32 v174, s10, v174\n" \
-  "global_load_dword v221, v174, s[46:47] nt\n" \
-  "v_add_u32 v174, s10, v174\n" \
-  "global_load_dword v222, v174, s[46:47] nt\n" \
-  "v_add_u32 v174, s10, v174\n" \
-  "global_load_dword v223, v174, s[46:47] nt\n" \
-  "v_add_u32 v174, s10, v174\n" \
-  "global_load_dword v224, v174, s[46:47] nt\n" \
-  "v_add_u32 v174, s10, v174\n" \
-  "global_load_dword v225, v174, s[46:47] nt\n" \
-  "v_add_u32 v174, s10, v174\n" \
+  "s_mul_i32 s4, s10, 12\n" \
+  "v_lshlrev_b32 v174, 2, v0\n" \
+  "v_add_u32 v174, s4, v174\n" \
+  "s_lshl_b32 s4, s10, 2\n" \
+  "global_load_dwordx4 v[188:191], v174, s[46:47] nt\n" \
+  "v_add_u32 v174, s4, v174\n" \
+  "global_load_dwordx4 v[192:195], v174, s[46:47] nt\n" \
+  "v_add_u32 v174, s4, v174\n" \
+  "global_load_dwordx4 v[196:199], v174, s[46:47] nt\n" \
+  "v_add_u32 v174, s4, v174\n" \
+  "global_load_dwordx4 v[200:203], v174, s[46:47] nt\n" \
+  "v_add_u32 v174, s4, v174\n" \
+  "global_load_dwordx4 v[204:207], v174, s[46:47] nt\n" \
+  "v_add_u32 v174, s4, v174\n" \
+  "global_load_dwordx4 v[214:217], v174, s[46:47] nt\n" \
+  "v_add_u32 v174, s4, v174\n" \
+  "global_load_dwordx4 v[218:221], v174, s[46:47] nt\n" \
+  "v_add_u32 v174, s4, v174\n" \
+  "global_load_dwordx4 v[222:225], v174, s[46:47] nt\n" \
+  "s_mul_i32 s4, s10, 44\n" \
+  "v_add_u32 v174, s4, v0\n" \
   "global_load_dword v226, v174, s[46:47] nt\n" \
   "v_accvgpr_read_b32 v176, a246\n" \
   "v_accvgpr_read_b32 v177, a247\n" \
@@ -6625,6 +6489,22 @@
   "global_store_dword v174, v212, s[42:43] nt\n" \
   "v_add_u32 v174, s10, v174\n" \
   "s_waitcnt vmcnt(0)\n" \
+  "v_mov_b32 v209, v193\n" \
+  "v_mov_b32 v228, v199\n" \
+  "v_mov_b32 v229, v205\n" \
+  "v_mov_b32 v193, v192\n" \
+  "v_mov_b32 v199, v198\n" \
+  "v_mov_b32 v205, v204\n" \
+  "v_mov_b32 v192, v191\n" \
+  "v_mov_b32 v198, v197\n" \
+  "v_mov_b32 v204, v203\n" \
+  "v_mov_b32 v191, v209\n" \
+  "v_mov_b32 v197, v228\n" \
+  "v_mov_b32 v203, v229\n" \
+  "v_mov_b32 v209, v217\n" \
+  "v_mov_b32 v217, v216\n" \
+  "v_mov_b32 v216, v215\n" \
+  "v_mov_b32 v215, v209\n" \
   "v_pk_mul_f32 v[2:3], v[176:177], v[2:3] op_sel:[0,0] op_sel_hi:[1,1] neg_lo:[0,0] neg_hi:[0,0]\n" \
   "v_pk_mul_f32 v[88:89], v[176:177], v[88:89] op_sel:[0,0] op_sel_hi:[1,1] neg_lo:[0,0] neg_hi:[0,0]\n" \
   "v_pk_mul_f32 v[4:5], v[178:179], v[4:5] op_sel:[0,0] op_sel_hi:[1,1] neg_lo:[0,0] neg_hi:[0,0]\n" \
@@ -6672,79 +6552,28 @@
   "v_pk_mul_f32 v[46:47], v[226:227], v[46:47] op_sel:[0,0] op_sel_hi:[1,1] neg_lo:[0,0] neg_hi:[0,0]\n" \
   "v_pk_mul_f32 v[132:133], v[226:227], v[132:133] op_sel:[0,0] op_sel_hi:[1,1] neg_lo:[0,0] neg_hi:[0,0]\n" \
   "s_mul_i32 s4, s10, 45\n" \
+  "v_lshlrev_b32 v174, 2, v0\n" \
+  "v_add_u32 v174, s4, v174\n" \
+  "s_lshl_b32 s4, s10, 2\n" \
+  "global_load_dwordx4 v[176:179], v174, s[46:47] nt\n" \
+  "v_add_u32 v174, s4, v174\n" \
+  "global_load_dwordx4 v[180:183], v174, s[46:47] nt\n" \
+  "v_add_u32 v174, s4, v174\n" \
+  "global_load_dwordx4 v[184:187], v174, s[46:47] nt\n" \
+  "v_add_u32 v174, s4, v174\n" \
+  "global_load_dwordx4 v[188:191], v174, s[46:47] nt\n" \
+  "v_add_u32 v174, s4, v174\n" \
+  "global_load_dwordx4 v[192:195], v174, s[46:47] nt\n" \
+  "v_add_u32 v174, s4, v174\n" \
+  "global_load_dwordx4 v[196:199], v174, s[46:47] nt\n" \
+  "v_add_u32 v174, s4, v174\n" \
+  "global_load_dwordx4 v[200:203], v174, s[46:47] nt\n" \
+  "v_add_u32 v174, s4, v174\n" \
+  "global_load_dwordx4 v[204:207], v174, s[46:47] nt\n" \
+  "v_add_u32 v174, s4, v174\n" \
+  "global_load_dwordx4 v[214:217], v174, s[46:47] nt\n" \
+  "s_mul_i32 s4, s10, 0x51\n" \
   "v_add_u32 v174, s4, v0\n" \
-  "global_load_dword v176, v174, s[46:47] nt\n" \
-  "v_add_u32 v174, s10, v174\n" \
-  "global_load_dword v177, v174, s[46:47] nt\n" \
-  "v_add_u32 v174, s10, v174\n" \
-  "global_load_dword v178, v174, s[46:47] nt\n" \
-  "v_add_u32 v174, s10, v174\n" \
-  "global_load_dword v180, v174, s[46:47] nt\n" \
-  "v_add_u32 v174, s10, v174\n" \
-  "global_load_dword v181, v174, s[46:47] nt\n" \
-  "v_add_u32 v174, s10, v174\n" \
-  "global_load_dword v179, v174, s[46:47] nt\n" \
-  "v_add_u32 v174, s10, v174\n" \
-  "global_load_dword v182, v174, s[46:47] nt\n" \
-  "v_add_u32 v174, s10, v174\n" \
-  "global_load_dword v183, v174, s[46:47] nt\n" \
-  "v_add_u32 v174, s10, v174\n" \
-  "global_load_dword v184, v174, s[46:47] nt\n" \
-  "v_add_u32 v174, s10, v174\n" \
-  "global_load_dword v186, v174, s[46:47] nt\n" \
-  "v_add_u32 v174, s10, v174\n" \
-  "global_load_dword v187, v174, s[46:47] nt\n" \
-  "v_add_u32 v174, s10, v174\n" \
-  "global_load_dword v185, v174, s[46:47] nt\n" \
-  "v_add_u32 v174, s10, v174\n" \
-  "global_load_dword v188, v174, s[46:47] nt\n" \
-  "v_add_u32 v174, s10, v174\n" \
-  "global_load_dword v189, v174, s[46:47] nt\n" \
-  "v_add_u32 v174, s10, v174\n" \
-  "global_load_dword v190, v174, s[46:47] nt\n" \
-  "v_add_u32 v174, s10, v174\n" \
-  "global_load_dword v192, v174, s[46:47] nt\n" \
-  "v_add_u32 v174, s10, v174\n" \
-  "global_load_dword v193, v174, s[46:47] nt\n" \
-  "v_add_u32 v174, s10, v174\n" \
-  "global_load_dword v191, v174, s[46:47] nt\n" \
-  "v_add_u32 v174, s10, v174\n" \
-  "global_load_dword v194, v174, s[46:47] nt\n" \
-  "v_add_u32 v174, s10, v174\n" \
-  "global_load_dword v195, v174, s[46:47] nt\n" \
-  "v_add_u32 v174, s10, v174\n" \
-  "global_load_dword v196, v174, s[46:47] nt\n" \
-  "v_add_u32 v174, s10, v174\n" \
-  "global_load_dword v198, v174, s[46:47] nt\n" \
-  "v_add_u32 v174, s10, v174\n" \
-  "global_load_dword v199, v174, s[46:47] nt\n" \
-  "v_add_u32 v174, s10, v174\n" \
-  "global_load_dword v197, v174, s[46:47] nt\n" \
-  "v_add_u32 v174, s10, v174\n" \
-  "global_load_dword v200, v174, s[46:47] nt\n" \
-  "v_add_u32 v174, s10, v174\n" \
-  "global_load_dword v201, v174, s[46:47] nt\n" \
-  "v_add_u32 v174, s10, v174\n" \
-  "global_load_dword v202, v174, s[46:47] nt\n" \
-  "v_add_u32 v174, s10, v174\n" \
-  "global_load_dword v204, v174, s[46:47] nt\n" \
-  "v_add_u32 v174, s10, v174\n" \
-  "global_load_dword v205, v174, s[46:47] nt\n" \
-  "v_add_u32 v174, s10, v174\n" \
-  "global_load_dword v203, v174, s[46:47] nt\n" \
-  "v_add_u32 v174, s10, v174\n" \
-  "global_load_dword v206, v174, s[46:47] nt\n" \
-  "v_add_u32 v174, s10, v174\n" \
-  "global_load_dword v207, v174, s[46:47] nt\n" \
-  "v_add_u32 v174, s10, v174\n" \
-  "global_load_dword v214, v174, s[46:47] nt\n" \
-  "v_add_u32 v174, s10, v174\n" \
-  "global_load_dword v216, v174, s[46:47] nt\n" \
-  "v_add_u32 v174, s10, v174\n" \
-  "global_load_dword v217, v174, s[46:47] nt\n" \
-  "v_add_u32 v174, s10, v174\n" \
-  "global_load_dword v215, v174, s[46:47] nt\n" \
-  "v_add_u32 v174, s10, v174\n" \
   "global_load_dword v218, v174, s[46:47] nt\n" \
   "v_add_u32 v174, s10, v174\n" \
   "global_load_dword v219, v174, s[46:47] nt\n" \
@@ -6849,6 +6678,30 @@
   "v_mov_b32 v250, s87\n" \
   "33:\n" \
   "s_waitcnt vmcnt(0)\n" \
+  "v_mov_b32 v251, v181\n" \
+  "v_mov_b32 v252, v187\n" \
+  "v_mov_b32 v253, v193\n" \
+  "v_mov_b32 v181, v180\n" \
+  "v_mov_b32 v187, v186\n" \
+  "v_mov_b32 v193, v192\n" \
+  "v_mov_b32 v180, v179\n" \
+  "v_mov_b32 v186, v185\n" \
+  "v_mov_b32 v192, v191\n" \
+  "v_mov_b32 v179, v251\n" \
+  "v_mov_b32 v185, v252\n" \
+  "v_mov_b32 v191, v253\n" \
+  "v_mov_b32 v251, v199\n" \
+  "v_mov_b32 v252, v205\n" \
+  "v_mov_b32 v253, v217\n" \
+  "v_mov_b32 v199, v198\n" \
+  "v_mov_b32 v205, v204\n" \
+  "v_mov_b32 v217, v216\n" \
+  "v_mov_b32 v198, v197\n" \
+  "v_mov_b32 v204, v203\n" \
+  "v_mov_b32 v216, v215\n" \
+  "v_mov_b32 v197, v251\n" \
+  "v_mov_b32 v203, v252\n" \
+  "v_mov_b32 v215, v253\n" \
   "v_pk_mul_f32 v[48:49], v[176:177], v[48:49] op_sel:[0,0] op_sel_hi:[1,1] neg_lo:[0,0] neg_hi:[0,0]\n" \
   "v_pk_mul_f32 v[134:135], v[176:177], v[134:135] op_sel:[0,0] op_sel_hi:[1,1] neg_lo:[0,0] neg_hi:[0,0]\n" \
   "v_pk_mul_f32 v[50:51], v[178:179], v[50:51] op_sel:[0,0] op_sel_hi:[1,1] neg_lo:[0,0] neg_hi:[0,0]\n" \
diff --git a/robobee3d_amd/isasim.py b/robobee3d_amd/isasim.py
--- a/robobee3d_amd/isasim.py
+++ b/robobee3d_amd/isasim.py
@@ -110,7 +110,7 @@
                 self.V[:, r] = val
             self.V[:, LANE_LDS_VGPR] = 16 * np.arange(lanes)
         self.lds = np.zeros((1, 0), u32) if lds is None else lds
-        self.regions = [(b, st, arr, arr.view(u32).reshape(-1), arr.itemsize) for b, st, arr in regions]
+        self.regions = [(r[0], r[1], r[2], r[2].view(u32).reshape(-1), r[2].itemsize, r[3] if len(r) > 3 else 0) for r in regions]
         self.set_exec(np.ones(lanes, bool))
         self.scc = 0
         self.max_exec, self.quad, self.log = max_exec, quad or {}, log
@@ -219,11 +219,13 @@
 
     def gaddr(self, sbase, voff, imm, ln, n):
         addr = (self.s64(sbase) + (int(self.V[ln, _decode(voff)[1]]) if voff is not None else 0) + imm) & 0xFFFFFFFFFFFFFFFF
-        for base, stride, arr, words, size in self.regions:
+        for base, stride, arr, words, size, cell in self.regions:
             if base <= addr < base + len(arr) * stride:
                 i, b = divmod(addr - base, stride)
                 if b % 4 == 0 and b + 4 * n <= size * (len(arr) - i if stride == size else 1):
                     return words, (i * size + b) // 4
+                if cell and size == 4 and b % 4 == 0 and b + 4 * n <= cell and i + b // 4 + n <= len(arr):
+                    return words, i + b // 4
         raise AddressFault("%r touches 0x%016x, outside every array of the call" % (self.ins[self.pc], addr))
 
     def lds_word(self, base, off, ln):
@@ -627,6 +629,7 @@
     "v_and_b32": _bitop(lambda a, b: a & b),
     "v_or_b32": _bitop(lambda a, b: a | b),
     "v_lshrrev_b32": _bitop(lambda a, b: b >> (a & u64(31))),
+    "v_lshlrev_b32": _bitop(lambda a, b: (b << (a & u64(31))) & u64(0xFFFFFFFF)),
     "v_mul_u32_u24": _bitop(lambda a, b: ((a & u64(0xFFFFFF)) * (b & u64(0xFFFFFF))) & u64(0xFFFFFFFF)),
     "v_bfe_u32": lambda mc, t: mc.write(t[1], (mc.bits(t[2]) >> u32(t[3] & 31)) & u32((1 << t[4]) - 1)),
     "v_cvt_f32_i32": lambda mc, t: mc.wf(t[1], mc.bits(t[2]).view(np.int32).astype(f32)),
@@ -669,5 +672,6 @@
     VECTOR["v_cmp_%s_f32" % _op] = VECTOR["v_cmp_%s_f32_e64" % _op] = _cmp("f32")
 OPS = dict(SALU, **VECTOR)
 for _m in ("ds_read_b32", "ds_read_b64", "ds_read_b128", "ds_write_b32", "ds_write_b64", "ds_write_b128", "ds_min_f32",
-           "global_load_dword", "global_load_dwordx2", "global_load_dwordx4", "global_store_dword", "global_store_dwordx2"):
+           "global_load_dword", "global_load_dwordx2", "global_load_dwordx4", "global_store_dword", "global_store_dwordx2",
+           "global_store_dwordx4"):
     OPS[_m] = _ds if _m.startswith("ds_") else _global
```

Measured after the change: 549.9 million (median of 6 runs). Within noise of the previous version (+0.8%).
